# LasseWolter/laughter-detection-icsi

Hardware: AMD Instinct MI355X
Metric: 1 s@16 kHz segments/sec (featurize+ResNet fwd/bwd) (higher is better)
Workload: dtype f32 (64->64 and 32->32 convolutions: f16x2 split operands with per-tile power-of-two scales, f32 accumulate; error vs float64 within 1.5x of the exact-f32 kernels'); 1 GPU; BASELINE configs[2]: end-to-end featurize (HIP fbank 44 mel) + ResNetBigger resnet_base fwd/bwd + clip + Adam, random labels, dropout 0.5; global_batch=512, parallelism=dp1, overlap_wgrad=False, overlap_wgrad_small=True, bf16x3_convs=True, f16x2_convs=True, relu_bits=True, virtual_a1=True

## Files before the change

### include/lad_hip.h

```cpp
#ifndef LAD_HIP_H
#define LAD_HIP_H

#include <stdint.h>

#ifdef __cplusplus
extern "C" {
#endif

#define LAD_VERSION 100

enum lad_status {
    LAD_OK = 0,
    LAD_ERR_INVALID = -1,
    LAD_ERR_HIP = -2,
    LAD_ERR_NOMEM = -3,
    LAD_NOT_COVERED = 1
};

int lad_version(void);
const char *lad_last_error(void);

enum lad_pad_mode {
    LAD_PAD_KALDI_MIRROR = 0,
    LAD_PAD_CENTER_REFLECT = 1,
    LAD_PAD_CENTER_ZERO = 2
};
enum lad_log_mode {
    LAD_LOG_LN = 0,
    LAD_LOG_DB = 1,
    LAD_LOG_NONE = 2
};

typedef struct lad_fbank_cfg {
    int32_t n_fft;
    int32_t frame_len;
    int32_t hop;
    int32_t n_mels;
    int32_t n_mfcc;
    int32_t pad_mode;
    int32_t log_mode;
    int32_t remove_dc;
    float preemph;
    float log_floor;
} lad_fbank_cfg;

int lad_fbank_plan_create(const lad_fbank_cfg *cfg, const float *window, const float *melbank,
                          const float *dct, void **plan_out);
int lad_fbank_plan_destroy(void *plan);
int lad_fbank_plan_set_kernel(void *plan, int32_t which);
int lad_fbank_plan_has_fast_kernel(const void *plan);
int64_t lad_fbank_num_frames(const void *plan, int64_t samples_per_clip);
int lad_fbank_forward(void *plan, const float *pcm, int64_t n_clips, int64_t samples_per_clip,
                      float *out, void *stream);
int lad_fbank_forward_long(void *plan, const float *pcm, int64_t n_samples, float *out, void *stream);

int lad_gather_segments(const float *const *chan_ptr, const int64_t *chan_frames, const int32_t *chan,
                        const int64_t *first, const int32_t *count, int64_t n_seg, int32_t n_frames, int32_t F, float pad,
                        float *out, void *stream);

typedef struct lad_augment_params {
    uint64_t seed;
    uint32_t epoch;
    float p, mix_p;
    float snr_lo, snr_hi;
    float gain_lo, gain_hi;
    int32_t W;
    int32_t n_time, Wt;
    int32_t n_freq, Wf;
} lad_augment_params;
int lad_gather_segments_aug(const float *const *chan_ptr, const int64_t *chan_frames, const int32_t *chan,
                            const int64_t *first, const int32_t *count, int64_t n_seg, int32_t n_frames, int32_t F, float pad,
                            const lad_augment_params *params, const int32_t *noise_list, int32_t n_noise,
                            int64_t min_noise_frames, float *out, void *stream);

int lad_assemble_windows(const void *stream_act, const void *strips, void *out, int64_t n_windows, int32_t H, int32_t W,
                         int32_t band, int32_t row_bytes, void *stream);


int64_t lad_act_rows(int64_t batch, int32_t H, int32_t W);

int64_t lad_conv_packed_weight_floats(int32_t cout, int32_t cin, int32_t taps, int32_t mode);
int lad_conv_pack_weights(const float *w, int32_t cout, int32_t cin, int32_t taps, int32_t mode, float *wt,
                          void *stream);
int lad_conv_pack_weights_multi(const void *descs, int32_t n_desc, void *stream);
int64_t lad_conv_num_tiles(int64_t batch, int32_t H, int32_t W);
int lad_conv_fwd(const float *in, const float *wt, const float *bias, const float *addend, float *out,
                 float *stat_partials, int64_t batch, int32_t H, int32_t W, int32_t cin, int32_t cout, int32_t taps,
                 void *stream);
int lad_conv_s2_fwd(const float *in, const float *wt, const float *bias, float *out, float *stat_partials,
                    int64_t batch, int32_t H, int32_t W, int32_t cin, int32_t cout, int32_t taps, void *stream);
int lad_bn_fold(const float *gamma, const float *beta, const float *running_mean, const float *running_var,
                const float *conv_bias, int32_t channels, float *scale, float *shift, void *stream);
int lad_conv_fwd_eval(const float *in, const float *wt, const float *scale, const float *shift, const float *addend,
                      float *out, int64_t batch, int32_t H, int32_t W, int32_t cin, int32_t cout, int32_t taps,
                      int32_t relu, void *stream);
int lad_conv_s2_fwd_eval(const float *in, const float *wt, const float *scale, const float *shift, float *out,
                         int64_t batch, int32_t H, int32_t W, int32_t cin, int32_t cout, int32_t taps, int32_t relu,
                         void *stream);
int lad_upsample2(const float *src, float *up, int64_t batch, int32_t H, int32_t W, int32_t channels, void *stream);
int lad_conv_s2_dgrad(const float *dout, const float *wt, float *dx, int64_t batch, int32_t H, int32_t W, int32_t cin,
                      int32_t cout, int32_t taps, int32_t accumulate, void *stream);
int64_t lad_conv_s2_wgrad_workspace_floats(int32_t cin, int32_t cout, int32_t taps);
int lad_conv_s2_wgrad(const float *in, const float *dout, float *workspace, float *dw, float *dbias, int64_t batch, int32_t H,
                      int32_t W, int32_t cin, int32_t cout, int32_t taps, void *stream);
int64_t lad_conv_s2_wgrad_fused_workspace_floats(int32_t cin, int32_t cout);
int lad_conv_s2_wgrad_fused(const float *in, const float *dout, const float *dout_sc, float *workspace, float *dw,
                            float *dbias, float *dw_sc, int64_t batch, int32_t H, int32_t W, int32_t cin, int32_t cout,
                            void *stream);
int lad_conv_s2_fwd_fused(const float *in, const float *wt, const float *bias, const float *wt_sc, float *out,
                          float *stat_partials, float *out_sc, float *stat_partials_sc, int64_t batch, int32_t H, int32_t W,
                          int32_t cin, int32_t cout, void *stream);
int lad_conv_s2_dgrad_fused(const float *dout, const float *wt, const float *dout_sc, const float *wt_sc, float *dx,
                            int64_t batch, int32_t H, int32_t W, int32_t cin, int32_t cout, void *stream);
int64_t lad_conv_s2b3_packed_weight_bytes(void);
int lad_conv_s2b3_pack_weights(const float *w, const float *w_sc, void *wt, void *stream);
int lad_conv_s2b3_fwd(const float *in, const void *wt, const float *bias, float *out, float *stat_partials, float *out_sc,
                      float *stat_partials_sc, int64_t batch, int32_t H, int32_t W, void *stream);
int64_t lad_conv_s2b3_dgrad_packed_weight_bytes(void);
int lad_conv_s2b3_dgrad_pack_weights(const float *w, const float *w_sc, void *wt, void *stream);
int lad_conv_s2b3_pack_weights_pair(const float *w, const float *w_sc, void *wt_fwd, void *wt_dgrad, void *stream);
int64_t lad_conv_s2b3_dgrad_partials(int64_t batch, int32_t H, int32_t W);
int lad_conv_s2b3_dgrad(const float *dout, const float *dout_sc, const void *wt, float *dx, float *stat_partials, const float *bn_x,
                        const uint64_t *bn_bits, const float *bn_coef, int64_t batch, int32_t H, int32_t W, void *stream);
int64_t lad_conv_s2_dgrad_partials(int64_t batch, int32_t H, int32_t W);
int lad_conv_s2_dgrad_fused_bnstat(const float *dout, const float *wt, const float *dout_sc, const float *wt_sc, float *dx,
                                   float *stat_partials, const float *bn_x, const uint64_t *bn_bits, const float *bn_coef,
                                   int64_t batch, int32_t H, int32_t W, int32_t cin, int32_t cout, void *stream);
int64_t lad_conv_wgrad_workspace_floats(int32_t cin, int32_t cout, int32_t taps);
int lad_conv_wgrad(const float *in, const float *dout, float *workspace, float *dw, float *dbias, int64_t batch,
                   int32_t H, int32_t W, int32_t cin, int32_t cout, int32_t taps, void *stream);

int64_t lad_conv_b3_packed_weight_bytes(void);
int lad_conv_b3_pack_weights(const float *w, int32_t mode, void *wt, void *stream);
int lad_conv_b3_fwd_f32(const float *in, const void *wt, const float *bias, const float *addend, float *out,
                        float *partials, int64_t batch, int32_t H, int32_t W, void *stream);
int lad_conv_b3_fwd_f32_gated(const float *in, const void *wt, const float *bias, const float *addend,
                              const uint64_t *addend_bits, float *out, float *partials, int64_t batch, int32_t H,
                              int32_t W, void *stream);
int lad_conv_b3_dgrad_bnstat(const float *in, const void *wt, const float *addend, const uint64_t *addend_bits,
                             float *out, float *stat_partials, const float *bn_x, const uint64_t *bn_bits,
                             const float *bn_coef, int64_t batch, int32_t H, int32_t W, void *stream);
int64_t lad_conv_b3c_packed_weight_bytes(int32_t channels);
int lad_conv_b3c_pack_weights(const float *w, int32_t mode, void *wt, int32_t channels, void *stream);
int lad_conv_b3c_fwd_f32(const float *in, const void *wt, const float *bias, const float *addend, float *out,
                         float *partials, int64_t batch, int32_t H, int32_t W, int32_t channels, void *stream);
int lad_conv_b3c_dgrad_bnstat(const float *in, const void *wt, const float *addend, float *out, float *stat_partials,
                              const float *bn_x, const float *bn_coef, int64_t batch, int32_t H, int32_t W,
                              int32_t channels, void *stream);
int lad_conv_b3c_fwd_f32_bnrelu(const float *in, const float *in_coef, const void *wt, const float *bias, float *out,
                                float *partials, int64_t batch, int32_t H, int32_t W, int32_t channels, void *stream);
int64_t lad_conv_h2_packed_weight_bytes(int32_t channels);
int lad_conv_h2_pack_weights_multi(const void *table, int32_t n, int32_t channels, void *stream);
int lad_conv_wgrad_h2(const float *in, const float *in_coef, const float *dout, float *workspace, float *dw, float *dbias,
                      int64_t batch, int32_t H, int32_t W, int32_t channels, void *stream);
int lad_conv_wgrad_h2_bnbwd(const float *in, const float *in_coef, const float *dy, const float *bn_x, const uint64_t *bn_bits,
                            const float *bn_coef, const float *bcoef, float *dc, float *workspace, float *dw, float *dbias,
                            int64_t batch, int32_t H, int32_t W, int32_t channels, void *stream);
int lad_conv_h2(const float *in, const float *in_coef, const void *wt, const float *bias, const float *addend,
                const uint64_t *addend_bits, float *out, float *partials, const float *bn_x, const uint64_t *bn_bits,
                const float *bn_coef, int64_t batch, int32_t H, int32_t W, int32_t channels, void *stream);
int64_t lad_conv_wgrad_b3c_workspace_floats(int32_t channels);
int lad_conv_wgrad_b3c(const float *in, const float *in_coef, const float *dout, float *workspace, float *dw, float *dbias,
                       int64_t batch, int32_t H, int32_t W, int32_t channels, void *stream);
int lad_conv_b3_fwd_f32_bnrelu(const float *in, const float *in_coef, const void *wt, const float *bias, float *out,
                               float *partials, int64_t batch, int32_t H, int32_t W, void *stream);
int lad_conv_wgrad_b3_bnrelu(const float *in, const float *in_coef, const float *dout, float *workspace, float *dw,
                             float *dbias, int64_t batch, int32_t H, int32_t W, void *stream);
int lad_wgrad_defer_begin(void);
int lad_wgrad_defer_flush(void *stream);
int lad_conv_wgrad_b3(const float *in, const float *dout, float *workspace, float *dw, float *dbias, int64_t batch,
                      int32_t H, int32_t W, void *stream);

int lad_stem_fwd(const float *feat, const float *weight, float *out, float *stat_partials, int64_t batch, int32_t H,
                 int32_t W, int32_t cout, void *stream);
int lad_stem_fwd_eval(const float *feat, const float *weight, const float *scale, const float *shift, float *out,
                      int64_t batch, int32_t H, int32_t W, int32_t cout, int64_t frame_stride, int64_t frames_avail,
                      void *stream);
int64_t lad_stem_moments_workspace_doubles(void);
int64_t lad_stem_moments_doubles(void);
int lad_stem_bn_stats(const float *feat, const float *weight, const float *gamma, const float *beta, float *running_mean,
                      float *running_var, float momentum, float *coef, double *moments, double *workspace, int64_t batch, int32_t H,
                      int32_t W, int32_t cout, void *stream);
int64_t lad_stem_bwd_onepass_workspace_floats(void);
int lad_stem_bwd_onepass(const float *feat, const float *weight, const float *dy, const float *coef, const float *gamma,
                         const double *moments, float *workspace, float *dw, float *dgamma, float *dbeta, int64_t batch, int32_t H,
                         int32_t W, int32_t cout, void *stream);
int64_t lad_stem_wgrad_workspace_floats(void);
int lad_stem_wgrad(const float *feat, const float *dout, float *workspace, float *dw, int64_t batch, int32_t H,
                   int32_t W, int32_t cout, void *stream);
int lad_stem_wgrad_bn(const float *feat, const float *dy, const float *x, const float *weight, const float *coef,
                      const float *bcoef, float *workspace, float *dw, int64_t batch, int32_t H, int32_t W, int32_t cout,
                      void *stream);
int64_t lad_stem_bn_bwd_groups(int64_t batch, int32_t H, int32_t W);
int lad_stem_bn_bwd_sums(const float *feat, const float *weight, const float *dy, const float *coef, float *partials,
                         int64_t batch, int32_t H, int32_t W, int32_t cout, void *stream);

int lad_bn_finalize(float *stat_partials, int64_t n_tiles, int32_t channels, int64_t count, const float *gamma,
                    const float *beta, float *running_mean, float *running_var, float momentum, float *coef,
                    void *stream);
int lad_bn_finalize_pair(float *stat_partials_a, float *stat_partials_b, int64_t n_tiles, int32_t channels, int64_t count,
                         const float *gamma_a, const float *beta_a, float *running_mean_a, float *running_var_a, float *coef_a,
                         const float *gamma_b, const float *beta_b, float *running_mean_b, float *running_var_b, float *coef_b,
                         float momentum, void *stream);
int lad_bn_act(const float *x, const float *coef, const float *res, const float *res_coef, float *y, int64_t batch,
               int32_t H, int32_t W, int32_t channels, int32_t relu, void *stream);
int64_t lad_bn_bwd_workspace_floats(int32_t channels);
int lad_bn_bwd(const float *dy, const float *y, const float *x, const float *coef, const float *gamma,
               const float *xs, const float *scoef, const float *sgamma, float *dx, float *aux, float *dgamma,
               float *dbeta, float *dsgamma, float *dsbeta, float *workspace, float *bcoef, float *pre_partials,
               int64_t pre_tiles, int64_t batch, int32_t H, int32_t W, int32_t channels, int32_t relu, int32_t mode,
               void *stream);
int lad_bn_act_bits(const float *x, const float *coef, const float *res, const float *res_coef, float *y,
                    uint64_t *y_bits, int64_t batch, int32_t H, int32_t W, int32_t channels, void *stream);
int lad_bn_bwd_bits(const float *dy, const uint64_t *y_bits, const float *x, const float *coef, const float *gamma,
                    float *dx, float *dgamma, float *dbeta, float *workspace, float *bcoef, float *pre_partials,
                    int64_t pre_tiles, int64_t batch, int32_t H, int32_t W, int32_t channels, void *stream);
int lad_conv_fwd_bnstat(const float *in, const float *wt, const float *addend, float *out, float *stat_partials,
                        const float *bn_x, const float *bn_y, const float *bn_coef, int64_t batch, int32_t H, int32_t W,
                        int32_t cin, int32_t cout, int32_t taps, void *stream);

int lad_pool_fwd(const float *x, float *pooled, int64_t batch, int32_t H, int32_t W, int32_t channels, void *stream);
int lad_pool_bwd(const float *dpooled, float *dx, int64_t batch, int32_t H, int32_t W, int32_t channels, void *stream);
int64_t lad_head_workspace_floats(int64_t batch, int32_t F);
int lad_head_fwd_train(const float *const *params, const float *pooled, int64_t batch, int32_t F, const float *drop1,
                       const float *drop2, const int32_t *labels, float momentum, float *h, float *stats,
                       float *probs, float *metrics, void *stream);
int lad_head_fwd_train_rng(const float *const *params, const float *pooled, int64_t batch, int32_t F, float *drop1, float *drop2, float keep,
                           uint64_t seed, int64_t *rng_counter, int64_t *nbt, int32_t n_nbt, const int32_t *labels, float momentum,
                           float *h, float *stats, float *probs, float *metrics, void *stream);
int lad_head_fwd_eval(const float *const *params, const float *pooled, int64_t batch, int32_t F, float *probs,
                      void *stream);
int lad_bce_metrics(const float *probs, const int32_t *labels, int64_t n, float *metrics, void *stream);
int lad_head_bwd(const float *const *params, float *const *grads, const float *pooled, const float *h,
                 const float *stats, const float *probs, const float *dprobs, int64_t batch, int32_t F,
                 const float *drop1, const float *drop2, const int32_t *labels, float *workspace, float *dpooled,
                 void *stream);

int64_t lad_f16_packed_weight_halfs(int32_t cout, int32_t cin, int32_t taps);
int lad_f16_pack_weights(const float *w, int32_t cout, int32_t cin, int32_t taps, void *wt, void *stream);
int lad_f16_stem_fwd(const float *feat, const float *weight, const float *scale, const float *shift, void *out,
                     int64_t batch, int32_t H, int32_t W, int32_t cout, int64_t frame_stride, int64_t frames_avail,
                     void *stream);
int lad_f16_conv_fwd(const void *in, const void *wt, const float *scale, const float *shift, const void *addend, void *out,
                     int64_t batch, int32_t H, int32_t W, int32_t cin, int32_t cout, int32_t taps, int32_t relu,
                     void *stream);
int lad_f16_conv_s2_fwd(const void *in, const void *wt, const float *scale, const float *shift, void *out, int64_t batch,
                        int32_t H, int32_t W, int32_t cin, int32_t cout, int32_t taps, int32_t relu, void *stream);
int lad_f16_block_fwd(const void *x, const void *wt1, const float *scale1, const float *shift1, const void *wt2,
                      const float *scale2, const float *shift2, void *y, int64_t batch, int32_t H, int32_t W, int32_t channels,
                      void *stream);
int lad_f16_block_fwd_stem_rows(const void *stream_act, int64_t stream_rows, int64_t stream_row0, const float *feat, int64_t frames_avail,
                                const float *stem_weight, const float *stem_scale, const float *stem_shift, const void *wt1,
                                const float *scale1, const float *shift1, const void *wt2, const float *scale2, const float *shift2, void *y,
                                int64_t batch, int32_t H, int32_t W, void *stream);
int lad_f16_conv_s2_strips_fwd(const void *act, const void *wt, const float *scale, const float *shift, void *out, const void *wt_sc,
                               const float *scale_sc, const float *shift_sc, void *out_sc, int64_t n_windows, int32_t H, int32_t W,
                               int32_t band, int32_t strip_rows, int64_t bottom_image0, int64_t stream_row0, int64_t act_rows,
                               int32_t out_rows, void *stream);
int lad_f16_tail_fwd(const void *act, int64_t n_windows, int32_t H, int32_t W, int32_t band, int32_t strip_rows, int64_t bot_img0,
                     int64_t stream_row0, int32_t phases, int64_t phase_img, int64_t act_rows, const void *const *conv_params,
                     const float *const *head_params, int32_t F, float *probs, void *stream);
int lad_f16_conv_s2_fwd_windows(const void *act, const void *wt, const float *scale, const float *shift, void *out,
                                int64_t n_windows, int32_t H, int32_t W, int32_t band, int32_t cin, int32_t cout, int32_t taps,
                                int32_t relu, void *stream);
int lad_f16_conv_s2_fwd_mapped(const void *act, const void *wt, const float *scale, const float *shift, void *out,
                               int64_t n_windows, int32_t H, int32_t W, int32_t band, int32_t strip_rows, int64_t bottom_image0,
                               int64_t stream_row0, int32_t phases, int64_t phase_rows, int64_t act_rows, int32_t out_rows,
                               int32_t cin, int32_t cout, int32_t taps, int32_t relu, void *stream);
int lad_f16_conv_s2_fwd_sc(const void *in, const void *wt, const float *scale, const float *shift, void *out, const void *wt_sc,
                           const float *scale_sc, const float *shift_sc, void *out_sc, int64_t batch, int32_t H, int32_t W,
                           int32_t cin, int32_t cout, int32_t relu, void *stream);
int lad_f16_conv_s2_fwd_mapped_sc(const void *act, const void *wt, const float *scale, const float *shift, void *out,
                                  const void *wt_sc, const float *scale_sc, const float *shift_sc, void *out_sc, int64_t n_windows,
                                  int32_t H, int32_t W, int32_t band, int32_t strip_rows, int64_t bottom_image0, int64_t stream_row0,
                                  int32_t phases, int64_t phase_rows, int64_t act_rows, int32_t out_rows, int32_t cin, int32_t cout,
                                  int32_t relu, void *stream);
int lad_f16_pool_fwd(const void *x, float *pooled, int64_t batch, int32_t H, int32_t W, int32_t channels, void *stream);

int32_t lad_grad_sumsq_partials(void);
int lad_grad_sumsq(const float *grad, int64_t n, float *partials, int64_t *step_counter, void *stream);
int lad_grad_accumulate(float *acc, const float *grad, int64_t n, double scale, void *stream);
int lad_adam_step(float *param, float *grad, float *exp_avg, float *exp_avg_sq, int64_t n,
                  const float *sumsq_partials, double grad_scale, double max_norm, double lr, double beta1,
                  double beta2, double eps, int64_t step, const int64_t *step_counter, int32_t zero_grad,
                  float *norm_out, void *stream);

enum lad_runs_dtype { LAD_RUNS_F32 = 0, LAD_RUNS_F64 = 1 };
int32_t lad_runs_tile_frames(void);
int32_t lad_runs_max_thresholds(void);
int64_t lad_runs_workspace_bytes(int64_t channels, int64_t frames, int32_t n_thresholds);
int lad_runs_count(const void *probs, int32_t dtype, int64_t channels, int64_t frames, const double *thresholds,
                   int32_t n_thresholds, void *workspace, void *stream);
int lad_runs_fill(const void *probs, int32_t dtype, int64_t channels, int64_t frames, const double *thresholds,
                  int32_t n_thresholds, const void *workspace, const int32_t *counts_host, int32_t *table,
                  int64_t capacity_runs, void *stream);

enum lad_score_class { LAD_SCORE_INVALID = 0, LAD_SCORE_LAUGH = 1, LAD_SCORE_SPEECH = 2, LAD_SCORE_NOISE = 3, LAD_SCORE_SILENCE = 4 };
enum lad_score_field { LAD_SCORE_N_PRED = 0, LAD_SCORE_N_VALID = 1, LAD_SCORE_PRED_MS = 2, LAD_SCORE_CORR_MS = 3,
                       LAD_SCORE_FP_SPEECH_MS = 4, LAD_SCORE_FP_NOISE_MS = 5, LAD_SCORE_FP_SILENCE_MS = 6, LAD_SCORE_FIELDS = 7 };
int32_t lad_score_max_min_lengths(void);
int64_t lad_score_workspace_bytes(int64_t channels, int64_t n_intervals, int32_t n_thresholds, int32_t n_min_lengths);
int lad_score_runs(const void *runs_workspace, const int32_t *table, const int32_t *counts_host, int64_t channels,
                   int64_t frames, int32_t n_thresholds, const int32_t *bounds, const int32_t *offsets,
                   const int32_t *bounds_host, const int32_t *offsets_host, int64_t n_intervals, const double *fps,
                   const double *fps_host, const double *min_lengths, int32_t n_min_lengths, void *workspace,
                   int64_t *scores, void *stream);

enum lad_event_field { LAD_EVENT_N_REF = 0, LAD_EVENT_REF_TOUCHED = 1, LAD_EVENT_REF_HIT = 2, LAD_EVENT_PRED_HIT = 3,
                       LAD_EVENT_LINKS = 4, LAD_EVENT_ONSET_ABS_MS = 5, LAD_EVENT_OFFSET_ABS_MS = 6, LAD_EVENT_FIELDS = 7 };
int64_t lad_score_events_workspace_bytes(int64_t channels, int64_t n_intervals, int32_t n_thresholds, int32_t n_min_lengths,
                                         int64_t total_runs);
int lad_score_events(const void *runs_workspace, const int32_t *table, const int32_t *counts_host, int64_t channels,
                     int64_t frames, int32_t n_thresholds, const int32_t *bounds, const int32_t *offsets,
                     const int32_t *bounds_host, const int32_t *offsets_host, int64_t n_intervals, const double *fps,
                     const double *fps_host, const double *min_lengths, int32_t n_min_lengths,
                     int32_t min_overlap_ms, int32_t min_overlap_pct, void *workspace, int64_t *events, void *stream);

int32_t lad_binarize_max_settings(void);
int64_t lad_binarize_workspace_bytes(int64_t channels, int64_t frames, int32_t n_settings);
int lad_binarize_count(const void *probs, int32_t dtype, int64_t channels, int64_t frames, const double *onsets,
                       const double *offsets, int32_t n_settings, void *workspace, void *stream);
int lad_binarize_fill(const void *probs, int32_t dtype, int64_t channels, int64_t frames, const double *onsets,
                      const double *offsets, const double *min_gaps, int32_t n_settings, const double *fps,
                      const double *fps_host, void *workspace, const int32_t *counts_host, int32_t *raw_table,
                      int32_t *table, int64_t capacity_runs, void *stream);

int32_t lad_viterbi_max_settings(void);
int32_t lad_viterbi_table_entries(void);
int64_t lad_viterbi_workspace_bytes(int64_t channels, int64_t frames, int32_t n_settings);
int lad_viterbi_count(const void *probs, int32_t dtype, int64_t channels, int64_t frames, const int32_t *emission,
                      const int32_t *emission_host, const int32_t *bias, const int32_t *penalty, int32_t n_settings,
                      void *workspace, int64_t *best, void *stream);
int lad_viterbi_fill(const void *workspace, const int32_t *counts_host, int64_t channels, int64_t frames, int32_t n_settings,
                     int32_t *table, int64_t capacity_runs, void *stream);

int32_t lad_surface_max_levels(void);
int32_t lad_surface_tile_frames(void);
int64_t lad_surface_workspace_bytes(int64_t channels, int64_t frames, int64_t n_intervals, int32_t n_levels, int32_t n_min_lengths);
int lad_score_surface(const void *probs, int32_t dtype, int64_t channels, int64_t frames, const double *levels, int32_t n_levels,
                      const int32_t *bounds, const int32_t *offsets, const int32_t *bounds_host, const int32_t *offsets_host,
                      int64_t n_intervals, const double *fps, const double *fps_host, const double *min_lengths,
                      int32_t n_min_lengths, void *workspace, int64_t *scores, void *stream);

enum lad_resample_dtype { LAD_RESAMPLE_F32 = 0, LAD_RESAMPLE_I16 = 1 };
int64_t lad_resample_out_len(int64_t n_in, int32_t up, int32_t down);
int32_t lad_resample_tile_outputs(void);
int32_t lad_resample_max_up(void);
int32_t lad_resample_max_down(void);
int32_t lad_resample_max_taps(void);
int64_t lad_resample_max_lds_bytes(void);
int64_t lad_resample_lds_bytes(int32_t up, int32_t down, int32_t K);
int lad_resample(const void *x, int32_t x_dtype, int64_t n_in, const float *table, int32_t up, int32_t down, int32_t K,
                 int64_t out_first, int64_t n_out, float *y, void *stream);

int32_t lad_lowpass_tile_frames(void);
int64_t lad_lowpass_workspace_bytes(int64_t channels, int64_t frames);
int lad_lowpass(const void *probs, int32_t dtype, int64_t channels, int64_t frames, const int64_t *lengths_host,
                const double *b_host, const double *a_host, const double *zi_host, double *out, void *workspace,
                void *stream);

enum lad_sample_kind { LAD_SAMPLE_FIXED = 0, LAD_SAMPLE_POOL_ROW = 1, LAD_SAMPLE_POOL_MEASURE = 2 };
int lad_sample_segments(const int32_t *kind, const int32_t *src, int64_t n_rows, const int64_t *row_id, const int32_t *regions,
                        int64_t n_regions, const int32_t *pool_off, const int64_t *pool_cum, int32_t n_pools,
                        const int32_t *kind_host, const int32_t *src_host, const int32_t *pool_off_host,
                        const int64_t *pool_total_host, int32_t T, uint64_t seed, uint32_t epoch, int32_t *chan, int64_t *first,
                        int32_t *count, int32_t *region, void *stream);
int lad_window_coverage(const int32_t *set_chan, const int64_t *first, const int32_t *count, int64_t n, int32_t fps,
                        const int32_t *bounds, const int32_t *offsets, const int32_t *bounds_host, const int32_t *offsets_host,
                        int64_t n_intervals, int32_t n_channels, int32_t n_sets, int32_t *out, void *stream);

#ifdef __cplusplus
}
#endif
#endif
```

### laughter-detection-icsi_amd/_hip.py

```python
import ctypes
import os

import torch

_HERE = os.path.dirname(os.path.abspath(__file__))
LIB_PATH = os.environ.get("LAD_HIP_LIB") or os.path.join(_HERE, "liblad_hip.so")

c_void_p = ctypes.c_void_p
c_int = ctypes.c_int
c_i64 = ctypes.c_int64
c_float = ctypes.c_float
c_double = ctypes.c_double
c_i32 = ctypes.c_int32
c_float_p = ctypes.POINTER(ctypes.c_float)


class LadHipError(RuntimeError):
    pass


class FbankCfg(ctypes.Structure):
    _fields_ = [("n_fft", ctypes.c_int32), ("frame_len", ctypes.c_int32), ("hop", ctypes.c_int32),
                ("n_mels", ctypes.c_int32), ("n_mfcc", ctypes.c_int32), ("pad_mode", ctypes.c_int32),
                ("log_mode", ctypes.c_int32), ("remove_dc", ctypes.c_int32), ("preemph", ctypes.c_float),
                ("log_floor", ctypes.c_float)]


class AugmentParams(ctypes.Structure):
    _fields_ = [("seed", ctypes.c_uint64), ("epoch", ctypes.c_uint32), ("p", ctypes.c_float), ("mix_p", ctypes.c_float),
                ("snr_lo", ctypes.c_float), ("snr_hi", ctypes.c_float), ("gain_lo", ctypes.c_float), ("gain_hi", ctypes.c_float),
                ("W", ctypes.c_int32), ("n_time", ctypes.c_int32), ("Wt", ctypes.c_int32), ("n_freq", ctypes.c_int32),
                ("Wf", ctypes.c_int32)]


SIGNATURES = {
    "lad_version": (c_int, []),
    "lad_last_error": (ctypes.c_char_p, []),
    "lad_fbank_plan_create": (c_int, [ctypes.POINTER(FbankCfg), c_void_p, c_void_p, c_void_p,
                                      ctypes.POINTER(c_void_p)]),
    "lad_fbank_plan_destroy": (c_int, [c_void_p]),
    "lad_fbank_plan_set_kernel": (c_int, [c_void_p, c_int]),
    "lad_fbank_plan_has_fast_kernel": (c_int, [c_void_p]),
    "lad_fbank_num_frames": (c_i64, [c_void_p, c_i64]),
    "lad_fbank_forward": (c_int, [c_void_p, c_void_p, c_i64, c_i64, c_void_p, c_void_p]),
    "lad_fbank_forward_long": (c_int, [c_void_p, c_void_p, c_i64, c_void_p, c_void_p]),
    "lad_gather_segments": (c_int, [c_void_p] * 5 + [c_i64, c_i32, c_i32, c_float, c_void_p, c_void_p]),
    "lad_gather_segments_aug": (c_int, [c_void_p] * 5 + [c_i64, c_i32, c_i32, c_float, ctypes.POINTER(AugmentParams), c_void_p, c_i32, c_i64,
                                        c_void_p, c_void_p]),
    "lad_assemble_windows": (c_int, [c_void_p, c_void_p, c_void_p, c_i64, c_i32, c_i32, c_i32, c_i32, c_void_p]),
    "lad_act_rows": (c_i64, [c_i64, c_i32, c_i32]),
    "lad_conv_packed_weight_floats": (c_i64, [c_i32, c_i32, c_i32, c_i32]),
    "lad_conv_pack_weights": (c_int, [c_void_p, c_i32, c_i32, c_i32, c_i32, c_void_p, c_void_p]),
    "lad_conv_pack_weights_multi": (c_int, [c_void_p, c_i32, c_void_p]),
    "lad_conv_num_tiles": (c_i64, [c_i64, c_i32, c_i32]),
    "lad_conv_fwd": (c_int, [c_void_p] * 6 + [c_i64, c_i32, c_i32, c_i32, c_i32, c_i32, c_void_p]),
    "lad_conv_b3_packed_weight_bytes": (c_i64, []),
    "lad_conv_b3_pack_weights": (c_int, [c_void_p, c_i32, c_void_p, c_void_p]),
    "lad_conv_b3_fwd_f32": (c_int, [c_void_p] * 6 + [c_i64, c_i32, c_i32, c_void_p]),
    "lad_conv_b3c_packed_weight_bytes": (c_i64, [c_i32]),
    "lad_conv_b3c_pack_weights": (c_int, [c_void_p, c_i32, c_void_p, c_i32, c_void_p]),
    "lad_conv_b3c_fwd_f32": (c_int, [c_void_p] * 6 + [c_i64, c_i32, c_i32, c_i32, c_void_p]),
    "lad_conv_b3c_fwd_f32_bnrelu": (c_int, [c_void_p] * 6 + [c_i64, c_i32, c_i32, c_i32, c_void_p]),
    "lad_conv_b3c_dgrad_bnstat": (c_int, [c_void_p] * 7 + [c_i64, c_i32, c_i32, c_i32, c_void_p]),
    "lad_conv_h2_packed_weight_bytes": (c_i64, [c_i32]),
    "lad_conv_h2_pack_weights_multi": (c_int, [c_void_p, c_i32, c_i32, c_void_p]),
    "lad_conv_wgrad_h2": (c_int, [c_void_p] * 6 + [c_i64, c_i32, c_i32, c_i32, c_void_p]),
    "lad_conv_h2": (c_int, [c_void_p] * 11 + [c_i64, c_i32, c_i32, c_i32, c_void_p]),
    "lad_conv_wgrad_h2_bnbwd": (c_int, [c_void_p] * 11 + [c_i64, c_i32, c_i32, c_i32, c_void_p]),
    "lad_conv_wgrad_b3c_workspace_floats": (c_i64, [c_i32]),
    "lad_conv_wgrad_b3c": (c_int, [c_void_p] * 6 + [c_i64, c_i32, c_i32, c_i32, c_void_p]),
    "lad_conv_b3_fwd_f32_gated": (c_int, [c_void_p] * 7 + [c_i64, c_i32, c_i32, c_void_p]),
    "lad_conv_b3_fwd_f32_bnrelu": (c_int, [c_void_p] * 6 + [c_i64, c_i32, c_i32, c_void_p]),
    "lad_conv_wgrad_b3_bnrelu": (c_int, [c_void_p] * 6 + [c_i64, c_i32, c_i32, c_void_p]),
    "lad_wgrad_defer_begin": (c_int, []),
    "lad_wgrad_defer_flush": (c_int, [c_void_p]),
    "lad_conv_b3_dgrad_bnstat": (c_int, [c_void_p] * 9 + [c_i64, c_i32, c_i32, c_void_p]),
    "lad_conv_wgrad_b3": (c_int, [c_void_p] * 5 + [c_i64, c_i32, c_i32, c_void_p]),
    "lad_conv_s2_fwd": (c_int, [c_void_p] * 5 + [c_i64, c_i32, c_i32, c_i32, c_i32, c_i32, c_void_p]),
    "lad_bn_fold": (c_int, [c_void_p] * 5 + [c_i32, c_void_p, c_void_p, c_void_p]),
    "lad_conv_fwd_eval": (c_int, [c_void_p] * 6 + [c_i64, c_i32, c_i32, c_i32, c_i32, c_i32, c_i32, c_void_p]),
    "lad_conv_s2_fwd_eval": (c_int, [c_void_p] * 5 + [c_i64, c_i32, c_i32, c_i32, c_i32, c_i32, c_i32, c_void_p]),
    "lad_upsample2": (c_int, [c_void_p, c_void_p, c_i64, c_i32, c_i32, c_i32, c_void_p]),
    "lad_conv_s2_dgrad": (c_int, [c_void_p] * 3 + [c_i64, c_i32, c_i32, c_i32, c_i32, c_i32, c_i32, c_void_p]),
    "lad_conv_s2_wgrad_workspace_floats": (c_i64, [c_i32, c_i32, c_i32]),
    "lad_conv_s2_fwd_fused": (c_int, [c_void_p] * 8 + [c_i64, c_i32, c_i32, c_i32, c_i32, c_void_p]),
    "lad_conv_s2_dgrad_partials": (c_i64, [c_i64, c_i32, c_i32]),
    "lad_conv_s2b3_packed_weight_bytes": (c_i64, []),
    "lad_conv_s2b3_pack_weights": (c_int, [c_void_p, c_void_p, c_void_p, c_void_p]),
    "lad_conv_s2b3_fwd": (c_int, [c_void_p] * 7 + [c_i64, c_i32, c_i32, c_void_p]),
    "lad_conv_s2b3_dgrad_packed_weight_bytes": (c_i64, []),
    "lad_conv_s2b3_dgrad_pack_weights": (c_int, [c_void_p, c_void_p, c_void_p, c_void_p]),
    "lad_conv_s2b3_pack_weights_pair": (c_int, [c_void_p] * 5),
    "lad_conv_s2b3_dgrad_partials": (c_i64, [c_i64, c_i32, c_i32]),
    "lad_conv_s2b3_dgrad": (c_int, [c_void_p] * 8 + [c_i64, c_i32, c_i32, c_void_p]),
    "lad_conv_s2_dgrad_fused_bnstat": (c_int, [c_void_p] * 9 + [c_i64, c_i32, c_i32, c_i32, c_i32, c_void_p]),
    "lad_conv_s2_dgrad_fused": (c_int, [c_void_p] * 5 + [c_i64, c_i32, c_i32, c_i32, c_i32, c_void_p]),
    "lad_conv_s2_wgrad_fused_workspace_floats": (c_i64, [c_i32, c_i32]),
    "lad_conv_s2_wgrad_fused": (c_int, [c_void_p] * 7 + [c_i64, c_i32, c_i32, c_i32, c_i32, c_void_p]),
    "lad_conv_s2_wgrad": (c_int, [c_void_p] * 5 + [c_i64, c_i32, c_i32, c_i32, c_i32, c_i32, c_void_p]),
    "lad_conv_wgrad_workspace_floats": (c_i64, [c_i32, c_i32, c_i32]),
    "lad_conv_wgrad": (c_int, [c_void_p] * 5 + [c_i64, c_i32, c_i32, c_i32, c_i32, c_i32, c_void_p]),
    "lad_stem_fwd": (c_int, [c_void_p] * 4 + [c_i64, c_i32, c_i32, c_i32, c_void_p]),
    "lad_stem_fwd_eval": (c_int, [c_void_p] * 5 + [c_i64, c_i32, c_i32, c_i32, c_i64, c_i64, c_void_p]),
    "lad_stem_wgrad_workspace_floats": (c_i64, []),
    "lad_stem_wgrad": (c_int, [c_void_p] * 4 + [c_i64, c_i32, c_i32, c_i32, c_void_p]),
    "lad_stem_wgrad_bn": (c_int, [c_void_p] * 8 + [c_i64, c_i32, c_i32, c_i32, c_void_p]),
    "lad_stem_bn_bwd_groups": (c_i64, [c_i64, c_i32, c_i32]),
    "lad_stem_bn_bwd_sums": (c_int, [c_void_p] * 5 + [c_i64, c_i32, c_i32, c_i32, c_void_p]),
    "lad_bn_finalize": (c_int, [c_void_p, c_i64, c_i32, c_i64, c_void_p, c_void_p, c_void_p, c_void_p, c_float,
                                c_void_p, c_void_p]),
    "lad_stem_moments_workspace_doubles": (c_i64, []),
    "lad_stem_moments_doubles": (c_i64, []),
    "lad_stem_bn_stats": (c_int, [c_void_p] * 6 + [c_float] + [c_void_p] * 3 + [c_i64, c_i32, c_i32, c_i32, c_void_p]),
    "lad_stem_bwd_onepass_workspace_floats": (c_i64, []),
    "lad_stem_bwd_onepass": (c_int, [c_void_p] * 10 + [c_i64, c_i32, c_i32, c_i32, c_void_p]),
    "lad_bn_finalize_pair": (c_int, [c_void_p, c_void_p, c_i64, c_i32, c_i64] + [c_void_p] * 10 + [c_float, c_void_p]),
    "lad_bn_act": (c_int, [c_void_p] * 5 + [c_i64, c_i32, c_i32, c_i32, c_i32, c_void_p]),
    "lad_bn_bwd_workspace_floats": (c_i64, [c_i32]),
    "lad_bn_act_bits": (c_int, [c_void_p] * 6 + [c_i64, c_i32, c_i32, c_i32, c_void_p]),
    "lad_bn_bwd_bits": (c_int, [c_void_p] * 11 + [c_i64, c_i64, c_i32, c_i32, c_i32, c_void_p]),
    "lad_bn_bwd": (c_int, [c_void_p] * 17 + [c_i64, c_i64, c_i32, c_i32, c_i32, c_i32, c_i32, c_void_p]),
    "lad_conv_fwd_bnstat": (c_int, [c_void_p] * 8 + [c_i64, c_i32, c_i32, c_i32, c_i32, c_i32, c_void_p]),
    "lad_pool_fwd": (c_int, [c_void_p, c_void_p, c_i64, c_i32, c_i32, c_i32, c_void_p]),
    "lad_pool_bwd": (c_int, [c_void_p, c_void_p, c_i64, c_i32, c_i32, c_i32, c_void_p]),
    "lad_head_workspace_floats": (c_i64, [c_i64, c_i32]),
    "lad_head_fwd_train": (c_int, [c_void_p, c_void_p, c_i64, c_i32, c_void_p, c_void_p, c_void_p, c_float,
                                   c_void_p, c_void_p, c_void_p, c_void_p, c_void_p]),
    "lad_head_fwd_train_rng": (c_int, [c_void_p, c_void_p, c_i64, c_i32, c_void_p, c_void_p, c_float, ctypes.c_uint64, c_void_p, c_void_p, c_i32,
                                       c_void_p, c_float, c_void_p, c_void_p, c_void_p, c_void_p, c_void_p]),
    "lad_head_fwd_eval": (c_int, [c_void_p, c_void_p, c_i64, c_i32, c_void_p, c_void_p]),
    "lad_bce_metrics": (c_int, [c_void_p, c_void_p, c_i64, c_void_p, c_void_p]),
    "lad_head_bwd": (c_int, [c_void_p] * 7 + [c_i64, c_i32] + [c_void_p] * 6),
    "lad_f16_packed_weight_halfs": (c_i64, [c_i32, c_i32, c_i32]),
    "lad_f16_pack_weights": (c_int, [c_void_p, c_i32, c_i32, c_i32, c_void_p, c_void_p]),
    "lad_f16_stem_fwd": (c_int, [c_void_p] * 5 + [c_i64, c_i32, c_i32, c_i32, c_i64, c_i64, c_void_p]),
    "lad_f16_conv_fwd": (c_int, [c_void_p] * 6 + [c_i64, c_i32, c_i32, c_i32, c_i32, c_i32, c_i32, c_void_p]),
    "lad_f16_block_fwd": (c_int, [c_void_p] * 8 + [c_i64, c_i32, c_i32, c_i32, c_void_p]),
    "lad_f16_conv_s2_fwd_sc": (c_int, [c_void_p] * 9 + [c_i64, c_i32, c_i32, c_i32, c_i32, c_i32, c_void_p]),
    "lad_f16_conv_s2_fwd_mapped_sc": (c_int, [c_void_p] * 9 + [c_i64, c_i32, c_i32, c_i32, c_i32, c_i64, c_i64, c_i32, c_i64, c_i64, c_i32,
                                              c_i32, c_i32, c_i32, c_void_p]),
    "lad_f16_conv_s2_fwd": (c_int, [c_void_p] * 5 + [c_i64, c_i32, c_i32, c_i32, c_i32, c_i32, c_i32, c_void_p]),
    "lad_f16_conv_s2_fwd_windows": (c_int, [c_void_p] * 5 + [c_i64, c_i32, c_i32, c_i32, c_i32, c_i32, c_i32, c_i32, c_void_p]),
    "lad_f16_conv_s2_fwd_mapped": (c_int, [c_void_p] * 5 + [c_i64, c_i32, c_i32, c_i32, c_i32, c_i64, c_i64, c_i32, c_i64, c_i64, c_i32,
                                                          c_i32, c_i32, c_i32, c_i32, c_void_p]),
    "lad_f16_block_fwd_stem_rows": (c_int, [c_void_p, c_i64, c_i64, c_void_p, c_i64] + [c_void_p] * 10 + [c_i64, c_i32, c_i32, c_void_p]),
    "lad_f16_conv_s2_strips_fwd": (c_int, [c_void_p] * 9 + [c_i64, c_i32, c_i32, c_i32, c_i32, c_i64, c_i64, c_i64, c_i32, c_void_p]),
    "lad_f16_tail_fwd": (c_int, [c_void_p, c_i64, c_i32, c_i32, c_i32, c_i32, c_i64, c_i64, c_i32, c_i64, c_i64, c_void_p, c_void_p, c_i32,
                                 c_void_p, c_void_p]),
    "lad_f16_pool_fwd": (c_int, [c_void_p, c_void_p, c_i64, c_i32, c_i32, c_i32, c_void_p]),
    "lad_grad_sumsq_partials": (c_i32, []),
    "lad_grad_sumsq": (c_int, [c_void_p, c_i64, c_void_p, c_void_p, c_void_p]),
    "lad_grad_accumulate": (c_int, [c_void_p, c_void_p, c_i64, c_double, c_void_p]),
    "lad_adam_step": (c_int, [c_void_p] * 4 + [c_i64, c_void_p] + [c_double] * 6 + [c_i64, c_void_p, c_i32, c_void_p, c_void_p]),
    "lad_runs_tile_frames": (c_i32, []),
    "lad_runs_max_thresholds": (c_i32, []),
    "lad_runs_workspace_bytes": (c_i64, [c_i64, c_i64, c_i32]),
    "lad_runs_count": (c_int, [c_void_p, c_i32, c_i64, c_i64, ctypes.POINTER(c_double), c_i32, c_void_p, c_void_p]),
    "lad_runs_fill": (c_int, [c_void_p, c_i32, c_i64, c_i64, ctypes.POINTER(c_double), c_i32, c_void_p,
                              ctypes.POINTER(c_i32), c_void_p, c_i64, c_void_p]),
    "lad_score_max_min_lengths": (c_i32, []),
    "lad_score_workspace_bytes": (c_i64, [c_i64, c_i64, c_i32, c_i32]),
    "lad_score_runs": (c_int, [c_void_p, c_void_p, ctypes.POINTER(c_i32), c_i64, c_i64, c_i32, c_void_p, c_void_p,
                               ctypes.POINTER(c_i32), ctypes.POINTER(c_i32), c_i64, c_void_p, ctypes.POINTER(c_double),
                               ctypes.POINTER(c_double), c_i32, c_void_p, c_void_p, c_void_p]),
    "lad_score_events_workspace_bytes": (c_i64, [c_i64, c_i64, c_i32, c_i32, c_i64]),
    "lad_score_events": (c_int, [c_void_p, c_void_p, ctypes.POINTER(c_i32), c_i64, c_i64, c_i32, c_void_p, c_void_p,
                                 ctypes.POINTER(c_i32), ctypes.POINTER(c_i32), c_i64, c_void_p, ctypes.POINTER(c_double),
                                 ctypes.POINTER(c_double), c_i32, c_i32, c_i32, c_void_p, c_void_p, c_void_p]),
    "lad_binarize_max_settings": (c_i32, []),
    "lad_binarize_workspace_bytes": (c_i64, [c_i64, c_i64, c_i32]),
    "lad_binarize_count": (c_int, [c_void_p, c_i32, c_i64, c_i64, ctypes.POINTER(c_double), ctypes.POINTER(c_double), c_i32,
                                   c_void_p, c_void_p]),
    "lad_binarize_fill": (c_int, [c_void_p, c_i32, c_i64, c_i64] + [ctypes.POINTER(c_double)] * 3
                          + [c_i32, c_void_p, ctypes.POINTER(c_double), c_void_p, ctypes.POINTER(c_i32), c_void_p, c_void_p, c_i64,
                             c_void_p]),
    "lad_viterbi_max_settings": (c_i32, []),
    "lad_viterbi_table_entries": (c_i32, []),
    "lad_viterbi_workspace_bytes": (c_i64, [c_i64, c_i64, c_i32]),
    "lad_viterbi_count": (c_int, [c_void_p, c_i32, c_i64, c_i64, c_void_p] + [ctypes.POINTER(c_i32)] * 3
                          + [c_i32, c_void_p, c_void_p, c_void_p]),
    "lad_viterbi_fill": (c_int, [c_void_p, ctypes.POINTER(c_i32), c_i64, c_i64, c_i32, c_void_p, c_i64, c_void_p]),
    "lad_surface_max_levels": (c_i32, []),
    "lad_surface_tile_frames": (c_i32, []),
    "lad_surface_workspace_bytes": (c_i64, [c_i64, c_i64, c_i64, c_i32, c_i32]),
    "lad_score_surface": (c_int, [c_void_p, c_i32, c_i64, c_i64, ctypes.POINTER(c_double), c_i32, c_void_p, c_void_p,
                                  ctypes.POINTER(c_i32), ctypes.POINTER(c_i32), c_i64, c_void_p, ctypes.POINTER(c_double),
                                  ctypes.POINTER(c_double), c_i32, c_void_p, c_void_p, c_void_p]),
    "lad_resample_out_len": (c_i64, [c_i64, c_i32, c_i32]),
    "lad_resample_tile_outputs": (c_i32, []),
    "lad_resample_max_up": (c_i32, []),
    "lad_resample_max_down": (c_i32, []),
    "lad_resample_max_taps": (c_i32, []),
    "lad_resample_max_lds_bytes": (c_i64, []),
    "lad_resample_lds_bytes": (c_i64, [c_i32, c_i32, c_i32]),
    "lad_resample": (c_int, [c_void_p, c_i32, c_i64, c_void_p, c_i32, c_i32, c_i32, c_i64, c_i64, c_void_p, c_void_p]),
    "lad_lowpass_tile_frames": (c_i32, []),
    "lad_lowpass_workspace_bytes": (c_i64, [c_i64, c_i64]),
    "lad_lowpass": (c_int, [c_void_p, c_i32, c_i64, c_i64, ctypes.POINTER(c_i64)] + [ctypes.POINTER(c_double)] * 3
                    + [c_void_p, c_void_p, c_void_p]),
    "lad_sample_segments": (c_int, [c_void_p, c_void_p, c_i64, c_void_p, c_void_p, c_i64, c_void_p, c_void_p, c_i32,
                                    ctypes.POINTER(c_i32), ctypes.POINTER(c_i32), ctypes.POINTER(c_i32), ctypes.POINTER(c_i64),
                                    c_i32, ctypes.c_uint64, ctypes.c_uint32, c_void_p, c_void_p, c_void_p, c_void_p, c_void_p]),
    "lad_window_coverage": (c_int, [c_void_p, c_void_p, c_void_p, c_i64, c_i32, c_void_p, c_void_p, ctypes.POINTER(c_i32),
                                    ctypes.POINTER(c_i32), c_i64, c_i32, c_i32, c_void_p, c_void_p]),
}

_lib = None


def lib():
    global _lib
    if _lib is None:
        if not os.path.exists(LIB_PATH):
            raise LadHipError(
                f"{LIB_PATH} not found: build it with `python laughter-detection-icsi_amd/build.py` "
                "(there is no CPU fallback for the HIP hot path)")
        l = ctypes.CDLL(LIB_PATH)
        for name, (res, args) in SIGNATURES.items():
            fn = getattr(l, name)
            fn.restype = res
            fn.argtypes = args
        _lib = l
    return _lib


LAD_ERR_INVALID = -1
LAD_NOT_COVERED = 1


def check(rc, what=""):
    if rc != 0:
        msg = lib().lad_last_error().decode("utf-8", "replace")
        raise LadHipError(f"{what or 'liblad_hip'} failed ({rc}): {msg}")


def require_cuda(t, name="tensor", dtype=None):
    if not isinstance(t, torch.Tensor) or not t.is_cuda:
        raise LadHipError(f"{name} must be a GPU tensor (the HIP path has no CPU fallback)")
    if not t.is_contiguous():
        raise LadHipError(f"{name} must be contiguous")
    if dtype is not None and t.dtype != dtype:
        raise LadHipError(f"{name} must have dtype {dtype}, got {t.dtype}")
    return t


def ptr(t):
    return c_void_p(t.data_ptr()) if t is not None else c_void_p(0)


def stream_handle(device=None):
    return c_void_p(torch.cuda.current_stream(device).cuda_stream)
```

### laughter-detection-icsi_amd/csrc/head.hip

```cpp
#include "lad_common.h"
#include "lad_device.h"
#include "lad_philox.h"

namespace {
using namespace lad;

#ifdef LAD_STAMP
__device__ unsigned long long lad_dbg_head[64];
#define LAD_HEAD_STAMP(k) if (threadIdx.x == 0) lad_dbg_head[k] = __builtin_amdgcn_s_memtime();
#else
#define LAD_HEAD_STAMP(k)
#endif

constexpr float BN_EPS = 1e-5f;
constexpr int HID = 32;
constexpr int HEAD_THREADS = 1024;
constexpr int MAX_F = 128;
constexpr int CH = 64;

struct HeadArgs {
    int B, F;
    const float *g2, *b2;
    float *rm2, *rv2;
    const float *W1, *bias1;
// ... 274 lines not shown
        metrics[tid] = (tid == 0) ? s / (float)B : s;
    }
    if (tid == 5) metrics[5] = (float)B;
    if (a.rng_counter != nullptr && tid == 6) *a.rng_counter += 1;
    if (a.nbt != nullptr && tid >= 64 && tid - 64 < a.n_nbt) a.nbt[tid - 64] += 1;
    LAD_HEAD_STAMP(6)
}

__global__ __launch_bounds__(256) void head_fwd_eval_kernel(HeadArgs a, const float *__restrict__ pooled, float *__restrict__ probs) {
    __shared__ float zs[MAX_F], zt[MAX_F];
    __shared__ float w1t[MAX_F * HID];
    __shared__ float us[HID], ut[HID], w2s[HID], b1s[HID];
    const int tid = threadIdx.x, F = a.F;
    for (int i = tid; i < F * HID; i += blockDim.x) {
        const int j = i / F, f = i - j * F;
        w1t[f * HID + j] = a.W1[i];
    }
    for (int f = tid; f < F; f += blockDim.x) {
        const float s = a.g2[f] / sqrtf(a.rv2[f] + BN_EPS);
        zs[f] = s;
        zt[f] = a.b2[f] - a.rm2[f] * s;
    }
    if (tid < HID) {
        const float s = a.g3[tid] / sqrtf(a.rv3[tid] + BN_EPS);
        us[tid] = s;
        ut[tid] = a.b3[tid] - a.rm3[tid] * s;
        w2s[tid] = a.W2[tid];
        b1s[tid] = a.bias1[tid];
    }
    __syncthreads();
    const int64_t b = (int64_t)blockIdx.x * blockDim.x + tid;
    if (b >= a.B) return;
    float acc[HID];
#pragma unroll
    for (int j = 0; j < HID; ++j) acc[j] = b1s[j];
    const float *pr = pooled + b * F;
    for (int f = 0; f < F; ++f) {
        const float z = fmaf(pr[f], zs[f], zt[f]);
#pragma unroll
        for (int j = 0; j < HID; ++j) acc[j] = fmaf(w1t[f * HID + j], z, acc[j]);
    }
    float logit = a.bias2[0];
#pragma unroll
    for (int j = 0; j < HID; ++j) logit = fmaf(w2s[j], fmaxf(fmaf(acc[j], us[j], ut[j]), 0.f), logit);
    probs[b] = sigmoidf(logit);
}

__global__ __launch_bounds__(HEAD_THREADS) void bce_metrics_kernel(const float *__restrict__ probs, const int *__restrict__ labels,
                                                                   int n, float *__restrict__ metrics) {
    __shared__ float red[5][HEAD_THREADS / 64];
    const int tid = threadIdx.x, nt = blockDim.x;
    float vals[5] = {0.f, 0.f, 0.f, 0.f, 0.f};
    for (int b = tid; b < n; b += nt) {
        const float p = probs[b], t = (float)labels[b];
        const float lp = fmaxf(logf(p), -100.f), l1p = fmaxf(logf(1.f - p), -100.f);
        vals[0] -= t * lp + (1.f - t) * l1p;
        const float pred = rintf(p);
        vals[1] += (pred == t) ? 1.f : 0.f;
        vals[2] += pred;
        vals[3] += (pred == 1.f && t == 1.f) ? 1.f : 0.f;
        vals[4] += t;
    }
#pragma unroll
    for (int k = 0; k < 5; ++k) {
        const float v = wave_sum64(vals[k]);
        if ((tid & 63) == 0) red[k][tid >> 6] = v;
    }
    __syncthreads();
    if (tid < 5) {
        float s = 0.f;
        for (int w = 0; w < nt / 64; ++w) s += red[tid][w];
        metrics[tid] = (tid == 0) ? s / (float)n : s;
    }
    if (tid == 5) metrics[5] = (float)n;
}

struct HeadGrads {
    float *dg2, *db2, *dW1, *dbias1, *dg3, *db3, *dW2, *dbias2;
};

__global__ __launch_bounds__(HEAD_THREADS) void head_bwd_kernel(HeadArgs a, HeadGrads gr_out, const float *__restrict__ pooled,
                                                                const float *__restrict__ h, const float *__restrict__ stats,
                                                                const float *__restrict__ probs, const float *__restrict__ dprobs,
                                                                float *__restrict__ ws, float *__restrict__ dpooled) {
    __shared__ float zs[MAX_F], zt[MAX_F];
    __shared__ __attribute__((aligned(16))) float w1t[MAX_F * HID];
    __shared__ float us[HID], ut[HID], w2s[HID];
    __shared__ float ca[MAX_F], cb[MAX_F];
    __shared__ float mu2[MAX_F], is2[MAX_F], kk2[MAX_F];
    __shared__ float redw[HEAD_THREADS / 64];
    __shared__ __attribute__((aligned(16))) float z_s[CH * (MAX_F + 1)];
    __shared__ __attribute__((aligned(16))) float dh_s[CH * (HID + 4)];
    double *scratch = reinterpret_cast<double *>(z_s);
    const int tid = threadIdx.x, nt = blockDim.x;
    const int B = a.B, F = a.F;
    const float *mean2 = stats, *istd2 = stats + F, *mean3 = stats + 2 * F, *istd3 = stats + 2 * F + HID;
    float *du = ws, *gr = du + (int64_t)B * HID, *dh = gr + (int64_t)B * HID, *dz = dh + (int64_t)B * HID;

    LAD_HEAD_STAMP(16)
    for (int i = tid; i < F * HID; i += nt) {
        const int j = i / F, f = i - j * F;
        w1t[f * HID + j] = a.W1[i];
    }
    for (int f = tid; f < F; f += nt) {
        const float s = istd2[f] * a.g2[f];
        zs[f] = s;
        zt[f] = a.b2[f] - mean2[f] * s;
        mu2[f] = mean2[f];
        is2[f] = istd2[f];
        kk2[f] = a.g2[f] * istd2[f];
    }
    if (tid < HID) {
        const float s = istd3[tid] * a.g3[tid];
        us[tid] = s;
        ut[tid] = a.b3[tid] - mean3[tid] * s;
        w2s[tid] = a.W2[tid];
    }
    const int jt = tid & (HID - 1);
    const float mean3_j = mean3[jt], istd3_j = istd3[jt], k3_j = a.g3[jt] * istd3[jt];
    __syncthreads();
    LAD_HEAD_STAMP(17)
    float dl_sum = 0.f;
    struct S1 {
        float p, t, h, m;
    };
    batched<8, S1>(tid, B * HID, nt,
                   [&](int idx) {
                       const int b = idx >> 5;
                       return S1{probs[b], dprobs != nullptr ? dprobs[b] : (float)a.labels[b], h[idx], a.m2 ? a.m2[idx] : 1.f};
                   },
                   [&](int idx, const S1 &v) {
                       const int j = idx & 31;
                       const float p = v.p;
                       float dlogit;
                       if (dprobs != nullptr) dlogit = v.t * p * (1.f - p);
                       else dlogit = (p - v.t) / (float)B;
                       if (j == 0) dl_sum += dlogit;
                       float u = fmaf(v.h, us[j], ut[j]);
                       const float m = v.m;
                       u *= m;
                       gr[idx] = dlogit * fmaxf(u, 0.f);
                       du[idx] = (u > 0.f) ? dlogit * w2s[j] * m : 0.f;
                   });
    dl_sum = wave_sum64(dl_sum);
    if ((tid & 63) == 0) redw[tid >> 6] = dl_sum;
    __syncthreads();
    if (tid == 0) {
        float s = 0.f;
        for (int w = 0; w < nt / 64; ++w) s += redw[w];
        gr_out.dbias2[0] = s;
    }
    LAD_HEAD_STAMP(18)
    col_dot2(gr, nullptr, nullptr, nullptr, B, HID, gr_out.dW2, nullptr, scratch);
    col_dot2(du, h, mean3, istd3, B, HID, ca, cb, scratch);
    __syncthreads();
    if (tid < HID) {
        gr_out.db3[tid] = ca[tid];
        gr_out.dg3[tid] = cb[tid];
    }
    LAD_HEAD_STAMP(19)
    {
        const float ca_j = ca[jt] / (float)B, cb_j = cb[jt];
        batched<16, F2>(tid, B * HID, nt, [&](int idx) { return F2{h[idx], du[idx]}; },
                       [&](int idx, const F2 &v) {
                           const float xh = (v.a - mean3_j) * istd3_j;
                           dh[idx] = k3_j * (v.b - ca_j - xh * cb_j / (float)B);
                       });
    }
    __syncthreads();
    LAD_HEAD_STAMP(20)
    {
        const int fh = (F + 1) / 2;
        #pragma unroll 1
        for (int t = tid; t < 2 * B; t += nt) {
            const int b = t >> 1, fa = (t & 1) * fh, fb = min(F, fa + fh);
            float dhr[HID];
            const float4 *dr = reinterpret_cast<const float4 *>(dh + (int64_t)b * HID);
#pragma unroll
            for (int j = 0; j < HID; j += 4) {
                const float4 v = dr[j >> 2];
                dhr[j] = v.x; dhr[j + 1] = v.y; dhr[j + 2] = v.z; dhr[j + 3] = v.w;
            }
            const float *mr = a.m1 ? a.m1 + (int64_t)b * F : nullptr;
            float *zr = dz + (int64_t)b * F;
            for (int f0 = fa; f0 < fb; f0 += 8) {
                float mv[8];
#pragma unroll
                for (int k = 0; k < 8; ++k) mv[k] = (mr != nullptr && f0 + k < fb) ? mr[f0 + k] : 1.f;
#pragma unroll
                for (int k = 0; k < 8; ++k) {
                    const int f = f0 + k;
                    if (f < fb) {
                        float sacc = 0.f;
#pragma unroll
                        for (int j = 0; j < HID; ++j) sacc = fmaf(w1t[f * HID + j], dhr[j], sacc);
                        if (mr != nullptr) sacc *= mv[k];
                        zr[f] = sacc;
                    }
                }
            }
        }
    }
    LAD_HEAD_STAMP(21)
    constexpr int TJ = 4, TF = 3, DHS = HID + 4;
    const int ftiles = (F + TF - 1) / TF, ntile = (HID / TJ) * ftiles;
    int KS = 8;
    while (KS > 1 && (ntile * KS > nt || KS * HID * F > CH * (MAX_F + 1))) KS >>= 1;
    const bool worker = tid < ntile * KS;
    const int g = tid / ntile, tile = tid - g * ntile, tj = tile / ftiles, tf = tile - tj * ftiles;
    float wacc[TJ][TF];
#pragma unroll
    for (int x = 0; x < TJ; ++x)
#pragma unroll
        for (int y = 0; y < TF; ++y) wacc[x][y] = 0.f;
    constexpr int NZ = (CH * MAX_F + HEAD_THREADS - 1) / HEAD_THREADS, ND = (CH * HID + HEAD_THREADS - 1) / HEAD_THREADS;
    F2 pz[NZ];
    float pd[ND];
    auto fetch = [&](int c0) {
        const int nb = min(CH, B - c0);
#pragma unroll
        for (int k = 0; k < NZ; ++k) {
            const int idx = tid + k * nt;
            if (idx < nb * F) pz[k] = F2{pooled[(int64_t)c0 * F + idx], a.m1 ? a.m1[(int64_t)c0 * F + idx] : 1.f};
        }
#pragma unroll
        for (int k = 0; k < ND; ++k) {
            const int idx = tid + k * nt;
            if (idx < nb * HID) pd[k] = dh[(int64_t)c0 * HID + idx];
        }
    };
    fetch(0);
    for (int c0 = 0; c0 < B; c0 += CH) {
        const int nb = min(CH, B - c0);
#pragma unroll
        for (int k = 0; k < NZ; ++k) {
            const int idx = tid + k * nt;
            if (idx < nb * F) {
                const int b = idx / F, f = idx - b * F;
                float z = fmaf(pz[k].a, zs[f], zt[f]);
                if (a.m1) z *= pz[k].b;
                z_s[b * (MAX_F + 1) + f] = z;
            }
        }
#pragma unroll
        for (int k = 0; k < ND; ++k) {
            const int idx = tid + k * nt;
            if (idx < nb * HID) dh_s[(idx / HID) * DHS + (idx % HID)] = pd[k];
        }
        __syncthreads();
        if (c0 + CH < B) fetch(c0 + CH);
        if (worker) {
            for (int b = g; b < nb; b += KS) {
                const float4 dv = *reinterpret_cast<const float4 *>(dh_s + b * DHS + tj * TJ);
                const float dd[TJ] = {dv.x, dv.y, dv.z, dv.w};
                float zz[TF];
#pragma unroll
                for (int y = 0; y < TF; ++y) zz[y] = z_s[b * (MAX_F + 1) + min(tf * TF + y, MAX_F - 1)];
#pragma unroll
                for (int x = 0; x < TJ; ++x)
#pragma unroll
                    for (int y = 0; y < TF; ++y) wacc[x][y] = fmaf(dd[x], zz[y], wacc[x][y]);
            }
        }
        __syncthreads();
    }
    {
        float *part = z_s;
        if (worker) {
#pragma unroll
            for (int x = 0; x < TJ; ++x)
#pragma unroll
                for (int y = 0; y < TF; ++y) {
                    const int f = tf * TF + y;
                    if (f < F) part[(g * HID + tj * TJ + x) * F + f] = wacc[x][y];
                }
        }
        __syncthreads();
        for (int idx = tid; idx < HID * F; idx += nt) {
            float sacc = part[idx];
            for (int q = 1; q < KS; ++q) sacc += part[q * HID * F + idx];
            gr_out.dW1[idx] = sacc;
        }
        __syncthreads();
    }
    LAD_HEAD_STAMP(22)
    col_dot2(dh, nullptr, nullptr, nullptr, B, HID, gr_out.dbias1, nullptr, scratch);
    LAD_HEAD_STAMP(23)
    col_dot2(dz, pooled, mean2, istd2, B, F, ca, cb, scratch);
    __syncthreads();
    for (int f = tid; f < F; f += nt) {
        gr_out.db2[f] = ca[f];
        gr_out.dg2[f] = cb[f];
    }
    LAD_HEAD_STAMP(24)
    batched<12, F2>(tid, B * F, nt, [&](int idx) { return F2{pooled[idx], dz[idx]}; },
                   [&](int idx, const F2 &v) {
                       const int f = idx % F;
                       const float xh = (v.a - mu2[f]) * is2[f];
                       dpooled[idx] = kk2[f] * (v.b - ca[f] / (float)B - xh * cb[f] / (float)B);
                   });
    LAD_HEAD_STAMP(25)
}

int check_head(const HeadArgs &a) {
    using namespace lad;
    LAD_REQUIRE(a.B >= 1 && a.F >= 1 && a.F <= MAX_F, "head: F must be 1..%d (got %d), B >= 1", MAX_F, a.F);
    LAD_REQUIRE(a.g2 && a.b2 && a.rm2 && a.rv2 && a.W1 && a.bias1 && a.g3 && a.b3 && a.rm3 && a.rv3 && a.W2 && a.bias2,
                "head: null parameter pointer");
    return LAD_OK;
}

}

extern "C" int lad_pool_fwd(const float *x, float *pooled, int64_t batch, int32_t H, int32_t W, int32_t channels, void *stream) {
    using namespace lad;
    LAD_REQUIRE(x && pooled, "lad_pool_fwd: null buffer");
    LAD_REQUIRE(H >= 4 && W >= 4 && channels >= 1, "lad_pool_fwd: AvgPool2d(4) needs H, W >= 4");
    if (batch == 0) return LAD_OK;
    const int PH = H / 4, PW = W / 4;
    const int64_t n = batch * channels * PH * PW;
    hipLaunchKernelGGL(pool_fwd_kernel, dim3((unsigned)ceil_div(n, 256)), dim3(256), 0, (hipStream_t)stream, x, pooled, batch, H + 1,
                       W + 1, channels, PH, PW);
    return check_launch("pool_fwd_kernel");
}

extern "C" int lad_pool_bwd(const float *dpooled, float *dx, int64_t batch, int32_t H, int32_t W, int32_t channels, void *stream) {
    using namespace lad;
    LAD_REQUIRE(dpooled && dx, "lad_pool_bwd: null buffer");
    LAD_REQUIRE(H >= 4 && W >= 4 && channels >= 1, "lad_pool_bwd: AvgPool2d(4) needs H, W >= 4");
    if (batch == 0) return LAD_OK;
    const int64_t n = batch * (H + 1) * (W + 1) * channels;
    hipLaunchKernelGGL(pool_bwd_kernel, dim3((unsigned)std::min<int64_t>(ceil_div(n, 256), 4096)), dim3(256), 0, (hipStream_t)stream,
                       dpooled, dx, batch, H + 1, W + 1, channels, H / 4, W / 4);
    return check_launch("pool_bwd_kernel");
}

static HeadArgs make_args(const float *const *p, int64_t B, int32_t F, const float *m1, const float *m2, const int32_t *labels,
                          float momentum) {
    HeadArgs a;
    a.B = (int)B; a.F = F;
    a.g2 = p[0]; a.b2 = p[1]; a.rm2 = (float *)p[2]; a.rv2 = (float *)p[3];
    a.W1 = p[4]; a.bias1 = p[5];
    a.g3 = p[6]; a.b3 = p[7]; a.rm3 = (float *)p[8]; a.rv3 = (float *)p[9];
    a.W2 = p[10]; a.bias2 = p[11];
    a.m1 = m1; a.m2 = m2; a.labels = (const int *)labels; a.momentum = momentum;
    a.keep = 1.f; a.seed = 0; a.rng_counter = nullptr; a.nbt = nullptr; a.n_nbt = 0;
    return a;
}

extern "C" int64_t lad_head_workspace_floats(int64_t batch, int32_t F) { return batch * (3 * HID + F); }

extern "C" int lad_head_fwd_train(const float *const *params, const float *pooled, int64_t batch, int32_t F, const float *drop1,
                                  const float *drop2, const int32_t *labels, float momentum, float *h, float *stats, float *probs,
                                  float *metrics, void *stream) {
    using namespace lad;
    LAD_REQUIRE(params && pooled && h && stats && probs && metrics, "lad_head_fwd_train: null buffer");
    LAD_REQUIRE(batch < (1 << 24), "lad_head_fwd_train: batch too large for the single-workgroup train head");
    HeadArgs a = make_args(params, batch, F, drop1, drop2, labels, momentum);
    int rc = check_head(a);
    if (rc) return rc;
    hipLaunchKernelGGL(head_fwd_train_kernel, dim3(1), dim3(HEAD_THREADS), 0, (hipStream_t)stream, a, pooled, h, stats, probs, metrics);
    return check_launch("head_fwd_train_kernel");
}

extern "C" int lad_head_fwd_train_rng(const float *const *params, const float *pooled, int64_t batch, int32_t F, float *drop1, float *drop2,
                                      float keep, uint64_t seed, int64_t *rng_counter, int64_t *nbt, int32_t n_nbt, const int32_t *labels,
                                      float momentum, float *h, float *stats, float *probs, float *metrics, void *stream) {
    using namespace lad;
    LAD_REQUIRE(params && pooled && h && stats && probs && metrics, "lad_head_fwd_train_rng: null buffer");
    LAD_REQUIRE(batch >= 2, "lad_head_fwd_train_rng: batch statistics need at least two samples");
    const bool drop = keep < 1.0f;
    LAD_REQUIRE(!drop || (keep > 0.f && drop1 && drop2 && rng_counter && F % 4 == 0), "lad_head_fwd_train_rng: dropout needs mask buffers, a counter and F %% 4 == 0");
    LAD_REQUIRE(n_nbt >= 0 && n_nbt <= HEAD_THREADS - 64 && (n_nbt == 0 || nbt), "lad_head_fwd_train_rng: bad counter list");
    HeadArgs a = make_args(params, batch, F, drop ? drop1 : nullptr, drop ? drop2 : nullptr, labels, momentum);
    int rc = check_head(a);
    if (rc) return rc;
    a.keep = keep; a.seed = seed; a.rng_counter = drop ? (long long *)rng_counter : nullptr; a.nbt = (long long *)nbt; a.n_nbt = n_nbt;
    hipLaunchKernelGGL(head_fwd_train_kernel, dim3(1), dim3(HEAD_THREADS), 0, (hipStream_t)stream, a, pooled, h, stats, probs, metrics);
    return check_launch("head_fwd_train_kernel");
}

extern "C" int lad_head_fwd_eval(const float *const *params, const float *pooled, int64_t batch, int32_t F, float *probs, void *stream) {
    using namespace lad;
    LAD_REQUIRE(params && pooled && probs, "lad_head_fwd_eval: null buffer");
    if (batch == 0) return LAD_OK;
    HeadArgs a = make_args(params, batch, F, nullptr, nullptr, nullptr, 0.f);
    int rc = check_head(a);
    if (rc) return rc;
    hipLaunchKernelGGL(head_fwd_eval_kernel, dim3((unsigned)ceil_div(batch, 256)), dim3(256), 0, (hipStream_t)stream, a, pooled, probs);
    return check_launch("head_fwd_eval_kernel");
}

extern "C" int lad_bce_metrics(const float *probs, const int32_t *labels, int64_t n, float *metrics, void *stream) {
    using namespace lad;
    LAD_REQUIRE(probs && labels && metrics && n >= 1 && n < (1 << 30), "lad_bce_metrics: bad argument");
    hipLaunchKernelGGL(bce_metrics_kernel, dim3(1), dim3(HEAD_THREADS), 0, (hipStream_t)stream, probs, (const int *)labels, (int)n,
                       metrics);
    return check_launch("bce_metrics_kernel");
}

extern "C" int lad_head_bwd(const float *const *params, float *const *grads, const float *pooled, const float *h, const float *stats,
                            const float *probs, const float *dprobs, int64_t batch, int32_t F, const float *drop1, const float *drop2,
                            const int32_t *labels, float *workspace, float *dpooled, void *stream) {
    using namespace lad;
    LAD_REQUIRE(params && grads && pooled && h && stats && probs && workspace && dpooled, "lad_head_bwd: null buffer");
    LAD_REQUIRE(dprobs || labels, "lad_head_bwd: need dprobs or labels");
    HeadArgs a = make_args(params, batch, F, drop1, drop2, labels, 0.f);
    int rc = check_head(a);
    if (rc) return rc;
    HeadGrads g;
    g.dg2 = grads[0]; g.db2 = grads[1]; g.dW1 = grads[2]; g.dbias1 = grads[3];
    g.dg3 = grads[4]; g.db3 = grads[5]; g.dW2 = grads[6]; g.dbias2 = grads[7];
    hipLaunchKernelGGL(head_bwd_kernel, dim3(1), dim3(HEAD_THREADS), 0, (hipStream_t)stream, a, g, pooled, h, stats, probs, dprobs,
                       workspace, dpooled);
    return check_launch("head_bwd_kernel");
}

#ifdef LAD_STAMP
extern "C" int lad_debug_read_head_stamps(unsigned long long *host_dst, int64_t n) {
    return hipMemcpyFromSymbol(host_dst, HIP_SYMBOL(lad_dbg_head), n * sizeof(unsigned long long)) == hipSuccess ? 0 : -2;
}
#endif
```

### laughter-detection-icsi_amd/engine.py

```python
import ctypes
import math
import struct
from typing import FrozenSet, NamedTuple, Optional, Tuple

import torch

import _hip

_VP = ctypes.c_void_p


PREDICT_CHUNK = {"fp16": 8192, "fp32": 2048}
BASE_WIDTHS = (64, 32, 16, 16)
STREAM_SUPER_MAX = 1 << 20


class _LazyLevels(dict):

    def __init__(self, make):
        super().__init__()
        self._make = make

    def __missing__(self, key):
        value = self[key] = self._make(key)
# ... 77 lines not shown
        for j in range(2):
            name = f"block{bi}.{j}"
            stride = 2 if (j == 0 and bi > 1) else 1
            b = _BlockSpec(name)
            b.conv1 = _ConvSpec(name + ".conv1", cin, cout, 9, stride, h, w, base_widths)
            h, w = b.conv1.h_out, b.conv1.w_out
            b.conv2 = _ConvSpec(name + ".conv2", cout, cout, 9, 1, h, w, base_widths)
            if stride != 1 or cin != cout:
                b.sc_conv = _ConvSpec(name + ".shortcut.0", cin, cout, 1, stride, b.conv1.h_in, b.conv1.w_in, base_widths)
            blocks.append(b)
            cin = cout
    return blocks


class _ConvChoice(NamedTuple):
    arith: str
    wgrad: str
    wgrad_bn: bool
    label_fwd: str
    label_dgrad: str


class _BlockChoice(NamedTuple):
    entry: str
    a1_virtual: bool
    bits: bool
    dgrad2_bn: Optional[str]
    dgrad1_bn: Optional[str]
    sc_wgrad_fused: bool
    conv1: _ConvChoice
    conv2: _ConvChoice
    sc: Optional[_ConvChoice]


class _TrainSchedule(NamedTuple):
    blocks: Tuple[_BlockChoice, ...]
    stem_onepass: bool
    images: FrozenSet[Tuple[str, str]]
    opts: Tuple[Tuple[str, object], ...]


_ROW_LIMIT = (1 << 31) - (1 << 20)


def train_schedule(blocks, B, opts, stem_onepass):
    o = dict(opts)

    def arith(cs):
        fits = cs.rows(B) < _ROW_LIMIT if cs.cin == 64 else cs.rows(B) * cs.cin * 4 < _ROW_LIMIT
        if not (o["bf16x3"] and cs.b3 and (cs.cin == 64 or o["bf16x3_32"]) and fits):
            return "f32"
        return "h2" if o["f16x2"] and (cs.cin == 64 or o["f16x2_32"]) else "b3"

    def conv(cs, dgrad_f32=False, label_fwd=None):
        a = arith(cs)
        wg = "f32" if a == "f32" or not cs.b3_wgrad else "h2" if a == "h2" and cs.cin == 64 else "b3c"
        f32_label = f"conv_s{cs.stride}<{cs.cin},{cs.cout},{cs.taps}>"
        return _ConvChoice(a, wg, bool(o["fuse_bn_bwd_wgrad"]) and wg == "h2",
                           label_fwd or (f32_label if a == "f32" else f"conv_{a}<{cs.cin},{cs.cout},{cs.taps}>"),
                           f"conv_s1<{cs.cout},{cs.cin},{cs.taps}>" if a == "f32" or dgrad_f32 else f"conv_{a}<{cs.cout},{cs.cin},{cs.taps}>")

    out = []
    for bi, b in enumerate(blocks):
        c1, c2, sc = b.conv1, b.conv2, b.sc_conv
        a1, a2 = arith(c1), arith(c2)
        below_bits = bi > 0 and out[bi - 1].bits
        entry = "plain"
        if c1.stride != 1 and o["fuse_s2_shortcut"]:
            entry = "s2b3" if o["bf16x3"] and o["s2_b3"] and c1.s2b3 and c1.rows(B) < _ROW_LIMIT else "s2_fused"
        bits = bool(o["relu_bits"]) and sc is None and c1.b3_full and a1 != "f32" and not o["fuse_bn_bwd"]
        dgrad2_bn = "f32" if o["fuse_bn_bwd"] else "split" if o["fuse_bn_bwd_b3"] and a2 != "f32" else None
        if c1.stride != 1:
            fused = entry == "s2b3" or (entry == "s2_fused" and c1.cin == 64 and c1.cout == 32)
            dgrad1_bn = "split" if fused and o["fuse_bn_bwd_b3"] and below_bits else None
        elif bits:
            dgrad1_bn = "split" if o["fuse_bn_bwd_b3"] and below_bits else None
        else:
            dgrad1_bn = "f32" if o["fuse_bn_bwd"] and bi > 0 and blocks[bi - 1].sc_conv is None else None
        s2_label = f"conv_{'s2b3' if entry == 's2b3' else 's2'}<{c1.cin},{c1.cout},9>" if c1.stride != 1 else None
        out.append(_BlockChoice(entry, bool(o["virtual_a1"]) and a2 != "f32" and c2.b3_wgrad, bits, dgrad2_bn, dgrad1_bn,
                                c1.stride != 1 and bool(o["fuse_s2_shortcut_wgrad"]),
                                conv(c1, dgrad1_bn == "f32", s2_label), conv(c2, dgrad2_bn == "f32"), conv(sc) if sc is not None else None))
    images = {(ch.arith if ch.arith == "h2" else "b3c", cs.name) for b, blk in zip(blocks, out)
              for cs, ch in ((b.conv1, blk.conv1), (b.conv2, blk.conv2)) if ch.arith != "f32"}
    images |= {("s2b3", b.conv1.name) for b, blk in zip(blocks, out) if blk.entry == "s2b3"}
    return _TrainSchedule(tuple(out), bool(stem_onepass), frozenset(images), tuple(o.items()))


def conv_s1_entry(arith, cin, in_coef=False, gated=False, bn=None):
    if arith == "h2" and bn != "y":
        return "lad_conv_h2"
    if arith == "b3" and in_coef and not gated and bn is None:
        return "lad_conv_b3c_fwd_f32_bnrelu"
    if arith == "b3" and gated and not in_coef and cin == 64 and bn in (None, "bits"):
        return "lad_conv_b3_dgrad_bnstat" if bn else "lad_conv_b3_fwd_f32_gated"
    if arith == "b3" and not in_coef and not gated and bn in (None, "x"):
        return "lad_conv_b3c_dgrad_bnstat" if bn else "lad_conv_b3c_fwd_f32"
    if arith == "f32" and not in_coef and not gated and bn != "bits":
        return "lad_conv_fwd_bnstat" if bn else "lad_conv_fwd"
    raise _hip.LadHipError(f"no stride-1 convolution kernel for arithmetic {arith!r} at {cin} channels with in_coef={in_coef}, "
                           f"gated={gated}, bn={bn!r}")


def conv_wgrad_entry(kind, in_coef=False, bn=False):
    if kind == "h2":
        return "lad_conv_wgrad_h2_bnbwd" if bn else "lad_conv_wgrad_h2"
    if kind == "b3c" and not bn:
        return "lad_conv_wgrad_b3c"
    if kind == "f32" and not bn and not in_coef:
        return "lad_conv_wgrad"
    raise _hip.LadHipError(f"no weight-gradient kernel for {kind!r} with in_coef={in_coef}, bn={bn}")


def _s2_shortcut_rides(b, opts):
    return bool(opts["f16_s2_shortcut_fused"]) and b.conv1.cin != 32


def _block_fits_lds(b, B, opts, hw=None):
    c = b.conv1
    if b.sc_conv is not None or c.stride != 1 or c.taps != 9 or c.cin != c.cout:
        return False
    h, w = hw if hw is not None else (c.h_in, c.w_in)
    img = (h + 1) * (w + 1)
    if c.cin == 64:
        return bool(opts["strip_block_fused"]) and B >= 256 and img <= 512 and img + w <= 562
    return bool(opts["small_block_fused"]) and c.cin in (16, 32) and B >= 512 and img <= 2048


def _tail_blocks_ok(tail):
    if len(tail) != 4:
        return False
    for k, b in enumerate(tail):
        down = k % 2 == 0
        cin = 32 if k == 0 else 16
        if (b.conv1.cin, b.conv1.cout, b.conv1.taps, b.conv1.stride) != (cin, 16, 9, 2 if down else 1):
            return False
        if (b.conv2.cin, b.conv2.cout, b.conv2.taps, b.conv2.stride) != (16, 16, 9, 1):
            return False
        if down != (b.sc_conv is not None) or (down and (b.sc_conv.cin, b.sc_conv.cout, b.sc_conv.taps, b.sc_conv.stride) != (cin, 16, 1, 2)):
            return False
    return True


class _StreamLayout(NamedTuple):
    B: int
    H: int
    W: int
    half: bool
    mode: str
    run: Optional[Tuple[int, int]]
    n1: int
    band: int
    Ht: Optional[int]
    Hs: Optional[int]
    n_strip: Optional[int]
    n_strip_max: Optional[int]
    img_t_rows: Optional[int]
    stream_row0: Optional[int]
    cat_rows: Optional[int]
    k3: Optional[int]
    H2: Optional[int]
    W2: Optional[int]
    band2: Optional[int]
    Ht2: Optional[int]
    shift2: Optional[int]
    h2s: Optional[int]
    n_strip2: Optional[int]
    n_strip2_max: Optional[int]
    img_t2: Optional[int]
    img_s2: Optional[int]
    stream2_base: Optional[int]
    rows2: Optional[int]
    window_fused: Tuple[bool, ...]
    rides: Tuple[bool, ...]
    stream_fused: Tuple[bool, ...]
    strip_fused: Tuple[bool, ...]
    stem_kept: bool
    strip_stem_rows: bool
    stream2_fused: Tuple[bool, ...]
    strip2_fused: Tuple[bool, ...]
    strips2_resident: bool
    tail_fused: bool

    @property
    def stream_rows(self):
        return self.Hs if self.run is None else self.run[0] + self.H - 1


def stream_layout(blocks, B, H, W, half, opts, run=None):
    o = dict(opts)
    n = len(blocks)
    window_fused = tuple(bool(half) and _block_fits_lds(b, B, o) for b in blocks)
    rides = tuple(bool(half) and b.sc_conv is not None and b.conv1.stride == 2 and b.sc_conv.stride == 2 and b.conv1.taps == 9
                  and b.sc_conv.taps == 1 and _s2_shortcut_rides(b, o) for b in blocks)
    n1 = 0
    while n1 < n and blocks[n1].conv1.stride == 1 and blocks[n1].sc_conv is None and blocks[n1].conv1.h_out == H:
        n1 += 1
    band = 1 + 2 * n1
    if n1 == 0 or H < 4 * band or B < 2:
        return _StreamLayout(B, H, W, bool(half), "per_window", None, n1, band, *(None,) * 20, window_fused, rides, (), (), False, False,
                             (), (), False, False)
    Hs, Ht = B + H - 1, 2 * band
    n_strip = B + H - Ht
    nb = blocks[n1] if n1 < n else None
    direct = bool(half and nb is not None and nb.sc_conv is not None and nb.conv1.stride == 2
                  and (nb.conv1.cin, nb.conv1.cout) == (64, 32) and o["stream_direct"])
    img_t_rows = (Ht + 1) * (W + 1)
    k3 = n1 + 1
    while direct and k3 < n and blocks[k3].conv1.stride == 1 and blocks[k3].sc_conv is None:
        k3 += 1
    n2 = k3 - n1 - 1
    margin2 = 1 + 2 * n2
    band2 = band // 2 + 1 + margin2
    Ht2 = 2 * band2
    shift2 = 2 * (H // 2 - Ht2)
    share2 = bool(direct and o["stream_level2"] and H % 2 == 0 and k3 < n and blocks[k3].sc_conv is not None
                  and blocks[k3].conv1.stride == 2 and (blocks[k3].conv1.cin, blocks[k3].conv1.cout) == (32, 16)
                  and H // 2 >= 2 * Ht2)
    if not (share2 and o["stream_super"]):
        run = None
    mode = "shared2" if share2 else "direct" if direct else "assembled"
    stream_rows = Hs if run is None else run[0] + H - 1
    n_strip_max = n_strip if run is None else run[1] + H - Ht
    stream_row0 = cat_rows = None
    if direct:
        stream_row0 = n_strip_max * img_t_rows
        cat_rows = stream_row0 + (stream_rows + 1) * (W + 1) + W + 2 + (2 * (W + 1) if share2 else 0)
    strip_fused = tuple(bool(half) and _block_fits_lds(b, n_strip, o, (Ht, W)) for b in blocks[:n1])
    stream_fused = tuple(bool(half) and _block_fits_lds(b, 1, o, (stream_rows, W)) for b in blocks[:n1])
    stem_kept = bool(half and o["strip_stem_shared"])
    strip_stem_rows = stem_kept and Ht >= 3 and strip_fused[0] and blocks[0].conv1.cin == 64
    level1 = (n1, band, Ht, Hs, n_strip, n_strip_max, img_t_rows, stream_row0, cat_rows)
    if not share2:
        return _StreamLayout(B, H, W, bool(half), mode, None, *level1, *(None,) * 13, window_fused, rides, stream_fused, strip_fused,
                             stem_kept, strip_stem_rows, (), (), False, False)
    H2, W2 = nb.conv1.h_out, nb.conv1.w_out
    h2s = (stream_rows + 1) // 2
    n_strip2 = B + shift2
    n_strip2_max = n_strip2 if run is None else run[1] + shift2
    img_t2, img_s2 = (Ht2 + 1) * (W2 + 1), (h2s + 1) * (W2 + 1)
    stream2_base = n_strip2_max * img_t2
    rows2 = stream2_base + 2 * img_s2 + W2 + 2
    return _StreamLayout(B, H, W, True, mode, run, *level1, k3, H2, W2, band2, Ht2, shift2, h2s, n_strip2, n_strip2_max, img_t2, img_s2,
                         stream2_base, rows2, window_fused, rides, stream_fused, strip_fused, stem_kept, strip_stem_rows,
                         tuple(_block_fits_lds(b, 2, o, (h2s, W2)) for b in blocks[n1 + 1:k3]),
                         tuple(_block_fits_lds(b, n_strip2, o, (Ht2, W2)) for b in blocks[n1 + 1:k3]),
                         rides[n1] and bool(o["strip2_resident"]) and (nb.conv1.cin, nb.conv1.cout) == (64, 32),
                         bool(o["tail_fused"]) and _tail_blocks_ok(blocks[k3:]))


class _StreamRun:
    __slots__ = ("i0", "S", "B_max", "base", "frames_avail", "cat", "cat2", "stem")

    def __init__(self, i0, S, B_max, base, frames_avail):
        self.i0, self.S, self.B_max = i0, S, B_max
        self.base, self.frames_avail = base, frames_avail
        self.cat = self.cat2 = self.stem = None


class ResNetEngine:
    KERNEL_OPTIONS =("bf16x3", "bf16x3_32", "f16x2", "f16x2_32", "relu_bits", "virtual_a1", "fuse_bn_bwd", "fuse_bn_bwd_b3", "fuse_bn_bwd_wgrad", "fuse_s2_shortcut",
                      "fuse_s2_shortcut_wgrad", "s2_b3")
    INFER_OPTIONS = ("stream_direct", "stream_level2", "stream_super", "strip_block_fused", "small_block_fused", "tail_fused", "strip2_resident",
                     "strip_stem_shared", "f16_s2_shortcut_fused")

    def __init__(self, model):
        self.model = model
        self.device = None
        self._flat_p = self._flat_g = None
        self._plans = {}
        self._step_count = 0
        self._lib = None
        self._grad_dirty = False
        self._train_forwards = 0
        self._weights_version = 0
        self.fuse_bn_bwd = False
        self.overlap_wgrad = False
        self.overlap_wgrad_small = "auto"
        self.stem_onepass = True
        self.bf16x3 = True
        self.fuse_bn_bwd_b3 = True
        self.fuse_bn_bwd_wgrad = True
        self.f16x2 = True
        self.f16x2_32 = True
        self.bf16x3_32 = True
        self.virtual_a1 = True
        self.s2_b3 = True
        self.stream_direct = True
        self.stream_level2 = True
        self.strip_block_fused = True
        self.small_block_fused = True
        self.stream_super = True
        self.tail_fused = True
        self.strip2_resident = True
        self.strip_stem_shared = True
        self._sup_cache = {}
        self._sup_plans = {}
        self._layouts = {}
        self.f16_s2_shortcut_fused = True
        self.fuse_s2_shortcut = True
        self.fuse_s2_shortcut_wgrad = True
        self.defer_wgrad_sums = True
        self._defer_on = False
        self._schedules = {}
        self.relu_bits = True
        self._side = None
        self._side_readers = {}
        self._side_pending = False
        self.debug_capture = None
        self.kernel_events = None
        self.base_widths = list(model.filter_sizes) == list(BASE_WIDTHS)
        if not self.base_widths:
            for k in self.KERNEL_OPTIONS:
                setattr(self, k, False)

    def lib(self):
        if self._lib is None:
            self._lib = _hip.lib()
        return self._lib

    def _named_params(self):
        return list(self.model.named_parameters())

    def ensure_flat(self):
        params = self._named_params()
        dev = params[0][1].device
        if dev.type != "cuda":
            raise _hip.LadHipError("ResNetBigger runs on the MI355X only: call model.set_device('cuda') first "
                                   "(the HIP path has no CPU fallback)")
        ok = self._flat_p is not None and self._flat_p.device == dev
        if ok:
            base = self._flat_p.data_ptr()
            for (name, p), off in zip(params, self._offsets):
                if p.data_ptr() != base + 4 * off or p.dtype != torch.float32:
                    ok = False
                    break
        if ok:
            return
        offs, total = [], 0
        for _, p in params:
            offs.append(total)
            total += _align4(p.numel())
        flat_p = torch.zeros(total, device=dev, dtype=torch.float32)
        flat_g = torch.zeros(total, device=dev, dtype=torch.float32)
        with torch.no_grad():
            for (name, p), off in zip(params, offs):
                view = flat_p[off:off + p.numel()].view(p.shape)
                view.copy_(p.data.to(torch.float32))
                old_grad = p.grad
                p.data = view
                gview = flat_g[off:off + p.numel()].view(p.shape)
                if old_grad is not None:
                    gview.copy_(old_grad)
                    p.grad = gview
        self._flat_p, self._flat_g, self._offsets, self._n_flat = flat_p, flat_g, offs, total
        self._acc_g = None
        self._exp_avg = torch.zeros_like(flat_p)
        self._exp_avg_sq = torch.zeros_like(flat_p)
        self._norm_partials = torch.zeros(int(self.lib().lad_grad_sumsq_partials()), device=dev)
        self._norm_out = torch.zeros(1, device=dev)
        self._step_dev = torch.zeros(1, device=dev, dtype=torch.int64)
        self._rng_counter = torch.zeros(1, device=dev, dtype=torch.int64)
        self._rng_seed = None
        self.device = dev
        self._plans = {}
        self._views = {name: (flat_p[off:off + p.numel()].view(p.shape), flat_g[off:off + p.numel()].view(p.shape))
                       for (name, p), off in zip(params, offs)}
        bns = [m for m in self.model.modules() if isinstance(m, (torch.nn.BatchNorm1d, torch.nn.BatchNorm2d))]
        self._nbt = torch.zeros(len(bns), device=dev, dtype=torch.int64)
        with torch.no_grad():
            for i, m in enumerate(bns):
                self._nbt[i] = m.num_batches_tracked.to(dev)
                m._buffers["num_batches_tracked"] = self._nbt[i]
        self._build_specs()
        self._weights_version += 1
        self._param_list = [p for _, p in params]

    def bump_num_batches_tracked(self):
        self.ensure_flat()
        self._nbt.add_(1)

    def grad_views(self):
        return {k: v[1] for k, v in self._views.items()}

    def attach_grads(self):
        for name, p in self._named_params():
            g = self._views[name][1]
            if p.grad is None or p.grad.data_ptr() != g.data_ptr():
                p.grad = g

    def _build_specs(self):
        m = self.model
        bufs = dict(m.named_buffers())
        lib, dev = self.lib(), self.device

        def bn(name, c, conv_bias=None):
            return _BnParams(name, c, self._views, bufs, dev, conv_bias)

        self.stem_w, self.stem_gw = self._views["conv1.weight"]
        self.stem_cout = self.stem_w.shape[0]
        self.stem_bn = bn("bn1", self.stem_cout)
        self._convs, self._bns = {}, {}
        for b in block_geometry(self.stem_cout, m.filter_sizes, 1, 1, self.base_widths):
            for cs, bn_name in ((b.conv1, ".bn1"), (b.conv2, ".bn2"), (b.sc_conv, ".shortcut.1")):
                if cs is not None:
                    par = self._convs[cs.name] = _ConvParams(cs.name, cs.cin, cs.cout, cs.taps, cs.stride, self.base_widths, self._views, lib, dev)
                    self._bns[b.name + bn_name] = bn(b.name + bn_name, cs.cout, par.b)
            if b.sc_conv is not None:
                self._convs[b.conv1.name].shortcut = self._convs[b.sc_conv.name]
        self._geom_specs = {}
        self._packed = None
        self._folded = None
        self._f16_packed = None
        self._pack_tables = {}
        self._tail_ptrs = None
        self.head_bn2 = bn("bn2", m.linear_layer_size)
        self.head_bn3 = bn("bn3", 32)
        names = ["bn2.weight", "bn2.bias", None, None, "linear1.weight", "linear1.bias", "bn3.weight", "bn3.bias",
                 None, None, "linear2.weight", "linear2.bias"]
        ptrs = []
        for i, n in enumerate(names):
            if n is not None:
                ptrs.append(self._views[n][0].data_ptr())
            else:
                t = {2: self.head_bn2.rm, 3: self.head_bn2.rv, 8: self.head_bn3.rm, 9: self.head_bn3.rv}[i]
                ptrs.append(t.data_ptr())
        self._head_params = (_VP * 12)(*ptrs)
        gnames = ["bn2.weight", "bn2.bias", "linear1.weight", "linear1.bias", "bn3.weight", "bn3.bias",
                  "linear2.weight", "linear2.bias"]
        self._head_grads = (_VP * 8)(*[self._views[n][1].data_ptr() for n in gnames])

    def _blocks_for(self, H, W, partial=False):
        key = (H, W, partial)
        if key in self._geom_specs:
            return self._geom_specs[key]
        blocks = block_geometry(self.stem_cout, self.model.filter_sizes, H, W, self.base_widths)
        for b in blocks:
            b.bn1, b.bn2 = self._bns[b.name + ".bn1"], self._bns[b.name + ".bn2"]
            b.conv1.par, b.conv2.par = self._convs[b.conv1.name], self._convs[b.conv2.name]
            if b.sc_conv is not None:
                b.sc_conv.par, b.sc_bn = self._convs[b.sc_conv.name], self._bns[b.name + ".shortcut.1"]
        h, w = blocks[-1].conv2.h_out, blocks[-1].conv2.w_out
        if partial:
            self._geom_specs[key] = (blocks, h, w, 0)
            return self._geom_specs[key]
        if h < 4 or w < 4:
            raise ValueError(f"input ({H},{W}) is too small: AvgPool2d(4) sees a {h}x{w} map")
        feat = blocks[-1].conv2.cout * (h // 4) * (w // 4)
        if feat != self.model.linear_layer_size:
            raise RuntimeError(f"running_mean should contain {feat} elements not {self.model.linear_layer_size}")
        self._geom_specs[key] = (blocks, h, w, feat)
        return self._geom_specs[key]

    def _plan(self, B, H, W, train):
        key = (B, H, W, train)
        p = self._plans.get(key)
        if p is not None:
            return p
        dev = self.device
        blocks, h4, w4, feat = self._blocks_for(H, W)
        lib = self.lib()

        def act(h, w, c):
            return torch.zeros(int(lib.lad_act_rows(B, h, w)) * c, device=dev, dtype=torch.float32)

        p = {"blocks": blocks, "h4": h4, "w4": w4, "feat": feat}
        c0 = self.stem_cout
        p["stem_a"] = act(H, W, c0)
        p["stem_coef"] = torch.zeros(6 * c0, device=dev)
        if train:
            p["stem_mom"] = torch.zeros(int(lib.lad_stem_moments_doubles()), device=dev, dtype=torch.float64)
            p["stem_mom_ws"] = torch.zeros(int(lib.lad_stem_moments_workspace_doubles()), device=dev, dtype=torch.float64)
            p["stem_bwd_ws"] = torch.zeros(int(lib.lad_stem_bwd_onepass_workspace_floats()), device=dev)
        max_tiles = int(lib.lad_conv_num_tiles(B, H, W))
        for b in blocks:
            if b.conv1.s2b3:
                max_tiles = max(max_tiles, int(lib.lad_conv_s2b3_dgrad_partials(B, b.conv1.h_in, b.conv1.w_in)))
        cmax = max([64] + [b.conv1.cout for b in blocks])
        p["partials"] = torch.zeros(max_tiles * 2 * cmax, device=dev)
        p["partials_sc"] = torch.zeros(max(int(lib.lad_conv_num_tiles(B, b.conv1.h_out, b.conv1.w_out)) * 2 * b.conv1.cout
                                           for b in blocks if b.sc_conv is not None) if any(b.sc_conv is not None for b in blocks) else 0,
                                       device=dev)
        acts = []
        for b in blocks:
            ho, wo, co = b.conv1.h_out, b.conv1.w_out, b.conv1.cout
            d = {"c1": act(ho, wo, co), "a1": act(ho, wo, co), "c2": act(ho, wo, co), "y": act(ho, wo, co),
                 "coef1": torch.zeros(6 * co, device=dev), "coef2": torch.zeros(6 * co, device=dev)}
            if b.sc_conv is not None:
                d["cs"] = act(ho, wo, co)
                d["coefs"] = torch.zeros(6 * co, device=dev)
            elif train and b.conv1.b3_full:
                d["ybits"] = torch.zeros(int(lib.lad_act_rows(B, ho, wo)), device=dev, dtype=torch.int64)
            acts.append(d)
        p["acts"] = acts
        p["pooled"] = torch.zeros(B * feat, device=dev)
        p["probs"] = torch.zeros(B, device=dev)
        if train:
            p["h"] = torch.zeros(B * 32, device=dev)
            p["hstats"] = torch.zeros(2 * feat + 64, device=dev)
            p["metrics"] = torch.zeros(8, device=dev)
            p["head_ws"] = torch.zeros(int(lib.lad_head_workspace_floats(B, feat)), device=dev)
            p["dpooled"] = torch.zeros(B * feat, device=dev)
            levels = {}
            for b, d in zip(blocks, acts):
                ho, wo, co = b.conv1.h_out, b.conv1.w_out, b.conv1.cout
                d["dc1"], d["dc2"] = act(ho, wo, co), act(ho, wo, co)
                if b.conv1.stride != 1:
                    d["aux"] = act(ho, wo, co)
            sizes = {(H, W): c0}
            for b in blocks:
                sizes[(b.conv1.h_out, b.conv1.w_out)] = max(sizes.get((b.conv1.h_out, b.conv1.w_out), 0), b.conv1.cout)
                sizes[(b.conv1.h_in, b.conv1.w_in)] = max(sizes.get((b.conv1.h_in, b.conv1.w_in), 0), b.conv1.cin,
                                                            b.conv1.cout)
            for (h, w), c in sizes.items():
                levels[(h, w)] = [act(h, w, c) for _ in range(4)]
            p["g"] = levels
            ws = max(max(int(lib.lad_conv_wgrad_workspace_floats(cs.cin, cs.cout, cs.taps)),
                         int(lib.lad_conv_s2_wgrad_fused_workspace_floats(cs.cin, cs.cout)) if cs.stride != 1 else 0)
                     for b in blocks for cs in (b.conv1, b.conv2, b.sc_conv) if cs is not None)
            ws = max(ws, int(lib.lad_stem_wgrad_workspace_floats()), int(lib.lad_conv_wgrad_b3c_workspace_floats(32)))
            p["wgrad_ws"] = torch.zeros(ws, device=dev)
            p["wgrad_ws_of"] = {}
            for b in blocks:
                for cs in (b.conv1, b.conv2, b.sc_conv):
                    if cs is not None:
                        n = int(lib.lad_conv_wgrad_workspace_floats(cs.cin, cs.cout, cs.taps))
                        if cs.b3_wgrad:
                            n = max(n, int(lib.lad_conv_wgrad_b3c_workspace_floats(cs.cin)))
                        if cs.stride != 1:
                            n = int(lib.lad_conv_s2_wgrad_fused_workspace_floats(cs.cin, cs.cout)) if cs.taps == 9 else \
                                int(lib.lad_conv_s2_wgrad_workspace_floats(cs.cin, cs.cout, cs.taps))
                        p["wgrad_ws_of"][cs.name] = torch.zeros(n, device=dev)
            p["bn_ws"] = torch.zeros(int(lib.lad_bn_bwd_workspace_floats(cmax)), device=dev)
            p["bcoef"] = torch.zeros(8 * cmax, device=dev)
        self._plans[key] = p
        return p

    def _st(self):
        return _hip.stream_handle(self.device)

    def notify_weights_changed(self):
        self._weights_version += 1

    def _weights_stamp(self):
        return (self._weights_version, sum(p._version for p in self._param_list))

    def _state_tag(self):
        bufs = sum(b._version for b in self.model.buffers())
        return self._weights_stamp() + (bufs, self._train_forwards)

    def _pack_weights(self, need_dgrad, sched=None):
        ver = self._weights_stamp()
        want = sched.images if sched is not None else frozenset()
        have = self._packed
        fresh = have is not None and have[0] == ver
        if fresh and have[1] >= need_dgrad and want <= have[2]:
            return
        lib, st = self.lib(), self._st()
        if not (fresh and have[1] >= need_dgrad):
            table = self._pack_tables.get(need_dgrad)
            if table is None:
                recs = [struct.pack("<QQiiii", par.w.data_ptr(), (par.wt_f if mode == 0 else par.wt_d).data_ptr(), par.cout, par.cin, par.taps, mode)
                        for par in self._convs.values() for mode in ((0, 1) if need_dgrad else (0,))]
                table = self._pack_tables[need_dgrad] = (torch.frombuffer(bytearray(b"".join(recs)), dtype=torch.uint8).to(self.device), len(recs))
            _hip.check(lib.lad_conv_pack_weights_multi(_hip.ptr(table[0]), table[1], st), "lad_conv_pack_weights_multi")
        h2 = []
        for kind, name in sorted(want - have[2] if fresh else want):
            par = self._convs[name]
            if kind == "s2b3":
                _hip.check(lib.lad_conv_s2b3_pack_weights_pair(_hip.ptr(par.w), _hip.ptr(par.shortcut.w), _hip.ptr(par.wt3_s2f),
                                                               _hip.ptr(par.wt3_s2d), st), "lad_conv_s2b3_pack_weights_pair")
            elif kind == "b3c":
                for mode, wt in ((0, par.wt3_f), (1, par.wt3_d)):
                    _hip.check(lib.lad_conv_b3c_pack_weights(_hip.ptr(par.w), mode, _hip.ptr(wt), par.cin, st), "lad_conv_b3c_pack_weights")
            else:
                h2.append(par)
        if h2:
            hkey = ("h2",) + tuple(par.name for par in h2)
            htab = self._pack_tables.get(hkey)
            if htab is None:
                recs = [struct.pack("<QQii", par.w.data_ptr(), wt.data_ptr(), mode, par.cin) for par in h2
                        for mode, wt in ((0, par.wt2_f), (1, par.wt2_d))]
                htab = self._pack_tables[hkey] = (torch.frombuffer(bytearray(b"".join(recs)), dtype=torch.uint8).to(self.device), len(recs))
            _hip.check(lib.lad_conv_h2_pack_weights_multi(_hip.ptr(htab[0]), htab[1], 0, st), "lad_conv_h2_pack_weights_multi")
        self._packed = (ver, need_dgrad or have[1], want | have[2]) if fresh else (ver, need_dgrad, want)

    def _eval_prepare(self, half):
        if not half:
            self._pack_weights(need_dgrad=False)
        tag = self._state_tag()
        lib, st = self.lib(), self._st()
        if self._folded != tag:
            for bn in (self.stem_bn, *self._bns.values()):
                _hip.check(lib.lad_bn_fold(_hip.ptr(bn.g), _hip.ptr(bn.b), _hip.ptr(bn.rm), _hip.ptr(bn.rv), _hip.ptr(bn.conv_bias),
                                           bn.c, _hip.ptr(bn.fold[0]), _hip.ptr(bn.fold[1]), st), "lad_bn_fold " + bn.name)
            self._folded = tag
        if half and self._f16_packed != tag:
            for par in self._convs.values():
                _hip.check(lib.lad_f16_pack_weights(_hip.ptr(par.w), par.cout, par.cin, par.taps, _hip.ptr(par.wt_h), st),
                           "lad_f16_pack_weights " + par.name)
            self._f16_packed = tag

    def _mark(self, label):
        if self.kernel_events is None or label not in self.kernel_events:
            return None
        ev = torch.cuda.Event(enable_timing=True)
        ev.record(torch.cuda.current_stream(self.device))
        return ev

    def _mark_end(self, label, start):
        if start is not None:
            ev = torch.cuda.Event(enable_timing=True)
            ev.record(torch.cuda.current_stream(self.device))
            self.kernel_events[label].append((start, ev))

    def _schedule(self, B, H, W):
        key = (B, H, W, self.stem_onepass) + tuple(getattr(self, k) for k in self.KERNEL_OPTIONS)
        sched = self._schedules.get(key)
        if sched is None:
            sched = self._schedules[key] = train_schedule(self._blocks_for(H, W)[0], B, {k: getattr(self, k) for k in self.KERNEL_OPTIONS},
                                                          self.stem_onepass)
        return sched

    def _conv_s1(self, cs, arith, direction, x, out, B, label=None, *, in_coef=None, bias=None, addend=None, abits=None, partials=None, bn=None):
        bx, bmask, bcoef = bn if bn is not None else (None, None, None)
        fn = conv_s1_entry(arith, cs.cin, in_coef is not None, abits is not None,
                           None if bn is None else "x" if bmask is None else "bits" if bmask.dtype == torch.int64 else "y")
        P, fwd, h, w = _hip.ptr, direction == "fwd", cs.h_in, cs.w_in
        wt = P(getattr(cs.par, {"h2": "wt2_", "b3": "wt3_", "f32": "wt_"}[arith] + ("f" if fwd else "d")))
        cio = (cs.cin, cs.cout) if fwd else (cs.cout, cs.cin)
        if fn == "lad_conv_h2":
            args = (P(x), P(in_coef), wt, P(bias), P(addend), P(abits), P(out), P(partials), P(bx), P(bmask), P(bcoef), B, h, w, cs.cin)
        elif fn == "lad_conv_b3c_fwd_f32":
            args = (P(x), wt, P(bias), P(addend), P(out), P(partials), B, h, w, cs.cin)
        elif fn == "lad_conv_b3c_fwd_f32_bnrelu":
            args = (P(x), P(in_coef), wt, P(bias), P(out), P(partials), B, h, w, cs.cin)
        elif fn == "lad_conv_b3c_dgrad_bnstat":
            args = (P(x), wt, P(addend), P(out), P(partials), P(bx), P(bcoef), B, h, w, cs.cin)
        elif fn == "lad_conv_b3_fwd_f32_gated":
            args = (P(x), wt, P(bias), P(addend), P(abits), P(out), P(partials), B, h, w)
        elif fn == "lad_conv_b3_dgrad_bnstat":
            args = (P(x), wt, P(addend), P(abits), P(out), P(partials), P(bx), P(bmask), P(bcoef), B, h, w)
        elif fn == "lad_conv_fwd":
            args = (P(x), wt, P(bias), P(addend), P(out), P(partials), B, h, w, *cio, cs.taps)
        else:
            args = (P(x), wt, P(addend), P(out), P(partials), P(bx), P(bmask), P(bcoef), B, h, w, *cio, cs.taps)
        t0 = self._mark(label)
        _hip.check(getattr(self.lib(), fn)(*args, self._st()), f"{fn}({direction}) {cs.name}")
        self._mark_end(label, t0)

    def _conv_fwd(self, cs, ch, x, out, partials, B, in_coef=None):
        if cs.stride == 1:
            self._conv_s1(cs, ch.arith, "fwd", x, out, B, ch.label_fwd, in_coef=in_coef, bias=cs.par.b, partials=partials)
            return
        t0 = self._mark(ch.label_fwd)
        _hip.check(self.lib().lad_conv_s2_fwd(_hip.ptr(x), _hip.ptr(cs.par.wt_f), _hip.ptr(cs.par.b), _hip.ptr(out), _hip.ptr(partials),
                                              B, cs.h_in, cs.w_in, cs.cin, cs.cout, cs.taps, self._st()), "lad_conv_s2_fwd " + cs.name)
        self._mark_end(ch.label_fwd, t0)

    def _bn_coef(self, bn, coef, partials, B, h, w):
        lib, st = self.lib(), self._st()
        n_tiles = int(lib.lad_conv_num_tiles(B, h, w))
        _hip.check(lib.lad_bn_finalize(_hip.ptr(partials), n_tiles, bn.c, B * h * w, _hip.ptr(bn.g), _hip.ptr(bn.b),
                                       _hip.ptr(bn.rm), _hip.ptr(bn.rv), 0.1, _hip.ptr(coef), st),
                   "lad_bn_finalize " + bn.name)

    def _bn_coef_pair(self, bn_a, coef_a, part_a, bn_b, coef_b, part_b, B, h, w):
        lib, st = self.lib(), self._st()
        n_tiles = int(lib.lad_conv_num_tiles(B, h, w))
        _hip.check(lib.lad_bn_finalize_pair(_hip.ptr(part_a), _hip.ptr(part_b), n_tiles, bn_a.c, B * h * w,
                                            _hip.ptr(bn_a.g), _hip.ptr(bn_a.b), _hip.ptr(bn_a.rm), _hip.ptr(bn_a.rv), _hip.ptr(coef_a),
                                            _hip.ptr(bn_b.g), _hip.ptr(bn_b.b), _hip.ptr(bn_b.rm), _hip.ptr(bn_b.rv), _hip.ptr(coef_b),
                                            0.1, st), "lad_bn_finalize_pair " + bn_a.name)

    def _bn_act(self, x, coef, res, rcoef, y, B, h, w, c, relu=1):
        _hip.check(self.lib().lad_bn_act(_hip.ptr(x), _hip.ptr(coef), _hip.ptr(res), _hip.ptr(rcoef), _hip.ptr(y), B, h, w, c,
                                         relu, self._st()), "lad_bn_act")

    def forward(self, x, train, labels=None, drop_masks=None):
        self.ensure_flat()
        _hip.require_cuda(x, "x", torch.float32)
        if x.dim() == 4:
            if x.shape[1] != 1:
                raise ValueError("ResNetBigger expects a single input channel: (B,1,T,F)")
            B, _, H, W = x.shape
        elif x.dim() == 3:
            B, H, W = x.shape
        else:
            raise ValueError("x must be (B,1,T,F) or (B,T,F)")
        if B == 0:
            return torch.zeros(0, device=x.device)
        if not train:
            return self._forward_eval(x.view(-1), B, H, W, frame_stride=H, frames_avail=B * H)
        if B < 2:
            raise ValueError("Expected more than 1 value per channel when training, got input size "
                             f"torch.Size([{B}, {self.model.linear_layer_size}])")
        lib, st = self.lib(), self._st()
        p = self._plan(B, H, W, True)
        blocks = p["blocks"]
        sched = p["schedule"] = self._schedule(B, H, W)
        self._pack_weights(need_dgrad=True, sched=sched)
        part = p["partials"]
        if sched.stem_onepass:
            bn = self.stem_bn
            _hip.check(lib.lad_stem_bn_stats(_hip.ptr(x), _hip.ptr(self.stem_w), _hip.ptr(bn.g), _hip.ptr(bn.b), _hip.ptr(bn.rm), _hip.ptr(bn.rv),
                                             0.1, _hip.ptr(p["stem_coef"]), _hip.ptr(p["stem_mom"]), _hip.ptr(p["stem_mom_ws"]), B, H, W,
                                             self.stem_cout, st), "lad_stem_bn_stats")
        else:
            _hip.check(lib.lad_stem_fwd(_hip.ptr(x), _hip.ptr(self.stem_w), None, _hip.ptr(part), B, H, W, self.stem_cout, st),
                       "lad_stem_fwd")
            self._bn_coef(self.stem_bn, p["stem_coef"], part, B, H, W)
        c0 = self.stem_cout
        scale, shift = p["stem_coef"][:c0], p["stem_coef"][c0:2 * c0]
        _hip.check(lib.lad_stem_fwd_eval(_hip.ptr(x), _hip.ptr(self.stem_w), _hip.ptr(scale), _hip.ptr(shift), _hip.ptr(p["stem_a"]),
                                         B, H, W, c0, H, B * H, st), "lad_stem_fwd_eval (train)")
        cur = p["stem_a"]
        for b, ch, a in zip(blocks, sched.blocks, p["acts"]):
            ho, wo, co = b.conv1.h_out, b.conv1.w_out, b.conv1.cout
            if ch.entry == "plain":
                self._conv_fwd(b.conv1, ch.conv1, cur, a["c1"], part, B)
                self._bn_coef(b.bn1, a["coef1"], part, B, ho, wo)
            else:
                t0 = self._mark(ch.conv1.label_fwd)
                if ch.entry == "s2b3":
                    _hip.check(lib.lad_conv_s2b3_fwd(_hip.ptr(cur), _hip.ptr(b.conv1.par.wt3_s2f), _hip.ptr(b.conv1.par.b), _hip.ptr(a["c1"]), _hip.ptr(part),
                                                     _hip.ptr(a["cs"]), _hip.ptr(p["partials_sc"]), B, b.conv1.h_in, b.conv1.w_in, st),
                               "lad_conv_s2b3_fwd " + b.conv1.name)
                else:
                    _hip.check(lib.lad_conv_s2_fwd_fused(_hip.ptr(cur), _hip.ptr(b.conv1.par.wt_f), _hip.ptr(b.conv1.par.b), _hip.ptr(b.sc_conv.par.wt_f),
                                                         _hip.ptr(a["c1"]), _hip.ptr(part), _hip.ptr(a["cs"]), _hip.ptr(p["partials_sc"]),
                                                         B, b.conv1.h_in, b.conv1.w_in, b.conv1.cin, b.conv1.cout, st),
                               "lad_conv_s2_fwd_fused " + b.conv1.name)
                self._mark_end(ch.conv1.label_fwd, t0)
                self._bn_coef_pair(b.bn1, a["coef1"], part, b.sc_bn, a["coefs"], p["partials_sc"], B, ho, wo)
            if ch.a1_virtual:
                self._conv_fwd(b.conv2, ch.conv2, a["c1"], a["c2"], part, B, in_coef=a["coef1"])
            else:
                self._bn_act(a["c1"], a["coef1"], None, None, a["a1"], B, ho, wo, co)
                self._conv_fwd(b.conv2, ch.conv2, a["a1"], a["c2"], part, B)
            self._bn_coef(b.bn2, a["coef2"], part, B, ho, wo)
            if b.sc_conv is not None:
                if ch.entry == "plain":
                    self._conv_fwd(b.sc_conv, ch.sc, cur, a["cs"], part, B)
                    self._bn_coef(b.sc_bn, a["coefs"], part, B, ho, wo)
                self._bn_act(a["c2"], a["coef2"], a["cs"], a["coefs"], a["y"], B, ho, wo, co)
            elif ch.bits:
                _hip.check(lib.lad_bn_act_bits(_hip.ptr(a["c2"]), _hip.ptr(a["coef2"]), _hip.ptr(cur), None, _hip.ptr(a["y"]),
                                               _hip.ptr(a["ybits"]), B, ho, wo, co, st), "lad_bn_act_bits")
            else:
                self._bn_act(a["c2"], a["coef2"], cur, None, a["y"], B, ho, wo, co)
            a["x"] = cur
            cur = a["y"]
        last = blocks[-1].conv2
        _hip.check(lib.lad_pool_fwd(_hip.ptr(cur), _hip.ptr(p["pooled"]), B, p["h4"], p["w4"], last.cout, st), "lad_pool_fwd")
        m1 = m2 = None
        rng = isinstance(drop_masks, str) and drop_masks == "rng"
        if drop_masks is not None and not rng:
            m1, m2 = drop_masks
            _hip.require_cuda(m1, "drop mask 1", torch.float32)
            _hip.require_cuda(m2, "drop mask 2", torch.float32)
            if tuple(m1.shape) != (B, p["feat"]) or tuple(m2.shape) != (B, 32):
                raise ValueError("dropout masks must be (B,linear_layer_size) and (B,32)")
        if labels is not None:
            _hip.require_cuda(labels, "labels", torch.int32)
            if labels.numel() != B:
                raise ValueError("labels must have one entry per sample")
        if rng:
            keep = 1.0 - float(self.model.dropout.p)
            if keep < 1.0:
                if "m1" not in p:
                    p["m1"] = torch.zeros((B, p["feat"]), device=self.device)
                    p["m2"] = torch.zeros((B, 32), device=self.device)
                m1, m2 = p["m1"], p["m2"]
            seed = int(torch.cuda.default_generators[self.device.index or 0].initial_seed()) & ((1 << 64) - 1)
            if seed != self._rng_seed:
                self._rng_seed = seed
                self._rng_counter.zero_()
            _hip.check(lib.lad_head_fwd_train_rng(self._head_params, _hip.ptr(p["pooled"]), B, p["feat"], _hip.ptr(m1), _hip.ptr(m2), keep,
                                                  seed, _hip.ptr(self._rng_counter), _hip.ptr(self._nbt), int(self._nbt.numel()),
                                                  _hip.ptr(labels), 0.1, _hip.ptr(p["h"]), _hip.ptr(p["hstats"]), _hip.ptr(p["probs"]),
                                                  _hip.ptr(p["metrics"]), st), "lad_head_fwd_train_rng")
        else:
            _hip.check(lib.lad_head_fwd_train(self._head_params, _hip.ptr(p["pooled"]), B, p["feat"], _hip.ptr(m1), _hip.ptr(m2),
                                              _hip.ptr(labels), 0.1, _hip.ptr(p["h"]), _hip.ptr(p["hstats"]),
                                              _hip.ptr(p["probs"]), _hip.ptr(p["metrics"]), st), "lad_head_fwd_train")
        p["saved"] = (x, labels, m1, m2, B, H, W)
        self._last_train_plan = p
        self._train_forwards += 1
        return p["probs"]

    def _plan_eval(self, B, H, W, dtype=torch.float32, partial=False, owner=None):
        key = (B, H, W, "eval", dtype) + (("partial",) if partial else ())
        if owner is not None and key not in self._sup_plans.setdefault(owner, []):
            self._sup_plans[owner].append(key)
        p = self._plans.get(key)
        if p is not None:
            return p
        dev = self.device
        blocks, h4, w4, feat = self._blocks_for(H, W, partial)
        p = {"blocks": blocks, "h4": h4, "w4": w4, "feat": feat}
        levels = {(H, W): self.stem_cout}
        for b in blocks:
            k = (b.conv1.h_out, b.conv1.w_out)
            levels[k] = max(levels.get(k, 0), b.conv1.cout)
        rows_of = lambda k: int(self.lib().lad_act_rows(B, k[0], k[1]))
        p["lv"] = _LazyLevels(lambda k: [torch.zeros(rows_of(k) * levels[k], device=dev, dtype=dtype) for _ in range(4)])
        p["pooled"] = torch.zeros(B * feat, device=dev)
        p["probs"] = torch.zeros(B, device=dev)
        self._plans[key] = p
        return p

    def _conv_eval(self, cs, bn, x, addend, out, B, relu):
        lib, st = self.lib(), self._st()
        label = f"conv_s{cs.stride}<{cs.cin},{cs.cout},{cs.taps}>"
        t0 = self._mark(label)
        if cs.stride == 1:
            _hip.check(lib.lad_conv_fwd_eval(_hip.ptr(x), _hip.ptr(cs.par.wt_f), _hip.ptr(bn.fold[0]), _hip.ptr(bn.fold[1]),
                                             _hip.ptr(addend), _hip.ptr(out), B, cs.h_in, cs.w_in, cs.cin, cs.cout, cs.taps, relu, st),
                       "lad_conv_fwd_eval " + cs.name)
        else:
            if addend is not None:
                raise _hip.LadHipError("stride-2 eval convolution takes no residual")
            _hip.check(lib.lad_conv_s2_fwd_eval(_hip.ptr(x), _hip.ptr(cs.par.wt_f), _hip.ptr(bn.fold[0]), _hip.ptr(bn.fold[1]),
                                                _hip.ptr(out), B, cs.h_in, cs.w_in, cs.cin, cs.cout, cs.taps, relu, st),
                       "lad_conv_s2_fwd_eval " + cs.name)
        self._mark_end(label, t0)

    def _conv_eval_f16(self, cs, bn, x, addend, out, B, relu):
        lib, st = self.lib(), self._st()
        label = f"conv_f16_s{cs.stride}<{cs.cin},{cs.cout},{cs.taps}>"
        t0 = self._mark(label)
        if cs.stride == 1:
            _hip.check(lib.lad_f16_conv_fwd(_hip.ptr(x), _hip.ptr(cs.par.wt_h), _hip.ptr(bn.fold[0]), _hip.ptr(bn.fold[1]),
                                            _hip.ptr(addend), _hip.ptr(out), B, cs.h_in, cs.w_in, cs.cin, cs.cout, cs.taps, relu, st),
                       "lad_f16_conv_fwd " + cs.name)
        else:
            _hip.check(lib.lad_f16_conv_s2_fwd(_hip.ptr(x), _hip.ptr(cs.par.wt_h), _hip.ptr(bn.fold[0]), _hip.ptr(bn.fold[1]),
                                               _hip.ptr(out), B, cs.h_in, cs.w_in, cs.cin, cs.cout, cs.taps, relu, st),
                       "lad_f16_conv_s2_fwd " + cs.name)
        self._mark_end(label, t0)

    def _eval_stem(self, half, fptr, out, out_byte_offset, B, H, W, frame_stride, frames_avail):
        lib, st = self.lib(), self._st()
        optr = ctypes.c_void_p(out.data_ptr() + out_byte_offset)
        fn, name = (lib.lad_f16_stem_fwd, "lad_f16_stem_fwd") if half else (lib.lad_stem_fwd_eval, "lad_stem_fwd_eval")
        _hip.check(fn(fptr, _hip.ptr(self.stem_w), _hip.ptr(self.stem_bn.fold[0]), _hip.ptr(self.stem_bn.fold[1]), optr, B, H, W,
                      self.stem_cout, frame_stride, max(0, frames_avail), st), name)

    def _eval_blocks(self, half, p, blocks, cur, B, fused, rides, final_out=None):
        conv = self._conv_eval_f16 if half else self._conv_eval
        lv = p["lv"]
        for bi, b in enumerate(blocks):
            L = lv[(b.conv1.h_out, b.conv1.w_out)]
            free = [t for t in L if t is not cur]
            a1, y = free[0], free[1]
            if final_out is not None and bi == len(blocks) - 1:
                y = final_out
            if fused[bi]:
                label = f"block_f16<{b.conv1.cin}>"
                t0 = self._mark(label)
                rc = self.lib().lad_f16_block_fwd(_hip.ptr(cur), *self._f16_args(b.conv1, b.bn1), *self._f16_args(b.conv2, b.bn2), _hip.ptr(y),
                                                  B, b.conv1.h_in, b.conv1.w_in, b.conv1.cin, self._st())
                if rc != _hip.LAD_NOT_COVERED:
                    _hip.check(rc, "lad_f16_block_fwd " + b.conv1.name)
                    self._mark_end(label, t0)
                    cur = y
                    continue
            if rides[bi]:
                cs = free[2]
                self._s2_plain_f16(b, _hip.ptr(cur), (_hip.ptr(a1), _hip.ptr(cs)), B, b.conv1.h_in, b.conv1.w_in, True)
                conv(b.conv2, b.bn2, a1, cs, y, B, 1)
                cur = y
                continue
            conv(b.conv1, b.bn1, cur, None, a1, B, 1)
            if b.sc_conv is not None:
                cs = free[2]
                conv(b.sc_conv, b.sc_bn, cur, None, cs, B, 0)
                conv(b.conv2, b.bn2, a1, cs, y, B, 1)
            else:
                conv(b.conv2, b.bn2, a1, cur, y, B, 1)
            cur = y
        return cur

    @staticmethod
    def _f16_args(cs, bn):
        return _hip.ptr(cs.par.wt_h), _hip.ptr(bn.fold[0]), _hip.ptr(bn.fold[1])

    def _s2_entry_f16(self, b, launch_one, launch_sc, rides):
        if rides:
            label = f"conv_f16_s2sc<{b.conv1.cin},{b.conv1.cout}>"
            t0 = self._mark(label)
            launch_sc()
            self._mark_end(label, t0)
            return
        for cs, bn, slot, relu in ((b.conv1, b.bn1, 0, 1), (b.sc_conv, b.sc_bn, 1, 0)):
            label = f"conv_f16_s2<{cs.cin},{cs.cout},{cs.taps}>"
            t0 = self._mark(label)
            launch_one(cs, bn, slot, relu)
            self._mark_end(label, t0)

    def _s2_plain_f16(self, b, src, dst, B, h, w, rides):
        lib, st = self.lib(), self._st()

        def one(cs, bn, slot, relu):
            _hip.check(lib.lad_f16_conv_s2_fwd(src, *self._f16_args(cs, bn), dst[slot], B, h, w, cs.cin, cs.cout, cs.taps, relu, st),
                       "lad_f16_conv_s2_fwd " + cs.name)

        def both():
            _hip.check(lib.lad_f16_conv_s2_fwd_sc(src, *self._f16_args(b.conv1, b.bn1), dst[0], *self._f16_args(b.sc_conv, b.sc_bn), dst[1],
                                                  B, h, w, b.conv1.cin, b.conv1.cout, 1, st), "lad_f16_conv_s2_fwd_sc " + b.conv1.name)
        self._s2_entry_f16(b, one, both, rides)

    def _s2_mapped_f16(self, b, src, dst, wmap, rides, strips_resident=False):
        lib, st = self.lib(), self._st()

        def one(cs, bn, slot, relu):
            _hip.check(lib.lad_f16_conv_s2_fwd_mapped(_hip.ptr(src), *self._f16_args(cs, bn), _hip.ptr(dst[slot]), *wmap,
                                                      cs.cin, cs.cout, cs.taps, relu, st), "lad_f16_conv_s2_fwd_mapped " + cs.name)

        def both():
            args = (_hip.ptr(src), *self._f16_args(b.conv1, b.bn1), _hip.ptr(dst[0]), *self._f16_args(b.sc_conv, b.sc_bn), _hip.ptr(dst[1]))
            if strips_resident:
                rc = lib.lad_f16_conv_s2_strips_fwd(*args, *wmap[:7], *wmap[9:], st)
                if rc != _hip.LAD_NOT_COVERED:
                    _hip.check(rc, "lad_f16_conv_s2_strips_fwd " + b.conv1.name)
                    return
            _hip.check(lib.lad_f16_conv_s2_fwd_mapped_sc(*args, *wmap, b.conv1.cin, b.conv1.cout, 1, st),
                       "lad_f16_conv_s2_fwd_mapped_sc " + b.conv1.name)
        self._s2_entry_f16(b, one, both, rides)

    def _eval_tail(self, half, p, cur, B, probs_out=None):
        lib, st = self.lib(), self._st()
        last = p["blocks"][-1].conv2
        p["block_out"] = cur
        pool, name = (lib.lad_f16_pool_fwd, "lad_f16_pool_fwd") if half else (lib.lad_pool_fwd, "lad_pool_fwd")
        _hip.check(pool(_hip.ptr(cur), _hip.ptr(p["pooled"]), B, p["h4"], p["w4"], last.cout, st), name)
        probs = probs_out if probs_out is not None else p["probs"]
        _hip.check(lib.lad_head_fwd_eval(self._head_params, _hip.ptr(p["pooled"]), B, p["feat"], _hip.ptr(probs), st),
                   "lad_head_fwd_eval")
        return probs

    def _require_half(self):
        if not self.base_widths:
            raise ValueError(f"precision 'fp16' runs the stage widths {list(BASE_WIDTHS)} (resnet_base) only; this model has "
                             f"{list(self.model.filter_sizes)}: use precision 'fp32'")

    def _layout(self, blocks, B, H, W, half, run=None):
        key = (B, H, W, half, run) + tuple(getattr(self, k) for k in self.INFER_OPTIONS)
        lay = self._layouts.get(key)
        if lay is None:
            lay = self._layouts[key] = stream_layout(blocks, B, H, W, half, {k: getattr(self, k) for k in self.INFER_OPTIONS}, run)
        return lay

    def _forward_eval_any(self, half, feat_flat, B, H, W, frame_stride, frames_avail, feat_offset_floats=0, probs_out=None):
        if half:
            self._require_half()
        p = self._plan_eval(B, H, W, torch.float16 if half else torch.float32)
        blocks = p["blocks"]
        lay = self._layout(blocks, B, H, W, half)
        self._eval_prepare(half)
        cur = p["lv"][(H, W)][0]
        fptr = ctypes.c_void_p(feat_flat.data_ptr() + 4 * feat_offset_floats)
        self._eval_stem(half, fptr, cur, 0, B, H, W, frame_stride, frames_avail)
        cur = self._eval_blocks(half, p, blocks, cur, B, lay.window_fused, lay.rides)
        return self._eval_tail(half, p, cur, B, probs_out)

    def _forward_eval(self, feat_flat, B, H, W, frame_stride, frames_avail, feat_offset_floats=0):
        return self._forward_eval_any(False, feat_flat, B, H, W, frame_stride, frames_avail, feat_offset_floats)

    def _forward_eval_stream(self, half, feat_flat, B, H, W, frames_avail, feat_offset_floats=0, run=None, d=0, probs_out=None):
        dtype = torch.float16 if half else torch.float32
        pw = self._plan_eval(B, H, W, dtype)
        lay = pw["layout"] = self._layout(pw["blocks"], B, H, W, half, None if run is None else (run.S, run.B_max))
        if lay.mode == "per_window":
            return self._forward_eval_any(half, feat_flat, B, H, W, 1, frames_avail, feat_offset_floats, probs_out)
        if lay.run is None:
            run, d = None, 0
        plans = {"pw": pw, "ps": self._plan_eval(1, lay.Hs, W, dtype, partial=True),
                 "pt": self._plan_eval(lay.n_strip, lay.Ht, W, dtype, partial=True)}
        self._eval_prepare(half)
        bufs = {}
        src = (feat_flat.data_ptr() + 4 * feat_offset_floats, frames_avail)
        self._stream_level1(lay, plans, bufs, run, src)
        self._strips_level1(lay, plans, bufs, run, src, d)
        if lay.mode == "shared2":
            self._stream_level2(lay, plans, bufs, run, d)
        return self._stream_tail(lay, plans, bufs, d, probs_out)

    def _stream_level1(self, lay, plans, bufs, run, src):
        half, W, C, n1 = lay.half, lay.W, self.stem_cout, lay.n1
        dtype = torch.float16 if half else torch.float32
        rows, ride = lay.stream_rows, lay.rides[:n1]
        if run is not None:
            bufs["cat"] = run.cat
            if run.cat is None:
                key = (run.S, run.B_max, lay.H, W)
                bufs["cat"] = run.cat = self._sup_buffer("l1", lay.cat_rows * C, dtype, key)
                psS = self._plan_eval(1, rows, W, dtype, partial=True, owner="l1")
                if lay.stem_kept:
                    cS = run.stem = self._sup_buffer("l0", int(self.lib().lad_act_rows(1, rows, W)) * C, dtype, key)
                else:
                    cS = psS["lv"][(rows, W)][0]
                self._eval_stem(half, ctypes.c_void_p(run.base), cS, 0, 1, rows, W, 1, run.frames_avail)
                self._eval_blocks(half, psS, psS["blocks"][:n1], cS, 1, lay.stream_fused, ride, final_out=run.cat[lay.stream_row0 * C:])
            bufs["stem"], bufs["stream"] = run.stem, None
            return
        pw, ps = plans["pw"], plans["ps"]
        cat = out_s = None
        if lay.cat_rows is not None:
            cat = pw.get("l1cat")
            if cat is None or cat.numel() != lay.cat_rows * C:
                cat = pw["l1cat"] = torch.zeros(lay.cat_rows * C, device=self.device, dtype=dtype)
            out_s = cat[lay.stream_row0 * C:]
        stem = None
        if lay.stem_kept:
            if ps.get("stem_keep") is None:
                ps["stem_keep"] = torch.zeros(int(self.lib().lad_act_rows(1, rows, W)) * C, device=self.device, dtype=dtype)
            cs = stem = ps["stem_keep"]
        else:
            cs = ps["lv"][(rows, W)][0]
        self._eval_stem(half, ctypes.c_void_p(src[0]), cs, 0, 1, rows, W, 1, src[1])
        bufs["cat"], bufs["stem"] = cat, stem
        bufs["stream"] = self._eval_blocks(half, ps, ps["blocks"][:n1], cs, 1, lay.stream_fused, ride, final_out=out_s)

    def _strips_level1(self, lay, plans, bufs, run, src, d):
        half, W, C, n1, n_strip, Ht = lay.half, lay.W, self.stem_cout, lay.n1, lay.n_strip, lay.Ht
        lib, st, cat, pt = self.lib(), self._st(), bufs["cat"], plans["pt"]
        out_t = None
        if cat is not None:
            out_t = cat[:(n_strip * lay.img_t_rows + W + 2) * C]
            if n_strip < lay.n_strip_max:
                cat[n_strip * lay.img_t_rows * C:(n_strip * lay.img_t_rows + W + 2) * C].zero_()
        ct = None
        b0 = pt["blocks"][0]
        fused, ride = lay.strip_fused, lay.rides[:n1]
        if lay.strip_stem_rows:
            y0 = out_t if n1 == 1 else pt["lv"][(Ht, W)][1]
            label = f"block_f16<{b0.conv1.cin}>"
            t0 = self._mark(label)
            rc = lib.lad_f16_block_fwd_stem_rows(_hip.ptr(bufs["stem"]), lay.stream_rows, d, ctypes.c_void_p(src[0]), max(0, src[1]),
                                                 _hip.ptr(self.stem_w), _hip.ptr(self.stem_bn.fold[0]), _hip.ptr(self.stem_bn.fold[1]),
                                                 *self._f16_args(b0.conv1, b0.bn1), *self._f16_args(b0.conv2, b0.bn2), _hip.ptr(y0),
                                                 n_strip, Ht, W, st)
            if rc != _hip.LAD_NOT_COVERED:
                _hip.check(rc, "lad_f16_block_fwd_stem_rows " + b0.conv1.name)
                self._mark_end(label, t0)
                ct = y0 if n1 == 1 else self._eval_blocks(half, pt, pt["blocks"][1:n1], y0, n_strip, fused[1:], ride[1:], final_out=out_t)
        if ct is None:
            ct = pt["lv"][(Ht, W)][0]
            self._eval_stem(half, ctypes.c_void_p(src[0]), ct, 0, n_strip, Ht, W, 1, src[1])
            ct = self._eval_blocks(half, pt, pt["blocks"][:n1], ct, n_strip, fused, ride, final_out=out_t)
        bufs["strips"] = ct

    def _sup_buffer(self, name, numel, dtype, run_key):
        key = ("sup", name, numel, dtype, run_key)
        buf = self._sup_cache.get(key)
        if buf is None:
            for k in [k for k in self._sup_cache if k[1] == name]:
                del self._sup_cache[k]
            for pk in self._sup_plans.pop(name, []):
                self._release_plan(pk)
            buf = self._sup_cache[key] = torch.zeros(numel, device=self.device, dtype=dtype)
        return buf

    def _release_plan(self, key):
        p = self._plans.pop(key, None)
        if p is None or any(q.get("blocks") is p["blocks"] for q in self._plans.values()):
            return
        for gk in [gk for gk, gv in self._geom_specs.items() if gv[0] is p["blocks"]]:
            del self._geom_specs[gk]

    def _stream_level2(self, lay, plans, bufs, run, d):
        dtype, esize = torch.float16, 2
        H, W, n1, k3, Ht2, W2, h2s = lay.H, lay.W, lay.n1, lay.k3, lay.Ht2, lay.W2, lay.h2s
        pw, cat = plans["pw"], bufs["cat"]
        nb = pw["blocks"][n1]
        C1, C2 = nb.conv1.cin, nb.conv1.cout
        ps2 = self._plan_eval(2, 2 * h2s, W, dtype, partial=True)
        pt2 = self._plan_eval(lay.n_strip2, 2 * Ht2, W, dtype, partial=True)
        streams_ready = False
        if run is None:
            cat2 = pw.get("l2cat")
            if cat2 is None or cat2.numel() != lay.rows2 * C2:
                cat2 = pw["l2cat"] = torch.zeros(lay.rows2 * C2, device=self.device, dtype=dtype)
        elif run.cat2 is not None:
            cat2, streams_ready = run.cat2, True
        else:
            cat2 = run.cat2 = self._sup_buffer("l2", lay.rows2 * C2, dtype, (run.S, run.B_max, H, W))
            ps2 = self._plan_eval(2, 2 * h2s, W, dtype, partial=True, owner="l2")
        bufs["cat2"] = cat2
        out_t2 = cat2[:(lay.n_strip2 * lay.img_t2 + W2 + 2) * C2]
        if lay.n_strip2 < lay.n_strip2_max:
            cat2[lay.n_strip2 * lay.img_t2 * C2:(lay.n_strip2 * lay.img_t2 + W2 + 2) * C2].zero_()

        def rest_of_level(p, b, L, n_img, fused, final_out):
            y = final_out if k3 == n1 + 1 else L[2]
            self._conv_eval_f16(b.conv2, b.bn2, L[0], L[1], y, n_img, 1)
            if k3 > n1 + 1:
                self._eval_blocks(True, p, p["blocks"][n1 + 1:k3], y, n_img, fused, lay.rides[n1 + 1:k3], final_out=final_out)

        if not streams_ready:
            Ls, bs = ps2["lv"][(h2s, W2)], ps2["blocks"][n1]
            for phase in (0, 1):
                src = ctypes.c_void_p(cat.data_ptr() + (lay.stream_row0 + phase * (W + 1)) * C1 * esize)
                off = phase * lay.img_s2 * C2 * esize
                self._s2_plain_f16(bs, src, (ctypes.c_void_p(Ls[0].data_ptr() + off), ctypes.c_void_p(Ls[1].data_ptr() + off)),
                                   1, lay.stream_rows, W, lay.rides[n1])
            rest_of_level(ps2, bs, Ls, 2, lay.stream2_fused, cat2[lay.stream2_base * C2:])
        Lt, bt = pt2["lv"][(Ht2, W2)], pt2["blocks"][n1]
        wmap = (lay.B, H, W, lay.band, lay.Ht, H - lay.Ht, lay.stream_row0 + d * (W + 1), 1, 0, lay.cat_rows, Ht2)
        self._s2_mapped_f16(bt, cat, Lt, wmap, lay.rides[n1], lay.strips2_resident)
        rest_of_level(pt2, bt, Lt, lay.n_strip2, lay.strip2_fused, out_t2)

    def _stream_tail(self, lay, plans, bufs, d, probs_out):
        half, B, H, W, n1 = lay.half, lay.B, lay.H, lay.W, lay.n1
        pw = plans["pw"]
        blocks = pw["blocks"]
        fused, ride = lay.window_fused, lay.rides
        if lay.mode == "assembled":
            cur = pw["lv"][(H, W)][0]
            _hip.check(self.lib().lad_assemble_windows(_hip.ptr(bufs["stream"]), _hip.ptr(bufs["strips"]), _hip.ptr(cur), B, H, W, lay.band,
                                                       self.stem_cout * (2 if half else 4), self._st()), "lad_assemble_windows")
            cur = self._eval_blocks(half, pw, blocks[n1:], cur, B, fused[n1:], ride[n1:])
            return self._eval_tail(half, pw, cur, B, probs_out)
        if lay.mode == "direct":
            k, src = n1, bufs["cat"]
            wmap = (B, H, W, lay.band, lay.Ht, H - lay.Ht, lay.stream_row0, 1, 0, lay.cat_rows, 0)
        else:
            k, src = lay.k3, bufs["cat2"]
            wmap = (B, lay.H2, lay.W2, lay.band2, lay.Ht2, lay.shift2, lay.stream2_base + (d // 2) * (lay.W2 + 1), 2, lay.img_s2, lay.rows2, 0)
            if lay.tail_fused:
                probs = probs_out if probs_out is not None else pw["probs"]
                label = "tail_f16"
                t0 = self._mark(label)
                rc = self.lib().lad_f16_tail_fwd(_hip.ptr(src), *wmap[:-1], self._tail_params(blocks[k:]), self._head_params, pw["feat"],
                                                 _hip.ptr(probs), self._st())
                if rc != _hip.LAD_NOT_COVERED:
                    _hip.check(rc, "lad_f16_tail_fwd")
                    self._mark_end(label, t0)
                    return probs
        b = blocks[k]
        L = pw["lv"][(b.conv1.h_out, b.conv1.w_out)]
        if lay.mode == "direct" and not ride[k]:
            def one(cs, bn, slot, relu):
                _hip.check(self.lib().lad_f16_conv_s2_fwd_windows(_hip.ptr(src), *self._f16_args(cs, bn), _hip.ptr(L[slot]), B, H, W, lay.band,
                                                                  cs.cin, cs.cout, cs.taps, relu, self._st()),
                           "lad_f16_conv_s2_fwd_windows " + cs.name)
            self._s2_entry_f16(b, one, None, False)
        else:
            self._s2_mapped_f16(b, src, L, wmap, ride[k])
        self._conv_eval_f16(b.conv2, b.bn2, L[0], L[1], L[2], B, 1)
        cur = self._eval_blocks(half, pw, blocks[k + 1:], L[2], B, fused[k + 1:], ride[k + 1:])
        return self._eval_tail(half, pw, cur, B, probs_out)

    def _stream_super_cap(self, F):
        free, _ = torch.cuda.mem_get_info(self.device)
        free += torch.cuda.memory_reserved(self.device) - torch.cuda.memory_allocated(self.device)
        held = sum(b.numel() * b.element_size() for b in self._sup_cache.values())
        per_frame = 2 * (6 * (F + 1) * self.stem_cout + 5 * ((F + 1) // 2 + 1) * 32)
        return max(0, int(0.5 * (free + held)) // per_frame)

    def _tail_params(self, tail):
        if self._tail_ptrs is None:
            ptrs = []
            for b in tail:
                for cs, bn in ((b.conv1, b.bn1),) + (((b.sc_conv, b.sc_bn),) if b.sc_conv is not None else ()) + ((b.conv2, b.bn2),):
                    ptrs += [cs.par.wt_h.data_ptr(), bn.fold[0].data_ptr(), bn.fold[1].data_ptr()]
            self._tail_ptrs = (_VP * len(ptrs))(*ptrs)
        return self._tail_ptrs

    def predict_windows(self, feats, n_frames=100, chunk=None, start=0, stop=None, out=None, precision="fp32", stream=True):
        if precision not in ("fp32", "fp16"):
            raise ValueError("precision must be 'fp32' or 'fp16'")
        half = precision == "fp16"
        if half:
            self._require_half()
        chunk = PREDICT_CHUNK[precision] if chunk is None else chunk
        self.ensure_flat()
        _hip.require_cuda(feats, "feats", torch.float32)
        if feats.dim() != 2:
            raise ValueError("feats must be (T, F)")
        T, F = feats.shape
        stop = T if stop is None else min(stop, T)
        n = max(0, stop - start)
        if out is None:
            out = torch.empty(n, device=feats.device, dtype=torch.float32)
        elif out.dim() != 1 or out.numel() < n:
            raise ValueError(f"out must be a vector of at least {n} elements (one per window of [start, stop))")
        flat = feats.view(-1)
        i = start
        direct = out.dtype == torch.float32 and out.is_contiguous() and out.device == feats.device
        use_runs = half and stream and self.stream_super and chunk % 2 == 0 and stop - start > chunk
        run = None
        while i < stop:
            B = min(chunk, stop - i)
            dst = out[i - start:i - start + B]
            if use_runs and (run is None or i >= run.i0 + run.S):
                S = min(stop - i, max(chunk, min(STREAM_SUPER_MAX, self._stream_super_cap(F)) // chunk * chunk))
                run = _StreamRun(i, S, min(chunk, S), flat.data_ptr() + 4 * i * F, T - i)
            if stream:
                probs = self._forward_eval_stream(half, flat, B, n_frames, F, frames_avail=T - i, feat_offset_floats=i * F, run=run,
                                                  d=0 if run is None else i - run.i0, probs_out=dst if direct else None)
            else:
                probs = self._forward_eval_any(half, flat, B, n_frames, F, 1, frames_avail=T - i, feat_offset_floats=i * F,
                                               probs_out=dst if direct else None)
            if not direct:
                dst.copy_(probs[:B])
            i += B
        return out

    def _bn_bwd(self, p, bn, dy, y, x, coef, dx, B, h, w, relu, mode=0, aux=None, sbn=None, xs=None, scoef=None, pre=False):
        _hip.check(self.lib().lad_bn_bwd(
            _hip.ptr(dy), _hip.ptr(y), _hip.ptr(x), _hip.ptr(coef), _hip.ptr(bn.g), _hip.ptr(xs), _hip.ptr(scoef),
            _hip.ptr(sbn.g) if sbn is not None else None, _hip.ptr(dx), _hip.ptr(aux), _hip.ptr(bn.gg), _hip.ptr(bn.gb),
            _hip.ptr(sbn.gg) if sbn is not None else None, _hip.ptr(sbn.gb) if sbn is not None else None,
            _hip.ptr(p["bn_ws"]), _hip.ptr(p["bcoef"]), _hip.ptr(p["partials"]) if pre else None,
            int(self.lib().lad_conv_num_tiles(B, h, w)) if pre else 0, B, h, w, bn.c, relu, mode, self._st()), "lad_bn_bwd " + bn.name)

    def _side_stream(self):
        if self._side is None or self._side.device != self.device:
            self._side = torch.cuda.Stream(self.device)
        return self._side

    def _on_side(self, launch, read_buffer, small=False):
        if not (self.overlap_wgrad or (small and self._overlap_small_on())):
            launch(self._st())
            return
        side = self._side_stream()
        side.wait_stream(torch.cuda.current_stream(self.device))
        launch(ctypes.c_void_p(side.cuda_stream))
        ev = torch.cuda.Event()
        ev.record(side)
        self._side_readers[read_buffer.data_ptr()] = ev
        self._side_pending = True

    def _overlap_small_on(self):
        if self.overlap_wgrad_small != "auto":
            return bool(self.overlap_wgrad_small)
        p = getattr(self, "_last_train_plan", None)
        return p is not None and p["saved"][4] >= 256

    def _w(self, buf):
        ev = self._side_readers.pop(buf.data_ptr(), None)
        if ev is not None:
            torch.cuda.current_stream(self.device).wait_event(ev)
        return buf

    def _join_side(self):
        if self._side_pending:
            torch.cuda.current_stream(self.device).wait_stream(self._side)
            self._side_pending = False
            self._side_readers.clear()

    def _wg_ws(self, p, cs):
        return p["wgrad_ws_of"][cs.name] if self._defer_on else p["wgrad_ws"]

    def _conv_wgrad(self, p, cs, kind, x, dout, B, *, in_coef=None, bn=None):
        fn = conv_wgrad_entry(kind, in_coef is not None, bn is not None)
        lib, P, h, w, ws = self.lib(), _hip.ptr, cs.h_in, cs.w_in, self._wg_ws(p, cs)
        if bn is not None:
            dy, bx, bits, coef = bn
            _hip.check(lib.lad_conv_wgrad_h2_bnbwd(P(x), P(in_coef), P(dy), P(bx), P(bits), P(coef), P(p["bcoef"]), P(dout), P(ws), P(cs.par.gw),
                                                   P(cs.par.gb), B, h, w, cs.cin, self._st()), f"{fn} {cs.name}")
        elif kind == "f32":
            self._on_side(lambda st: _hip.check(lib.lad_conv_wgrad(P(x), P(dout), P(ws), P(cs.par.gw), P(cs.par.gb), B, h, w, cs.cin, cs.cout, cs.taps, st),
                                                f"{fn} {cs.name}"), dout, small=cs.cin <= 32)
        else:
            self._on_side(lambda st: _hip.check(getattr(lib, fn)(P(x), P(in_coef), P(dout), P(ws), P(cs.par.gw), P(cs.par.gb), B, h, w, cs.cin, st),
                                                f"{fn} {cs.name}"), dout, small=cs.cin <= 32)

    def backward(self, dprobs=None):
        try:
            self._backward(dprobs)
        except BaseException:
            if self._defer_on:
                self._defer_on = False
                self.lib().lad_wgrad_defer_begin()
                self.lib().lad_wgrad_defer_flush(None)
            raise

    def _backward(self, dprobs):
        p = getattr(self, "_last_train_plan", None)
        if p is None or "saved" not in p:
            raise _hip.LadHipError("backward() without a preceding train-mode forward()")
        x, labels, m1, m2, B, H, W = p["saved"]
        if dprobs is None and labels is None:
            raise _hip.LadHipError("backward() needs dprobs or labels passed to forward()")
        lib, st = self.lib(), self._st()
        blocks, acts, sched = p["blocks"], p["acts"], p["schedule"]
        last = blocks[-1].conv2
        self._defer_on = self.defer_wgrad_sums and not self.overlap_wgrad
        if self._defer_on:
            _hip.check(lib.lad_wgrad_defer_begin(), "lad_wgrad_defer_begin")
        _hip.check(lib.lad_head_bwd(self._head_params, self._head_grads, _hip.ptr(p["pooled"]), _hip.ptr(p["h"]),
                                    _hip.ptr(p["hstats"]), _hip.ptr(p["probs"]), _hip.ptr(dprobs), B, p["feat"], _hip.ptr(m1),
                                    _hip.ptr(m2), _hip.ptr(labels), _hip.ptr(p["head_ws"]), _hip.ptr(p["dpooled"]), st),
                   "lad_head_bwd")
        g_out = p["g"][(last.h_out, last.w_out)]
        dy = g_out[0]
        _hip.check(lib.lad_pool_bwd(_hip.ptr(p["dpooled"]), _hip.ptr(dy), B, p["h4"], p["w4"], last.cout, st), "lad_pool_bwd")
        pre2 = False
        pre2_tiles = 0
        for bi in range(len(blocks) - 1, -1, -1):
            b, a, ch = blocks[bi], acts[bi], sched.blocks[bi]
            c1s, c2s = b.conv1, b.conv2
            ho, wo, co = c1s.h_out, c1s.w_out, c1s.cout
            hi, wi = c1s.h_in, c1s.w_in
            G = p["g"][(ho, wo)]
            free = [t for t in G if t is not dy]
            aux, da1 = (self._w(a["aux"]) if "aux" in a else free[0]), free[1]
            dc2, dc1 = self._w(a["dc2"]), self._w(a["dc1"])
            bits = a["ybits"] if ch.bits else None
            lower = acts[bi - 1]
            fuse2 = ch.bits and ch.conv2.wgrad_bn and not self.overlap_wgrad
            fuse1 = ch.conv1.wgrad_bn and not self.overlap_wgrad
            if ch.bits:
                _hip.check(lib.lad_bn_bwd_bits(_hip.ptr(dy), _hip.ptr(bits), _hip.ptr(a["c2"]), _hip.ptr(a["coef2"]), _hip.ptr(b.bn2.g),
                                               None if fuse2 else _hip.ptr(dc2), _hip.ptr(b.bn2.gg), _hip.ptr(b.bn2.gb), _hip.ptr(p["bn_ws"]),
                                               _hip.ptr(p["bcoef"]), _hip.ptr(p["partials"]) if pre2 else None,
                                               (pre2_tiles or int(lib.lad_conv_num_tiles(B, ho, wo))) if pre2 else 0, B, ho, wo, co, st),
                           "lad_bn_bwd_bits " + b.bn2.name)
            elif b.sc_conv is None:
                self._bn_bwd(p, b.bn2, dy, a["y"], a["c2"], a["coef2"], dc2, B, ho, wo, 1, mode=1, aux=aux, pre=pre2)
            else:
                self._bn_bwd(p, b.bn2, dy, a["y"], a["c2"], a["coef2"], dc2, B, ho, wo, 1, mode=2, aux=aux,
                             sbn=b.sc_bn, xs=a["cs"], scoef=a["coefs"])
            xin, xcoef = (a["c1"], a["coef1"]) if ch.a1_virtual else (a["a1"], None)
            self._conv_wgrad(p, c2s, ch.conv2.wgrad, xin, dc2, B, in_coef=xcoef, bn=(dy, a["c2"], bits, a["coef2"]) if fuse2 else None)
            stat = (a["c1"], None, a["coef1"]) if ch.dgrad2_bn else None
            self._conv_s1(c2s, "f32" if ch.dgrad2_bn == "f32" else ch.conv2.arith, "dgrad", dc2, da1, B, ch.conv2.label_dgrad,
                          bn=stat, partials=p["partials"] if stat else None)
            self._bn_bwd(p, b.bn1, da1, None, a["c1"], a["coef1"], None if fuse1 else dc1, B, ho, wo, 2, mode=0, pre=stat is not None)
            if c1s.stride == 1:
                self._conv_wgrad(p, c1s, ch.conv1.wgrad, a["x"], dc1, B, bn=(da1, a["c1"], None, a["coef1"]) if fuse1 else None)
            if self.debug_capture is not None:
                self.debug_capture[b.name] = {"dy": dy.clone(), "dc2": dc2.clone(), "aux": aux.clone() if bits is None else None, "da1": da1.clone(),
                                              "dc1": dc1.clone()}
            if c1s.stride == 1:
                dx = dy
                if b.sc_conv is not None:
                    self._conv_wgrad(p, b.sc_conv, ch.sc.wgrad, a["x"], aux, B)
                    self._conv_s1(b.sc_conv, ch.sc.arith, "dgrad", aux, da1, B)
                    aux = da1
                stat = (lower["c2"], lower["ybits" if ch.dgrad1_bn == "split" else "y"], lower["coef2"]) if ch.dgrad1_bn else None
                self._conv_s1(c1s, "f32" if ch.dgrad1_bn == "f32" else ch.conv1.arith, "dgrad", dc1, dx, B, ch.conv1.label_dgrad,
                              addend=dy if ch.bits else aux, abits=bits, bn=stat, partials=p["partials"] if stat else None)
                pre2, pre2_tiles = stat is not None, 0
            else:
                dx = p["g"][(hi, wi)][0]
                sc = b.sc_conv

                def s2_wgrad(cs, dout, xin=a["x"]):
                    self._on_side(lambda sst: _hip.check(lib.lad_conv_s2_wgrad(
                        _hip.ptr(xin), _hip.ptr(dout), _hip.ptr(self._wg_ws(p, cs)), _hip.ptr(cs.par.gw), _hip.ptr(cs.par.gb), B, hi, wi, cs.cin, cs.cout,
                        cs.taps, sst), "lad_conv_s2_wgrad " + cs.name), dout, small=cs.cin <= 32)

                if ch.sc_wgrad_fused:
                    self._on_side(lambda sst, c1s=c1s, sc=sc, dc1=dc1, aux=aux, xin=a["x"]: _hip.check(lib.lad_conv_s2_wgrad_fused(
                        _hip.ptr(xin), _hip.ptr(dc1), _hip.ptr(aux), _hip.ptr(self._wg_ws(p, c1s)), _hip.ptr(c1s.par.gw), _hip.ptr(c1s.par.gb),
                        _hip.ptr(sc.par.gw), B, hi, wi, c1s.cin, c1s.cout, sst), "lad_conv_s2_wgrad_fused " + c1s.name), dc1, small=c1s.cin <= 32)
                    if dc1.data_ptr() in self._side_readers:
                        self._side_readers[aux.data_ptr()] = self._side_readers[dc1.data_ptr()]
                else:
                    s2_wgrad(c1s, dc1)
                stat = (lower["c2"], lower["ybits"], lower["coef2"]) if ch.dgrad1_bn else (None, None, None)
                n_part = 0
                if ch.entry == "s2b3":
                    n_part = int(lib.lad_conv_s2b3_dgrad_partials(B, hi, wi))
                    assert not ch.dgrad1_bn or n_part * 2 * 64 <= p["partials"].numel()
                    _hip.check(lib.lad_conv_s2b3_dgrad(_hip.ptr(dc1), _hip.ptr(aux), _hip.ptr(c1s.par.wt3_s2d), _hip.ptr(dx),
                                                       _hip.ptr(p["partials"]) if ch.dgrad1_bn else None, _hip.ptr(stat[0]), _hip.ptr(stat[1]),
                                                       _hip.ptr(stat[2]), B, hi, wi, st), "lad_conv_s2b3_dgrad " + c1s.name)
                elif ch.entry == "s2_fused" and ch.dgrad1_bn:
                    n_part = int(lib.lad_conv_s2_dgrad_partials(B, hi, wi))
                    assert n_part * 2 * 64 <= p["partials"].numel()
                    _hip.check(lib.lad_conv_s2_dgrad_fused_bnstat(_hip.ptr(dc1), _hip.ptr(c1s.par.wt_d), _hip.ptr(aux), _hip.ptr(sc.par.wt_d), _hip.ptr(dx),
                                                                  _hip.ptr(p["partials"]), _hip.ptr(stat[0]), _hip.ptr(stat[1]),
                                                                  _hip.ptr(stat[2]), B, hi, wi, c1s.cin, c1s.cout, st),
                               "lad_conv_s2_dgrad_fused_bnstat " + c1s.name)
                elif ch.entry == "s2_fused":
                    _hip.check(lib.lad_conv_s2_dgrad_fused(_hip.ptr(dc1), _hip.ptr(c1s.par.wt_d), _hip.ptr(aux), _hip.ptr(sc.par.wt_d), _hip.ptr(dx),
                                                           B, hi, wi, c1s.cin, c1s.cout, st), "lad_conv_s2_dgrad_fused " + c1s.name)
                else:
                    _hip.check(lib.lad_conv_s2_dgrad(_hip.ptr(dc1), _hip.ptr(c1s.par.wt_d), _hip.ptr(dx), B, hi, wi, c1s.cin, c1s.cout, 9, 0,
                                                     st), "lad_conv_s2_dgrad " + c1s.name)
                pre2, pre2_tiles = ch.dgrad1_bn is not None, n_part
                if not ch.sc_wgrad_fused:
                    s2_wgrad(sc, aux)
                if ch.entry == "plain":
                    _hip.check(lib.lad_conv_s2_dgrad(_hip.ptr(aux), _hip.ptr(sc.par.wt_d), _hip.ptr(dx), B, hi, wi, sc.cin, sc.cout, 1, 1, st),
                               "lad_conv_s2_dgrad " + sc.name)
            dy = dx
        if sched.stem_onepass:
            bn = self.stem_bn
            _hip.check(lib.lad_stem_bwd_onepass(_hip.ptr(x), _hip.ptr(self.stem_w), _hip.ptr(dy), _hip.ptr(p["stem_coef"]), _hip.ptr(bn.g),
                                                _hip.ptr(p["stem_mom"]), _hip.ptr(p["stem_bwd_ws"]), _hip.ptr(self.stem_gw), _hip.ptr(bn.gg),
                                                _hip.ptr(bn.gb), B, H, W, self.stem_cout, st), "lad_stem_bwd_onepass")
        else:
            groups = int(lib.lad_stem_bn_bwd_groups(B, H, W))
            _hip.check(lib.lad_stem_bn_bwd_sums(_hip.ptr(x), _hip.ptr(self.stem_w), _hip.ptr(dy), _hip.ptr(p["stem_coef"]),
                                                _hip.ptr(p["partials"]), B, H, W, self.stem_cout, st), "lad_stem_bn_bwd_sums")
            bn = self.stem_bn
            _hip.check(lib.lad_bn_bwd(_hip.ptr(dy), None, None, _hip.ptr(p["stem_coef"]), _hip.ptr(bn.g), None, None, None, None,
                                      None, _hip.ptr(bn.gg), _hip.ptr(bn.gb), None, None, _hip.ptr(p["bn_ws"]), _hip.ptr(p["bcoef"]),
                                      _hip.ptr(p["partials"]), groups, B, H, W, bn.c, 2, 0, st), "lad_bn_bwd " + bn.name)
            self._on_side(lambda sst: _hip.check(lib.lad_stem_wgrad_bn(_hip.ptr(x), _hip.ptr(dy), None, _hip.ptr(self.stem_w),
                                                                       _hip.ptr(p["stem_coef"]), _hip.ptr(p["bcoef"]),
                                                                       _hip.ptr(p["wgrad_ws"]), _hip.ptr(self.stem_gw), B, H, W,
                                                                       self.stem_cout, sst), "lad_stem_wgrad_bn"), dy)
        if self._defer_on:
            self._defer_on = False
            self._join_side()
            _hip.check(lib.lad_wgrad_defer_flush(st), "lad_wgrad_defer_flush")
        self._join_side()
        self._grad_dirty = True

    def export_relu_masks(self):
        p = getattr(self, "_last_train_plan", None)
        if p is None or "saved" not in p:
            raise _hip.LadHipError("export_relu_masks() without a preceding train-mode forward()")
        x, labels, m1, m2, B, H, W = p["saved"]

        def unpack(buf, h, w, c):
            body = buf[:B * (h + 1) * (w + 1) * c].view(B, h + 1, w + 1, c)[:, 1:, 1:, :]
            return (body > 0).permute(0, 3, 1, 2).cpu()

        out = {"stem": unpack(p["stem_a"], H, W, self.stem_cout)}
        for b, ch, a in zip(p["blocks"], p["schedule"].blocks, p["acts"]):
            ho, wo, co = b.conv1.h_out, b.conv1.w_out, b.conv1.cout
            if ch.a1_virtual:
                c = a["c1"][:B * (ho + 1) * (wo + 1) * co].view(B, ho + 1, wo + 1, co)[:, 1:, 1:, :].double()
                sc, sh = a["coef1"][:co].double(), a["coef1"][co:2 * co].double()
                out[b.name + ".a1"] = (c * sc + sh > 0).permute(0, 3, 1, 2).cpu()
            else:
                out[b.name + ".a1"] = unpack(a["a1"], ho, wo, co)
            out[b.name + ".y"] = unpack(a["y"], ho, wo, co)
        h = p["h"].view(B, 32).double()
        mean, var = h.mean(0), h.var(0, unbiased=False)
        u = (h - mean) / torch.sqrt(var + 1e-5) * self.head_bn3.g.double() + self.head_bn3.b.double()
        if m2 is not None:
            u = u * m2.double()
        out["head"] = (u > 0).cpu()
        return out

    def reset_optimizer(self):
        self.ensure_flat()
        self._exp_avg.zero_()
        self._exp_avg_sq.zero_()
        self._step_dev.zero_()
        self._step_count = 0

    def reset_dropout_rng(self):
        self.ensure_flat()
        self._rng_counter.zero_()

    def flat_grad(self):
        self.ensure_flat()
        return self._flat_g

    def flat_param(self):
        self.ensure_flat()
        return self._flat_p

    def accumulated_grad(self):
        self.ensure_flat()
        if getattr(self, "_acc_g", None) is None:
            self._acc_g = torch.zeros_like(self._flat_g)
        return self._acc_g

    def accumulate_grad(self, scale):
        acc = self.accumulated_grad()
        _hip.check(self.lib().lad_grad_accumulate(_hip.ptr(acc), _hip.ptr(self._flat_g), self._n_flat, float(scale), self._st()),
                   "lad_grad_accumulate")
        return acc

    def clip_and_step(self, lr=1e-3, betas=(0.9, 0.999), eps=1e-8, max_norm=1.0, grad_scale=1.0, zero_grad=True, grad=None):
        self.ensure_flat()
        lib, st = self.lib(), self._st()
        g = self._flat_g if grad is None else grad
        if g.numel() != self._n_flat or g.dtype != torch.float32 or not g.is_cuda:
            raise _hip.LadHipError("clip_and_step: grad must be a float32 GPU buffer of the flat parameter size")
        self._step_count += 1
        _hip.check(lib.lad_grad_sumsq(_hip.ptr(g), self._n_flat, _hip.ptr(self._norm_partials), _hip.ptr(self._step_dev), st),
                   "lad_grad_sumsq")
        _hip.check(lib.lad_adam_step(_hip.ptr(self._flat_p), _hip.ptr(g), _hip.ptr(self._exp_avg),
                                     _hip.ptr(self._exp_avg_sq), self._n_flat, _hip.ptr(self._norm_partials), float(grad_scale),
                                     float(max_norm if max_norm is not None else 0.0), float(lr), float(betas[0]), float(betas[1]),
                                     float(eps), self._step_count, _hip.ptr(self._step_dev), 1 if zero_grad else 0,
                                     _hip.ptr(self._norm_out), st), "lad_adam_step")
        self.notify_weights_changed()
        if zero_grad:
            self._grad_dirty = False
        return self._norm_out

    def optimizer_state(self):
        self.ensure_flat()
        return [self._flat_p, self._flat_g, self._exp_avg, self._exp_avg_sq, self._step_dev]

    def eval_metrics(self, probs, labels, out=None):
        _hip.require_cuda(probs, "probs", torch.float32)
        _hip.require_cuda(labels, "labels", torch.int32)
        if out is None:
            out = torch.zeros(8, device=probs.device)
        _hip.check(self.lib().lad_bce_metrics(_hip.ptr(probs), _hip.ptr(labels), probs.numel(), _hip.ptr(out), self._st()),
                   "lad_bce_metrics")
        return out

    def metrics(self):
        return self._last_train_plan["metrics"]


def dropout_masks(B, feat, rate, device, generator=None):
    if rate <= 0.0:
        return None
    keep = 1.0 - rate
    m1 = torch.empty((B, feat), device=device).bernoulli_(keep, generator=generator).div_(keep)
    m2 = torch.empty((B, 32), device=device).bernoulli_(keep, generator=generator).div_(keep)
    return m1, m2


def metrics_from_counters(m):
    loss, corr, pp, tp, tt, n = [float(v) for v in m[:6]]
    acc = corr / n if n else float("nan")
    prec = 1.0 if pp == 0 else tp / pp
    rec = tp / tt if tt != 0 else float("nan")
    return loss, acc, prec, rec
```

Before: 50020 segments/s.

## Parallelize classifier head across workgroups with fused pooling and last-block reductions

Adds a multi-workgroup version of the MLP head forward and backward. Each workgroup handles 64 samples, writes partial BN/metric sums, and a last-arriving workgroup (atomic ticket) finalizes the statistics. The new kernels also fold average pooling into the forward and unpooling into the backward. This replaces the previous head kernels, which appear to run on few workgroups, and removes separate pool launches, at the cost of more launches and the ticket synchronization.

```diff
diff --git a/include/lad_hip.h b/include/lad_hip.h
--- a/include/lad_hip.h
+++ b/include/lad_hip.h
@@ -235,6 +235,16 @@
                  const float *stats, const float *probs, const float *dprobs, int64_t batch, int32_t F,
                  const float *drop1, const float *drop2, const int32_t *labels, float *workspace, float *dpooled,
                  void *stream);
+int64_t lad_head_par_workgroups(int64_t batch);
+int64_t lad_head_par_workspace_floats(int64_t batch, int32_t F);
+int lad_head_fwd_train_par(const float *const *params, const float *x, float *pooled, int64_t batch, int32_t H, int32_t W,
+                           int32_t channels, int32_t F, float *drop1, float *drop2, float keep, uint64_t seed,
+                           int64_t *rng_counter, int64_t *nbt, int32_t n_nbt, const int32_t *labels, float momentum, float *h,
+                           float *stats, float *probs, float *metrics, float *workspace, void *stream);
+int lad_head_bwd_par(const float *const *params, float *const *grads, const float *pooled, const float *h,
+                     const float *stats, const float *probs, const float *dprobs, int64_t batch, int32_t F,
+                     const float *drop1, const float *drop2, const int32_t *labels, float *workspace, float *dpooled,
+                     float *dx, int32_t H, int32_t W, int32_t channels, void *stream);
 
 int64_t lad_f16_packed_weight_halfs(int32_t cout, int32_t cin, int32_t taps);
 int lad_f16_pack_weights(const float *w, int32_t cout, int32_t cin, int32_t taps, void *wt, void *stream);
diff --git a/laughter-detection-icsi_amd/_hip.py b/laughter-detection-icsi_amd/_hip.py
--- a/laughter-detection-icsi_amd/_hip.py
+++ b/laughter-detection-icsi_amd/_hip.py
@@ -131,6 +131,11 @@
     "lad_head_fwd_eval": (c_int, [c_void_p, c_void_p, c_i64, c_i32, c_void_p, c_void_p]),
     "lad_bce_metrics": (c_int, [c_void_p, c_void_p, c_i64, c_void_p, c_void_p]),
     "lad_head_bwd": (c_int, [c_void_p] * 7 + [c_i64, c_i32] + [c_void_p] * 6),
+    "lad_head_par_workgroups": (c_i64, [c_i64]),
+    "lad_head_par_workspace_floats": (c_i64, [c_i64, c_i32]),
+    "lad_head_fwd_train_par": (c_int, [c_void_p, c_void_p, c_void_p, c_i64, c_i32, c_i32, c_i32, c_i32, c_void_p, c_void_p, c_float,
+                                       ctypes.c_uint64, c_void_p, c_void_p, c_i32, c_void_p, c_float] + [c_void_p] * 6),
+    "lad_head_bwd_par": (c_int, [c_void_p] * 7 + [c_i64, c_i32] + [c_void_p] * 6 + [c_i32, c_i32, c_i32, c_void_p]),
     "lad_f16_packed_weight_halfs": (c_i64, [c_i32, c_i32, c_i32]),
     "lad_f16_pack_weights": (c_int, [c_void_p, c_i32, c_i32, c_i32, c_void_p, c_void_p]),
     "lad_f16_stem_fwd": (c_int, [c_void_p] * 5 + [c_i64, c_i32, c_i32, c_i32, c_i64, c_i64, c_void_p]),
diff --git a/laughter-detection-icsi_amd/csrc/head.hip b/laughter-detection-icsi_amd/csrc/head.hip
--- a/laughter-detection-icsi_amd/csrc/head.hip
+++ b/laughter-detection-icsi_amd/csrc/head.hip
@@ -600,6 +600,624 @@
     LAD_HEAD_STAMP(25)
 }
 
+constexpr int SPW = 64;
+constexpr int PAR_THREADS = 256;
+constexpr int POOL_SPW = 8;
+constexpr int POOL_THREADS = 512;
+constexpr int BWD_OUT_COLS = 3 * HID;
+constexpr int BWD_OUT_STRIDE = 128;
+
+struct ParWs {
+    double *p1, *p2, *p3, *q1, *q2;
+    float *du, *dz, *dh, *z, *dl;
+};
+__host__ __device__ inline int64_t par_workgroups(int64_t B) { return (B + SPW - 1) / SPW; }
+__host__ __device__ inline int64_t pool_workgroups(int64_t B) { return (B + POOL_SPW - 1) / POOL_SPW; }
+inline int64_t par_ws_doubles(int64_t B, int F) {
+    return pool_workgroups(B) * 2 * F + par_workgroups(B) * (2 * HID + 8 + BWD_OUT_STRIDE + HID + 2 * F);
+}
+inline ParWs carve(float *ws, int64_t B, int F) {
+    const int64_t nwg = par_workgroups(B);
+    ParWs w;
+    w.p1 = reinterpret_cast<double *>(ws);
+    w.p2 = w.p1 + pool_workgroups(B) * 2 * F;
+    w.p3 = w.p2 + nwg * 2 * HID;
+    w.q1 = w.p3 + nwg * 8;
+    w.q2 = w.q1 + nwg * BWD_OUT_STRIDE;
+    w.du = reinterpret_cast<float *>(w.q2 + nwg * (HID + 2 * F));
+    w.dz = w.du + B * HID;
+    w.dh = reinterpret_cast<float *>((reinterpret_cast<uintptr_t>(w.dz + B * F) + 15) & ~(uintptr_t)15);
+    w.z = w.dh + B * HID;
+    w.dl = w.z + B * F;
+    return w;
+}
+
+__device__ __forceinline__ bool last_workgroup(unsigned int *ticket) {
+    __shared__ int last_s;
+    asm volatile("s_waitcnt vmcnt(0)" ::: "memory");
+    __syncthreads();
+    if (threadIdx.x == 0) last_s = __hip_atomic_fetch_add(ticket, 1u, __ATOMIC_RELAXED, __HIP_MEMORY_SCOPE_AGENT) == gridDim.x - 1;
+    __syncthreads();
+    const bool last = last_s != 0;
+    if (last && threadIdx.x == 0) __hip_atomic_store(ticket, 0u, __ATOMIC_RELAXED, __HIP_MEMORY_SCOPE_AGENT);
+    return last;
+}
+
+template <int UN = 8, typename T>
+__device__ __forceinline__ double sum_parts(const T *p, int n, int64_t stride) {
+    double t = 0.0;
+    int w = 0;
+    for (; w + UN <= n; w += UN) {
+        T v[UN];
+#pragma unroll
+        for (int u = 0; u < UN; ++u) v[u] = __hip_atomic_load(p + (w + u) * stride, __ATOMIC_RELAXED, __HIP_MEMORY_SCOPE_AGENT);
+#pragma unroll
+        for (int u = 0; u < UN; ++u) t += (double)v[u];
+    }
+    for (; w + 8 <= n; w += 8) {
+        T v[8];
+#pragma unroll
+        for (int u = 0; u < 8; ++u) v[u] = __hip_atomic_load(p + (w + u) * stride, __ATOMIC_RELAXED, __HIP_MEMORY_SCOPE_AGENT);
+#pragma unroll
+        for (int u = 0; u < 8; ++u) t += (double)v[u];
+    }
+    for (; w < n; ++w) t += (double)__hip_atomic_load(p + w * stride, __ATOMIC_RELAXED, __HIP_MEMORY_SCOPE_AGENT);
+    return t;
+}
+
+template <int UN, typename Get>
+__device__ __forceinline__ double wg_col_sum(int nb, int ncol, double *scratch, Get get) {
+    const int tid = threadIdx.x, nph = min(8, (int)blockDim.x / ncol);
+    const int c = tid % ncol, ph = tid / ncol;
+    if (ph < nph) {
+        double s = 0.0;
+        for (int r0 = ph; r0 < nb; r0 += UN * nph) {
+            double v[UN];
+#pragma unroll
+            for (int u = 0; u < UN; ++u) {
+                const int r = r0 + u * nph;
+                v[u] = r < nb ? get(r, c) : 0.0;
+            }
+#pragma unroll
+            for (int u = 0; u < UN; ++u) s += v[u];
+        }
+        scratch[tid] = s;
+    }
+    __syncthreads();
+    double t = 0.0;
+    if (tid < ncol)
+        for (int q = 0; q < nph; ++q) t += scratch[q * ncol + tid];
+    __syncthreads();
+    return t;
+}
+
+__device__ __forceinline__ void bn1d_finish(double s1, double s2, int B, float *mean_o, float *istd_o, float *rmean, float *rvar,
+                                            float momentum) {
+    const double mean = s1 / B;
+    double var = s2 / B - mean * mean;
+    if (var < 0.0) var = 0.0;
+    *mean_o = (float)mean;
+    *istd_o = (float)(1.0 / sqrt(var + (double)BN_EPS));
+    if (rmean != nullptr) {
+        const double unb = B > 1 ? var * B / (B - 1.0) : var;
+        *rmean = (1.f - momentum) * *rmean + momentum * (float)mean;
+        *rvar = (1.f - momentum) * *rvar + momentum * (float)unb;
+    }
+}
+
+__global__ __launch_bounds__(POOL_THREADS) void head_par_pool_kernel(HeadArgs a, const float *__restrict__ x, float *pooled, int Hp, int Wp,
+                                                                      int C, int PH, int PW, float *__restrict__ stats, double *part,
+                                                                      unsigned int *ticket) {
+    __shared__ float pl[POOL_SPW * MAX_F];
+    __shared__ double tot[POOL_THREADS];
+    const int tid = threadIdx.x, nt = blockDim.x;
+    const int B = a.B, F = a.F, b0 = blockIdx.x * POOL_SPW, nb = min(POOL_SPW, B - b0);
+    constexpr int NV = POOL_SPW * MAX_F / POOL_THREADS;
+    if (x != nullptr) {
+        float win[NV][16];
+#pragma unroll
+        for (int k = 0; k < NV; ++k) {
+            const int idx = tid + k * nt;
+            if (idx < nb * F) {
+                const int bl = idx / F, f = idx - bl * F;
+                const int c = f / (PH * PW), ph = (f / PW) % PH, pw = f % PW;
+                const float *img = x + (int64_t)(b0 + bl) * Hp * Wp * C;
+#pragma unroll
+                for (int dy = 0; dy < 4; ++dy)
+#pragma unroll
+                    for (int dx = 0; dx < 4; ++dx) win[k][dy * 4 + dx] = img[((1 + 4 * ph + dy) * Wp + (1 + 4 * pw + dx)) * C + c];
+            }
+        }
+#pragma unroll
+        for (int k = 0; k < NV; ++k) {
+            const int idx = tid + k * nt;
+            if (idx < nb * F) {
+                float s = 0.f;
+#pragma unroll
+                for (int e = 0; e < 16; ++e) s += win[k][e];
+                const float v = s * 0.0625f;
+                pooled[(int64_t)b0 * F + idx] = v;
+                pl[idx] = v;
+            }
+        }
+    } else {
+#pragma unroll
+        for (int k = 0; k < NV; ++k) {
+            const int idx = tid + k * nt;
+            if (idx < nb * F) pl[idx] = pooled[(int64_t)b0 * F + idx];
+        }
+    }
+    __syncthreads();
+    {
+        const double s = wg_col_sum<8>(nb, 2 * F, tot, [&](int r, int c) {
+            const double v = (double)pl[r * F + (c < F ? c : c - F)];
+            return c < F ? v : v * v;
+        });
+        if (tid < 2 * F) __hip_atomic_store(part + (int64_t)blockIdx.x * 2 * F + tid, s, __ATOMIC_RELAXED, __HIP_MEMORY_SCOPE_AGENT);
+    }
+    if (!last_workgroup(ticket)) return;
+    if (tid < 2 * F) tot[tid] = sum_parts<32>(part + tid, (int)gridDim.x, 2 * F);
+    __syncthreads();
+    if (tid < F) bn1d_finish(tot[tid], tot[F + tid], B, stats + tid, stats + F + tid, a.rm2 + tid, a.rv2 + tid, a.momentum);
+}
+
+__global__ __launch_bounds__(PAR_THREADS) void head_par_linear1_kernel(HeadArgs a, const float *__restrict__ pooled, float *__restrict__ h,
+                                                                        float *stats, double *part, unsigned int *ticket) {
+    __shared__ float zs[MAX_F], zt[MAX_F];
+    __shared__ __attribute__((aligned(16))) float w1t[MAX_F * HID];
+    __shared__ float b1s[HID];
+    __shared__ float hs[SPW * (HID + 1)];
+    __shared__ float ps[SPW * (MAX_F + 1)];
+    __shared__ double tot[PAR_THREADS];
+    static_assert(PAR_THREADS == 4 * SPW && HID == 32, "four waves of a workgroup share its 64 samples, eight hidden units each");
+    constexpr int JQ = HID / 4;
+    const int tid = threadIdx.x, nt = blockDim.x;
+    const int B = a.B, F = a.F, b0 = blockIdx.x * SPW, nb = min(SPW, B - b0);
+    const float *mean2 = stats, *istd2 = stats + F;
+    batched<8, float>(tid, F * HID, nt, [&](int i) { return a.W1[i]; },
+                      [&](int i, float v) {
+                          const int j = i / F, f = i - j * F;
+                          w1t[f * HID + j] = v;
+                      });
+    for (int f = tid; f < F; f += nt) {
+        const float s = istd2[f] * a.g2[f];
+        zs[f] = s;
+        zt[f] = a.b2[f] - mean2[f] * s;
+    }
+    if (tid < HID) b1s[tid] = a.bias1[tid];
+    batched<12, float>(tid, nb * F, nt, [&](int idx) { return pooled[(int64_t)b0 * F + idx]; },
+                       [&](int idx, float v) {
+                           const int bl = idx / F;
+                           ps[bl * (MAX_F + 1) + idx - bl * F] = v;
+                       });
+    const bool rng = a.rng_counter != nullptr;
+    const long long draw = rng ? *a.rng_counter : 0;
+    __syncthreads();
+    const int sl = tid & (SPW - 1), q = tid / SPW, b = b0 + sl;
+    if (b < B) {
+        float acc[JQ];
+#pragma unroll
+        for (int j = 0; j < JQ; ++j) acc[j] = b1s[q * JQ + j];
+        const float *pr = ps + sl * (MAX_F + 1);
+        const float *mr = a.m1 ? a.m1 + (int64_t)b * F : nullptr;
+        for (int f0 = 0; f0 < F; f0 += 8) {
+            float pv[8], mv[8];
+#pragma unroll
+            for (int k = 0; k < 8; ++k) pv[k] = f0 + k < F ? pr[f0 + k] : 0.f;
+            if (rng) {
+                const unsigned g0 = (unsigned)(((int64_t)b * F + f0) >> 2);
+                const float4 ma = dropout_mask4(a.seed, draw, 0, g0, a.keep);
+                const float4 mb = f0 + 4 < F ? dropout_mask4(a.seed, draw, 0, g0 + 1, a.keep) : make_float4(1.f, 1.f, 1.f, 1.f);
+                mv[0] = ma.x; mv[1] = ma.y; mv[2] = ma.z; mv[3] = ma.w;
+                mv[4] = mb.x; mv[5] = mb.y; mv[6] = mb.z; mv[7] = mb.w;
+                if (q == 0) {
+                    float4 *o1 = reinterpret_cast<float4 *>(const_cast<float *>(a.m1));
+                    o1[g0] = ma;
+                    if (f0 + 4 < F) o1[g0 + 1] = mb;
+                }
+            } else {
+#pragma unroll
+                for (int k = 0; k < 8; ++k) mv[k] = (mr != nullptr && f0 + k < F) ? mr[f0 + k] : 1.f;
+            }
+#pragma unroll
+            for (int k = 0; k < 8; ++k) {
+                const int f = f0 + k;
+                if (f < F) {
+                    float z = fmaf(pv[k], zs[f], zt[f]);
+                    if (mr != nullptr) z *= mv[k];
+#pragma unroll
+                    for (int j = 0; j < JQ; ++j) acc[j] = fmaf(w1t[f * HID + q * JQ + j], z, acc[j]);
+                }
+            }
+        }
+        float4 *hr = reinterpret_cast<float4 *>(h + (int64_t)b * HID + q * JQ);
+        hr[0] = make_float4(acc[0], acc[1], acc[2], acc[3]);
+        hr[1] = make_float4(acc[4], acc[5], acc[6], acc[7]);
+#pragma unroll
+        for (int j = 0; j < JQ; ++j) hs[sl * (HID + 1) + q * JQ + j] = acc[j];
+        if (rng) {
+            float4 *o2 = reinterpret_cast<float4 *>(const_cast<float *>(a.m2));
+            const unsigned g = (unsigned)(b * (HID / 4) + 2 * q);
+            o2[g] = dropout_mask4(a.seed, draw, 1, g, a.keep);
+            o2[g + 1] = dropout_mask4(a.seed, draw, 1, g + 1, a.keep);
+        }
+    }
+    __syncthreads();
+    {
+        const double s = wg_col_sum<8>(nb, 2 * HID, tot, [&](int r, int c) {
+            const double v = (double)hs[r * (HID + 1) + (c & (HID - 1))];
+            return c < HID ? v : v * v;
+        });
+        if (tid < 2 * HID) __hip_atomic_store(part + (int64_t)blockIdx.x * 2 * HID + tid, s, __ATOMIC_RELAXED, __HIP_MEMORY_SCOPE_AGENT);
+    }
+    if (!last_workgroup(ticket)) return;
+    if (tid < 2 * HID) tot[tid] = sum_parts(part + tid, (int)gridDim.x, 2 * HID);
+    __syncthreads();
+    if (tid < HID)
+        bn1d_finish(tot[tid], tot[HID + tid], B, stats + 2 * F + tid, stats + 2 * F + HID + tid, a.rm3 + tid, a.rv3 + tid, a.momentum);
+}
+
+__global__ __launch_bounds__(SPW) void head_par_out_kernel(HeadArgs a, const float *__restrict__ h, const float *__restrict__ stats,
+                                                            float *__restrict__ probs, float *__restrict__ metrics, double *part,
+                                                            unsigned int *ticket) {
+    __shared__ float us[HID], ut[HID], w2s[HID];
+    const int tid = threadIdx.x;
+    const int B = a.B, F = a.F, b = blockIdx.x * SPW + tid;
+    const float *mean3 = stats + 2 * F, *istd3 = stats + 2 * F + HID;
+    if (tid < HID) {
+        const float s = istd3[tid] * a.g3[tid];
+        us[tid] = s;
+        ut[tid] = a.b3[tid] - mean3[tid] * s;
+        w2s[tid] = a.W2[tid];
+    }
+    __syncthreads();
+    float loss = 0.f, n_corr = 0.f, n_pp = 0.f, n_tp = 0.f, n_t = 0.f;
+    const float bias2 = a.bias2[0];
+    if (b < B) {
+        float part_j[HID], mk[HID];
+        const float4 *hr = reinterpret_cast<const float4 *>(h + (int64_t)b * HID);
+        const float4 *mr = a.m2 ? reinterpret_cast<const float4 *>(a.m2 + (int64_t)b * HID) : nullptr;
+#pragma unroll
+        for (int q = 0; q < HID / 4; ++q) {
+            const float4 hv = hr[q];
+            part_j[4 * q] = hv.x; part_j[4 * q + 1] = hv.y; part_j[4 * q + 2] = hv.z; part_j[4 * q + 3] = hv.w;
+            if (mr != nullptr) {
+                const float4 mv = mr[q];
+                mk[4 * q] = mv.x; mk[4 * q + 1] = mv.y; mk[4 * q + 2] = mv.z; mk[4 * q + 3] = mv.w;
+            }
+        }
+        const float t = a.labels != nullptr ? (float)a.labels[b] : 0.f;
+#pragma unroll
+        for (int j = 0; j < HID; ++j) {
+            float u = fmaf(part_j[j], us[j], ut[j]);
+            if (mr != nullptr) u *= mk[j];
+            part_j[j] = w2s[j] * fmaxf(u, 0.f);
+        }
+#pragma unroll
+        for (int off = HID / 2; off > 0; off >>= 1)
+#pragma unroll
+            for (int j = 0; j < off; ++j) part_j[j] += part_j[j + off];
+        const float p = sigmoidf(part_j[0] + bias2);
+        probs[b] = p;
+        if (a.labels != nullptr) {
+            const float lp = fmaxf(logf(p), -100.f), l1p = fmaxf(logf(1.f - p), -100.f);
+            loss -= t * lp + (1.f - t) * l1p;
+            const float pred = rintf(p);
+            n_corr += (pred == t) ? 1.f : 0.f;
+            n_pp += pred;
+            n_tp += (pred == 1.f && t == 1.f) ? 1.f : 0.f;
+            n_t += t;
+        }
+    }
+    const float vals[5] = {loss, n_corr, n_pp, n_tp, n_t};
+#pragma unroll
+    for (int k = 0; k < 5; ++k) {
+        const float v = wave_sum64(vals[k]);
+        if (tid == k) __hip_atomic_store(part + (int64_t)blockIdx.x * 8 + k, (double)v, __ATOMIC_RELAXED, __HIP_MEMORY_SCOPE_AGENT);
+    }
+    if (!last_workgroup(ticket)) return;
+    if (tid < 5) {
+        float s = 0.f;
+        batched<8, double>(0, (int)gridDim.x, 1,
+                           [&](int w) { return __hip_atomic_load(part + (int64_t)w * 8 + tid, __ATOMIC_RELAXED, __HIP_MEMORY_SCOPE_AGENT); },
+                           [&](int, double v) { s += (float)v; });
+        metrics[tid] = (tid == 0) ? s / (float)B : s;
+    }
+    if (tid == 5) metrics[5] = (float)B;
+    if (a.rng_counter != nullptr && tid == 6) *a.rng_counter += 1;
+    if (a.nbt != nullptr)
+        for (int i = tid; i < a.n_nbt; i += SPW) a.nbt[i] += 1;
+}
+
+__global__ __launch_bounds__(PAR_THREADS) void head_par_bwd_out_kernel(HeadArgs a, HeadGrads gr_out, const float *__restrict__ h,
+                                                                        const float *__restrict__ stats, const float *__restrict__ probs,
+                                                                        const float *__restrict__ dprobs, float *__restrict__ du,
+                                                                        float *dl, double *part, unsigned int *ticket) {
+    __shared__ float us[HID], ut[HID], w2s[HID];
+    __shared__ float gr_s[SPW * (HID + 1)], du_s[SPW * (HID + 1)], xh_s[SPW * (HID + 1)], dl_s[HID];
+    __shared__ double tot[PAR_THREADS];
+    const int tid = threadIdx.x;
+    const int B = a.B, F = a.F, b0 = blockIdx.x * SPW, nb = min(SPW, B - b0);
+    const float *mean3 = stats + 2 * F, *istd3 = stats + 2 * F + HID;
+    if (tid < HID) {
+        const float s = istd3[tid] * a.g3[tid];
+        us[tid] = s;
+        ut[tid] = a.b3[tid] - mean3[tid] * s;
+        w2s[tid] = a.W2[tid];
+    }
+    const int j = tid & (HID - 1);
+    const float mean3_j = mean3[j], istd3_j = istd3[j];
+    __syncthreads();
+#pragma unroll
+    for (int k = 0; k < SPW * HID / PAR_THREADS; ++k) {
+        const int bl = (tid + k * PAR_THREADS) >> 5, b = b0 + bl;
+        if (b < B) {
+            const int64_t idx = (int64_t)b * HID + j;
+            const float p = probs[b], t = dprobs != nullptr ? dprobs[b] : (float)a.labels[b], hv = h[idx], m = a.m2 ? a.m2[idx] : 1.f;
+            float dlogit;
+            if (dprobs != nullptr) dlogit = t * p * (1.f - p);
+            else dlogit = (p - t) / (float)B;
+            if (j == 0) __hip_atomic_store(dl + b, dlogit, __ATOMIC_RELAXED, __HIP_MEMORY_SCOPE_AGENT);
+            float u = fmaf(hv, us[j], ut[j]);
+            u *= m;
+            const float duv = (u > 0.f) ? dlogit * w2s[j] * m : 0.f;
+            du[idx] = duv;
+            gr_s[bl * (HID + 1) + j] = dlogit * fmaxf(u, 0.f);
+            du_s[bl * (HID + 1) + j] = duv;
+            xh_s[bl * (HID + 1) + j] = (hv - mean3_j) * istd3_j;
+        }
+    }
+    __syncthreads();
+    {
+        const double s = wg_col_sum<8>(nb, BWD_OUT_COLS, tot, [&](int r, int c) {
+            const int what = c >> 5, i = r * (HID + 1) + (c & (HID - 1));
+            return what == 0 ? (double)gr_s[i] : what == 1 ? (double)du_s[i] : (double)du_s[i] * (double)xh_s[i];
+        });
+        if (tid < BWD_OUT_COLS)
+            __hip_atomic_store(part + (int64_t)blockIdx.x * BWD_OUT_STRIDE + tid, s, __ATOMIC_RELAXED, __HIP_MEMORY_SCOPE_AGENT);
+    }
+    if (!last_workgroup(ticket)) return;
+    if (tid < BWD_OUT_COLS) {
+        const float s = (float)sum_parts(part + tid, (int)gridDim.x, BWD_OUT_STRIDE);
+        const int what = tid >> 5;
+        if (what == 0) gr_out.dW2[j] = s;
+        else if (what == 1) gr_out.db3[j] = s;
+        else gr_out.dg3[j] = s;
+    }
+    if (tid < HID) {
+        float sm = 0.f;
+        batched<8, float>(tid, B, HID, [&](int b) { return __hip_atomic_load(dl + b, __ATOMIC_RELAXED, __HIP_MEMORY_SCOPE_AGENT); },
+                          [&](int, float v) { sm += v; });
+        dl_s[tid] = sm;
+    }
+    __syncthreads();
+    if (tid == 0) {
+        float sm = 0.f;
+        for (int w = 0; w < HID / 2; ++w) sm += dl_s[2 * w] + dl_s[2 * w + 1];
+        gr_out.dbias2[0] = sm;
+    }
+}
+
+__global__ __launch_bounds__(PAR_THREADS) void head_par_bwd_hidden_kernel(HeadArgs a, HeadGrads gr_out, const float *__restrict__ pooled,
+                                                                           const float *__restrict__ h, const float *__restrict__ stats,
+                                                                           const float *__restrict__ du, float *__restrict__ dz,
+                                                                           float *__restrict__ dhg, float *__restrict__ zg, double *part,
+                                                                           unsigned int *ticket) {
+    __shared__ float zs[MAX_F], zt[MAX_F], mu2[MAX_F], is2[MAX_F];
+    __shared__ __attribute__((aligned(16))) float w1t[MAX_F * HID];
+    __shared__ __attribute__((aligned(16))) float z_s[SPW * (MAX_F + 1)];
+    constexpr int DHS = HID + 4;
+    __shared__ __attribute__((aligned(16))) float dh_s[SPW * DHS];
+    __shared__ double tot[PAR_THREADS];
+    const int tid = threadIdx.x, nt = blockDim.x;
+    const int B = a.B, F = a.F, b0 = blockIdx.x * SPW, nb = min(SPW, B - b0);
+    const float *mean2 = stats, *istd2 = stats + F, *mean3 = stats + 2 * F, *istd3 = stats + 2 * F + HID;
+    const int ncol = HID + 2 * F;
+    batched<8, float>(tid, F * HID, nt, [&](int i) { return a.W1[i]; },
+                      [&](int i, float v) {
+                          const int j = i / F, f = i - j * F;
+                          w1t[f * HID + j] = v;
+                      });
+    for (int f = tid; f < F; f += nt) {
+        const float s = istd2[f] * a.g2[f];
+        zs[f] = s;
+        zt[f] = a.b2[f] - mean2[f] * s;
+        mu2[f] = mean2[f];
+        is2[f] = istd2[f];
+    }
+    constexpr int NZ = SPW * MAX_F / PAR_THREADS;
+    F2 pz[NZ];
+#pragma unroll
+    for (int k = 0; k < NZ; ++k) {
+        const int idx = tid + k * nt;
+        if (idx < nb * F) pz[k] = F2{pooled[(int64_t)b0 * F + idx], a.m1 ? a.m1[(int64_t)b0 * F + idx] : 1.f};
+    }
+    const int jt = tid & (HID - 1);
+    const float mean3_j = mean3[jt], istd3_j = istd3[jt], k3_j = a.g3[jt] * istd3[jt];
+    {
+        const float ca_j = gr_out.db3[jt] / (float)B, cb_j = gr_out.dg3[jt];
+#pragma unroll
+        for (int k = 0; k < SPW * HID / PAR_THREADS; ++k) {
+            const int bl = (tid + k * PAR_THREADS) >> 5, b = b0 + bl;
+            if (b < B) {
+                const int64_t idx = (int64_t)b * HID + jt;
+                const float hv = h[idx], dv = du[idx];
+                const float xh = (hv - mean3_j) * istd3_j;
+                const float dhv = k3_j * (dv - ca_j - xh * cb_j / (float)B);
+                dh_s[bl * DHS + jt] = dhv;
+                dhg[idx] = dhv;
+            }
+        }
+    }
+    __syncthreads();
+#pragma unroll
+    for (int k = 0; k < NZ; ++k) {
+        const int idx = tid + k * nt;
+        if (idx < nb * F) {
+            const int bl = idx / F, f = idx - bl * F;
+            float z = fmaf(pz[k].a, zs[f], zt[f]);
+            if (a.m1) z *= pz[k].b;
+            z_s[bl * (MAX_F + 1) + f] = z;
+            zg[(int64_t)b0 * F + idx] = z;
+        }
+    }
+    __syncthreads();
+    {
+        const double s = wg_col_sum<8>(nb, HID, tot, [&](int r, int c) { return (double)dh_s[r * DHS + c]; });
+        if (tid < HID) __hip_atomic_store(part + (int64_t)blockIdx.x * ncol + tid, s, __ATOMIC_RELAXED, __HIP_MEMORY_SCOPE_AGENT);
+    }
+    __syncthreads();
+    if (tid < 2 * nb) {
+        const int fh = (F + 1) / 2;
+        const int bl = tid >> 1, b = b0 + bl, fa = (tid & 1) * fh, fb = min(F, fa + fh);
+        float dhr[HID];
+#pragma unroll
+        for (int j = 0; j < HID; j += 4) {
+            const float4 v = *reinterpret_cast<const float4 *>(dh_s + bl * DHS + j);
+            dhr[j] = v.x; dhr[j + 1] = v.y; dhr[j + 2] = v.z; dhr[j + 3] = v.w;
+        }
+        const float *mr = a.m1 ? a.m1 + (int64_t)b * F : nullptr;
+        float *zr = dz + (int64_t)b * F;
+        for (int f0 = fa; f0 < fb; f0 += 8) {
+            float mv[8];
+#pragma unroll
+            for (int k = 0; k < 8; ++k) mv[k] = (mr != nullptr && f0 + k < fb) ? mr[f0 + k] : 1.f;
+#pragma unroll
+            for (int k = 0; k < 8; ++k) {
+                const int f = f0 + k;
+                if (f < fb) {
+                    float sacc = 0.f;
+#pragma unroll
+                    for (int j = 0; j < HID; ++j) sacc = fmaf(w1t[f * HID + j], dhr[j], sacc);
+                    if (mr != nullptr) sacc *= mv[k];
+                    zr[f] = sacc;
+                    z_s[bl * (MAX_F + 1) + f] = sacc;
+                }
+            }
+        }
+    }
+    __syncthreads();
+    {
+        const double s = wg_col_sum<16>(nb, 2 * F, tot, [&](int r, int cc) {
+            const int c = cc < F ? cc : cc - F;
+            const double v = (double)z_s[r * (MAX_F + 1) + c];
+            return cc < F ? v : v * (double)((pooled[(int64_t)(b0 + r) * F + c] - mu2[c]) * is2[c]);
+        });
+        if (tid < 2 * F) __hip_atomic_store(part + (int64_t)blockIdx.x * ncol + HID + tid, s, __ATOMIC_RELAXED, __HIP_MEMORY_SCOPE_AGENT);
+    }
+    if (!last_workgroup(ticket)) return;
+    for (int i = tid; i < ncol; i += nt) {
+        const float s = (float)sum_parts(part + i, (int)gridDim.x, ncol);
+        if (i < HID) gr_out.dbias1[i] = s;
+        else if (i < HID + F) gr_out.db2[i - HID] = s;
+        else gr_out.dg2[i - HID - F] = s;
+    }
+}
+
+__device__ __forceinline__ void dw1_workgroup(int B, int F, int KS, int wg, const float *__restrict__ dh, const float *__restrict__ z,
+                                              float *__restrict__ dW1) {
+    constexpr int TJ = 4, TF = 3, UN = 16;
+    __shared__ float part[PAR_THREADS * TJ * TF];
+    const int tid = threadIdx.x, tpw = PAR_THREADS / KS;
+    const int ftiles = (F + TF - 1) / TF, ntile = (HID / TJ) * ftiles;
+    const int tl = tid % tpw, g = tid / tpw, tile = wg * tpw + tl;
+    const int tj = tile / ftiles, tf = tile - tj * ftiles;
+    float wacc[TJ][TF];
+#pragma unroll
+    for (int x = 0; x < TJ; ++x)
+#pragma unroll
+        for (int y = 0; y < TF; ++y) wacc[x][y] = 0.f;
+    if (tile < ntile) {
+        for (int b0 = g; b0 < B; b0 += KS * UN) {
+            float4 dv[UN];
+            float zz[UN][TF];
+#pragma unroll
+            for (int u = 0; u < UN; ++u) {
+                const int b = b0 + u * KS;
+                if (b < B) {
+                    dv[u] = *reinterpret_cast<const float4 *>(dh + (int64_t)b * HID + tj * TJ);
+#pragma unroll
+                    for (int y = 0; y < TF; ++y) zz[u][y] = z[(int64_t)b * F + min(tf * TF + y, F - 1)];
+                }
+            }
+#pragma unroll
+            for (int u = 0; u < UN; ++u) {
+                if (b0 + u * KS < B) {
+                    const float dd[TJ] = {dv[u].x, dv[u].y, dv[u].z, dv[u].w};
+#pragma unroll
+                    for (int x = 0; x < TJ; ++x)
+#pragma unroll
+                        for (int y = 0; y < TF; ++y) wacc[x][y] = fmaf(dd[x], zz[u][y], wacc[x][y]);
+                }
+            }
+        }
+    }
+#pragma unroll
+    for (int x = 0; x < TJ; ++x)
+#pragma unroll
+        for (int y = 0; y < TF; ++y) part[(g * tpw + tl) * TJ * TF + x * TF + y] = wacc[x][y];
+    __syncthreads();
+    for (int o = tid; o < tpw * TJ * TF; o += PAR_THREADS) {
+        const int tl2 = o / (TJ * TF), e = o - tl2 * TJ * TF, tile2 = wg * tpw + tl2;
+        const int tj2 = tile2 / ftiles, f = (tile2 - tj2 * ftiles) * TF + e % TF;
+        if (tile2 < ntile && f < F) {
+            float sacc = part[o];
+            for (int q = 1; q < KS; ++q) sacc += part[q * tpw * TJ * TF + o];
+            dW1[(tj2 * TJ + e / TF) * F + f] = sacc;
+        }
+    }
+}
+
+__global__ __launch_bounds__(PAR_THREADS) void head_par_bwd_in_kernel(HeadArgs a, HeadGrads gr_out, const float *__restrict__ pooled,
+                                                                       const float *__restrict__ stats, const float *__restrict__ dz,
+                                                                       float *__restrict__ dpooled, const float *__restrict__ dh,
+                                                                       const float *__restrict__ z, int KS, int ndw) {
+    const int B = a.B, F = a.F;
+    if ((int)blockIdx.x < ndw) {
+        dw1_workgroup(B, F, KS, (int)blockIdx.x, dh, z, gr_out.dW1);
+        return;
+    }
+    const int64_t idx = (int64_t)(blockIdx.x - ndw) * blockDim.x + threadIdx.x;
+    if (idx >= (int64_t)B * F) return;
+    const int f = (int)(idx % F);
+    const float is = stats[F + f], kk = a.g2[f] * is;
+    const float xh = (pooled[idx] - stats[f]) * is;
+    dpooled[idx] = kk * (dz[idx] - gr_out.db2[f] / (float)B - xh * gr_out.dg2[f] / (float)B);
+}
+
+__global__ __launch_bounds__(PAR_THREADS) void head_par_bwd_unpool_kernel(HeadArgs a, HeadGrads gr_out, const float *__restrict__ pooled,
+                                                                           const float *__restrict__ stats, const float *__restrict__ dz,
+                                                                           float *__restrict__ dpooled, float *__restrict__ dx, int Hp, int Wp,
+                                                                           int C, int PH, int PW, const float *__restrict__ dh,
+                                                                           const float *__restrict__ z, int KS, int ndw) {
+    const int B = a.B, F = a.F;
+    if ((int)blockIdx.x < ndw) {
+        dw1_workgroup(B, F, KS, (int)blockIdx.x, dh, z, gr_out.dW1);
+        return;
+    }
+    const int64_t total = (int64_t)B * Hp * Wp * C;
+    for (int64_t idx = (int64_t)(blockIdx.x - ndw) * blockDim.x + threadIdx.x; idx < total; idx += (int64_t)(gridDim.x - ndw) * blockDim.x) {
+        const int c = (int)(idx % C);
+        int64_t t = idx / C;
+        const int xp = (int)(t % Wp);
+        t /= Wp;
+        const int yp = (int)(t % Hp);
+        const int64_t b = t / Hp;
+        float v = 0.f;
+        const int y = yp - 1, xx = xp - 1;
+        if (y >= 0 && y < 4 * PH && xx >= 0 && xx < 4 * PW) {
+            const int f = c * PH * PW + (y >> 2) * PW + (xx >> 2);
+            const int64_t i = b * F + f;
+            const float is = stats[F + f], kk = a.g2[f] * is;
+            const float xh = (pooled[i] - stats[f]) * is;
+            const float d = kk * (dz[i] - gr_out.db2[f] / (float)B - xh * gr_out.dg2[f] / (float)B);
+            if (((y | xx) & 3) == 0) dpooled[i] = d;
+            v = d * 0.0625f;
+        }
+        dx[idx] = v;
+    }
+}
+
 int check_head(const HeadArgs &a) {
     using namespace lad;
     LAD_REQUIRE(a.B >= 1 && a.F >= 1 && a.F <= MAX_F, "head: F must be 1..%d (got %d), B >= 1", MAX_F, a.F);
@@ -714,6 +1332,95 @@
     return check_launch("head_bwd_kernel");
 }
 
+extern "C" int64_t lad_head_par_workgroups(int64_t batch) { return batch > 0 ? par_workgroups(batch) : 0; }
+
+extern "C" int64_t lad_head_par_workspace_floats(int64_t batch, int32_t F) {
+    if (batch <= 0 || F <= 0) return 0;
+    return 2 * par_ws_doubles(batch, F) + batch * (2 * (HID + F) + 1) + 4;
+}
+
+extern "C" int lad_head_fwd_train_par(const float *const *params, const float *x, float *pooled, int64_t batch, int32_t H, int32_t W,
+                                      int32_t channels, int32_t F, float *drop1, float *drop2, float keep, uint64_t seed,
+                                      int64_t *rng_counter, int64_t *nbt, int32_t n_nbt, const int32_t *labels, float momentum, float *h,
+                                      float *stats, float *probs, float *metrics, float *workspace, void *stream) {
+    using namespace lad;
+    LAD_REQUIRE(params && pooled && h && stats && probs && metrics && workspace, "lad_head_fwd_train_par: null buffer");
+    LAD_REQUIRE(batch >= 1 && batch < (1 << 24), "lad_head_fwd_train_par: batch must be 1 .. 2^24 - 1");
+    LAD_REQUIRE((reinterpret_cast<uintptr_t>(workspace) & 7) == 0, "lad_head_fwd_train_par: workspace must be 8-byte aligned");
+    LAD_REQUIRE(n_nbt >= 0 && (n_nbt == 0 || nbt), "lad_head_fwd_train_par: bad counter list");
+    const bool rng = rng_counter != nullptr && keep < 1.0f;
+    LAD_REQUIRE(!rng || (keep > 0.f && drop1 && drop2 && F % 4 == 0 && batch >= 2),
+                "lad_head_fwd_train_par: drawing masks needs both mask buffers, F %% 4 == 0 and two samples");
+    int PH = 0, PW = 0;
+    if (x != nullptr) {
+        LAD_REQUIRE(H >= 4 && W >= 4 && channels >= 1, "lad_head_fwd_train_par: AvgPool2d(4) needs H, W >= 4");
+        PH = H / 4; PW = W / 4;
+        LAD_REQUIRE((int64_t)channels * PH * PW == F, "lad_head_fwd_train_par: F must be channels * (H / 4) * (W / 4)");
+    }
+    HeadArgs a = make_args(params, batch, F, drop1, drop2, labels, momentum);
+    int rc = check_head(a);
+    if (rc) return rc;
+    a.keep = keep; a.seed = seed; a.rng_counter = rng ? (long long *)rng_counter : nullptr; a.nbt = (long long *)nbt; a.n_nbt = n_nbt;
+    const ParWs w = carve(workspace, batch, F);
+    const unsigned nwg = (unsigned)par_workgroups(batch);
+    unsigned int *t1 = launch_ticket(), *t2 = launch_ticket(), *t3 = launch_ticket();
+    LAD_REQUIRE(t1 && t2 && t3, "lad_head_fwd_train_par: no ticket");
+    hipLaunchKernelGGL(head_par_pool_kernel, dim3((unsigned)pool_workgroups(batch)), dim3(POOL_THREADS), 0, (hipStream_t)stream, a, x, pooled, H + 1, W + 1, channels, PH,
+                       PW, stats, w.p1, t1);
+    rc = check_launch("head_par_pool_kernel");
+    if (rc) return rc;
+    hipLaunchKernelGGL(head_par_linear1_kernel, dim3(nwg), dim3(PAR_THREADS), 0, (hipStream_t)stream, a, pooled, h, stats, w.p2, t2);
+    rc = check_launch("head_par_linear1_kernel");
+    if (rc) return rc;
+    hipLaunchKernelGGL(head_par_out_kernel, dim3(nwg), dim3(SPW), 0, (hipStream_t)stream, a, h, stats, probs, metrics, w.p3, t3);
+    return check_launch("head_par_out_kernel");
+}
+
+extern "C" int lad_head_bwd_par(const float *const *params, float *const *grads, const float *pooled, const float *h, const float *stats,
+                                const float *probs, const float *dprobs, int64_t batch, int32_t F, const float *drop1, const float *drop2,
+                                const int32_t *labels, float *workspace, float *dpooled, float *dx, int32_t H, int32_t W, int32_t channels,
+                                void *stream) {
+    using namespace lad;
+    LAD_REQUIRE(params && grads && pooled && h && stats && probs && workspace && dpooled, "lad_head_bwd_par: null buffer");
+    LAD_REQUIRE(dx == nullptr || (H >= 4 && W >= 4 && channels >= 1 && (int64_t)channels * (H / 4) * (W / 4) == F),
+                "lad_head_bwd_par: dx needs H, W >= 4 and F == channels * (H / 4) * (W / 4)");
+    LAD_REQUIRE(dprobs || labels, "lad_head_bwd_par: need dprobs or labels");
+    LAD_REQUIRE(batch >= 1 && batch < (1 << 24), "lad_head_bwd_par: batch must be 1 .. 2^24 - 1");
+    LAD_REQUIRE((reinterpret_cast<uintptr_t>(workspace) & 7) == 0, "lad_head_bwd_par: workspace must be 8-byte aligned");
+    HeadArgs a = make_args(params, batch, F, drop1, drop2, labels, 0.f);
+    int rc = check_head(a);
+    if (rc) return rc;
+    HeadGrads g;
+    g.dg2 = grads[0]; g.db2 = grads[1]; g.dW1 = grads[2]; g.dbias1 = grads[3];
+    g.dg3 = grads[4]; g.db3 = grads[5]; g.dW2 = grads[6]; g.dbias2 = grads[7];
+    const ParWs w = carve(workspace, batch, F);
+    const unsigned nwg = (unsigned)par_workgroups(batch);
+    unsigned int *t1 = launch_ticket(), *t2 = launch_ticket();
+    LAD_REQUIRE(t1 && t2, "lad_head_bwd_par: no ticket");
+    hipLaunchKernelGGL(head_par_bwd_out_kernel, dim3(nwg), dim3(PAR_THREADS), 0, (hipStream_t)stream, a, g, h, stats, probs, dprobs, w.du,
+                       w.dl, w.q1, t1);
+    rc = check_launch("head_par_bwd_out_kernel");
+    if (rc) return rc;
+    hipLaunchKernelGGL(head_par_bwd_hidden_kernel, dim3(nwg), dim3(PAR_THREADS), 0, (hipStream_t)stream, a, g, pooled, h, stats, w.du, w.dz,
+                       w.dh, w.z, w.q2, t2);
+    rc = check_launch("head_par_bwd_hidden_kernel");
+    if (rc) return rc;
+    const int ntile = (HID / 4) * ((F + 2) / 3);
+    int KS = 8;
+    while (KS > 1 && (ntile * KS > HEAD_THREADS || KS * HID * F > CH * (MAX_F + 1))) KS >>= 1;
+    const int ndw = (int)ceil_div(ntile, PAR_THREADS / KS);
+    if (dx != nullptr) {
+        const int64_t n = batch * (H + 1) * (W + 1) * channels;
+        hipLaunchKernelGGL(head_par_bwd_unpool_kernel, dim3((unsigned)std::min<int64_t>(ceil_div(n, (int64_t)PAR_THREADS), 4096) + ndw),
+                           dim3(PAR_THREADS), 0, (hipStream_t)stream, a, g, pooled, stats, w.dz, dpooled, dx, H + 1, W + 1, channels, H / 4,
+                           W / 4, w.dh, w.z, KS, ndw);
+        return check_launch("head_par_bwd_unpool_kernel");
+    }
+    hipLaunchKernelGGL(head_par_bwd_in_kernel, dim3((unsigned)ceil_div(batch * F, (int64_t)PAR_THREADS) + ndw), dim3(PAR_THREADS), 0,
+                       (hipStream_t)stream, a, g, pooled, stats, w.dz, dpooled, w.dh, w.z, KS, ndw);
+    return check_launch("head_par_bwd_in_kernel");
+}
+
 #ifdef LAD_STAMP
 extern "C" int lad_debug_read_head_stamps(unsigned long long *host_dst, int64_t n) {
     return hipMemcpyFromSymbol(host_dst, HIP_SYMBOL(lad_dbg_head), n * sizeof(unsigned long long)) == hipSuccess ? 0 : -2;
diff --git a/laughter-detection-icsi_amd/engine.py b/laughter-detection-icsi_amd/engine.py
--- a/laughter-detection-icsi_amd/engine.py
+++ b/laughter-detection-icsi_amd/engine.py
@@ -403,6 +403,7 @@
         self.fuse_s2_shortcut_wgrad = True
         self.defer_wgrad_sums = True
         self._defer_on = False
+        self.head_parallel = True
         self._schedules = {}
         self.relu_bits = True
         self._side = None
@@ -601,6 +602,7 @@
             p["hstats"] = torch.zeros(2 * feat + 64, device=dev)
             p["metrics"] = torch.zeros(8, device=dev)
             p["head_ws"] = torch.zeros(int(lib.lad_head_workspace_floats(B, feat)), device=dev)
+            p["head_pws"] = torch.zeros(int(lib.lad_head_par_workspace_floats(B, feat)), device=dev)
             p["dpooled"] = torch.zeros(B * feat, device=dev)
             levels = {}
             for b, d in zip(blocks, acts):
@@ -853,7 +855,9 @@
             a["x"] = cur
             cur = a["y"]
         last = blocks[-1].conv2
-        _hip.check(lib.lad_pool_fwd(_hip.ptr(cur), _hip.ptr(p["pooled"]), B, p["h4"], p["w4"], last.cout, st), "lad_pool_fwd")
+        par = bool(self.head_parallel) and int(lib.lad_head_par_workgroups(B)) > 1
+        if not par:
+            _hip.check(lib.lad_pool_fwd(_hip.ptr(cur), _hip.ptr(p["pooled"]), B, p["h4"], p["w4"], last.cout, st), "lad_pool_fwd")
         m1 = m2 = None
         rng = isinstance(drop_masks, str) and drop_masks == "rng"
         if drop_masks is not None and not rng:
@@ -877,15 +881,28 @@
             if seed != self._rng_seed:
                 self._rng_seed = seed
                 self._rng_counter.zero_()
-            _hip.check(lib.lad_head_fwd_train_rng(self._head_params, _hip.ptr(p["pooled"]), B, p["feat"], _hip.ptr(m1), _hip.ptr(m2), keep,
-                                                  seed, _hip.ptr(self._rng_counter), _hip.ptr(self._nbt), int(self._nbt.numel()),
-                                                  _hip.ptr(labels), 0.1, _hip.ptr(p["h"]), _hip.ptr(p["hstats"]), _hip.ptr(p["probs"]),
-                                                  _hip.ptr(p["metrics"]), st), "lad_head_fwd_train_rng")
+            if par:
+                _hip.check(lib.lad_head_fwd_train_par(self._head_params, _hip.ptr(cur), _hip.ptr(p["pooled"]), B, p["h4"], p["w4"], last.cout,
+                                                      p["feat"], _hip.ptr(m1), _hip.ptr(m2), keep, seed, _hip.ptr(self._rng_counter),
+                                                      _hip.ptr(self._nbt), int(self._nbt.numel()), _hip.ptr(labels), 0.1, _hip.ptr(p["h"]),
+                                                      _hip.ptr(p["hstats"]), _hip.ptr(p["probs"]), _hip.ptr(p["metrics"]),
+                                                      _hip.ptr(p["head_pws"]), st), "lad_head_fwd_train_par")
+            else:
+                _hip.check(lib.lad_head_fwd_train_rng(self._head_params, _hip.ptr(p["pooled"]), B, p["feat"], _hip.ptr(m1), _hip.ptr(m2), keep,
+                                                      seed, _hip.ptr(self._rng_counter), _hip.ptr(self._nbt), int(self._nbt.numel()),
+                                                      _hip.ptr(labels), 0.1, _hip.ptr(p["h"]), _hip.ptr(p["hstats"]), _hip.ptr(p["probs"]),
+                                                      _hip.ptr(p["metrics"]), st), "lad_head_fwd_train_rng")
+        elif par:
+            _hip.check(lib.lad_head_fwd_train_par(self._head_params, _hip.ptr(cur), _hip.ptr(p["pooled"]), B, p["h4"], p["w4"], last.cout,
+                                                  p["feat"], _hip.ptr(m1), _hip.ptr(m2), 1.0, 0, None, None, 0, _hip.ptr(labels), 0.1,
+                                                  _hip.ptr(p["h"]), _hip.ptr(p["hstats"]), _hip.ptr(p["probs"]), _hip.ptr(p["metrics"]),
+                                                  _hip.ptr(p["head_pws"]), st), "lad_head_fwd_train_par")
         else:
             _hip.check(lib.lad_head_fwd_train(self._head_params, _hip.ptr(p["pooled"]), B, p["feat"], _hip.ptr(m1), _hip.ptr(m2),
                                               _hip.ptr(labels), 0.1, _hip.ptr(p["h"]), _hip.ptr(p["hstats"]),
                                               _hip.ptr(p["probs"]), _hip.ptr(p["metrics"]), st), "lad_head_fwd_train")
         p["saved"] = (x, labels, m1, m2, B, H, W)
+        p["head_par"] = par
         self._last_train_plan = p
         self._train_forwards += 1
         return p["probs"]
@@ -1393,13 +1410,19 @@
         self._defer_on = self.defer_wgrad_sums and not self.overlap_wgrad
         if self._defer_on:
             _hip.check(lib.lad_wgrad_defer_begin(), "lad_wgrad_defer_begin")
-        _hip.check(lib.lad_head_bwd(self._head_params, self._head_grads, _hip.ptr(p["pooled"]), _hip.ptr(p["h"]),
-                                    _hip.ptr(p["hstats"]), _hip.ptr(p["probs"]), _hip.ptr(dprobs), B, p["feat"], _hip.ptr(m1),
-                                    _hip.ptr(m2), _hip.ptr(labels), _hip.ptr(p["head_ws"]), _hip.ptr(p["dpooled"]), st),
-                   "lad_head_bwd")
         g_out = p["g"][(last.h_out, last.w_out)]
         dy = g_out[0]
-        _hip.check(lib.lad_pool_bwd(_hip.ptr(p["dpooled"]), _hip.ptr(dy), B, p["h4"], p["w4"], last.cout, st), "lad_pool_bwd")
+        if p.get("head_par"):
+            _hip.check(lib.lad_head_bwd_par(self._head_params, self._head_grads, _hip.ptr(p["pooled"]), _hip.ptr(p["h"]),
+                                            _hip.ptr(p["hstats"]), _hip.ptr(p["probs"]), _hip.ptr(dprobs), B, p["feat"], _hip.ptr(m1),
+                                            _hip.ptr(m2), _hip.ptr(labels), _hip.ptr(p["head_pws"]), _hip.ptr(p["dpooled"]),
+                                            _hip.ptr(dy), p["h4"], p["w4"], last.cout, st), "lad_head_bwd_par")
+        else:
+            _hip.check(lib.lad_head_bwd(self._head_params, self._head_grads, _hip.ptr(p["pooled"]), _hip.ptr(p["h"]),
+                                        _hip.ptr(p["hstats"]), _hip.ptr(p["probs"]), _hip.ptr(dprobs), B, p["feat"], _hip.ptr(m1),
+                                        _hip.ptr(m2), _hip.ptr(labels), _hip.ptr(p["head_ws"]), _hip.ptr(p["dpooled"]), st),
+                       "lad_head_bwd")
+            _hip.check(lib.lad_pool_bwd(_hip.ptr(p["dpooled"]), _hip.ptr(dy), B, p["h4"], p["w4"], last.cout, st), "lad_pool_bwd")
         pre2 = False
         pre2_tiles = 0
         for bi in range(len(blocks) - 1, -1, -1):
```

Measured after the change: 50380 segments/s (median of 6 runs). Within noise of the previous version (+0.7%).
